# moberweger/deep-prior-pp

Measured on AMD Instinct MI355X. Metric: depth-crops/sec (NYU ResNet50 bs128) 1/2/4/8 GPU; mean 3D joint err (mm), higher is better.
Workload: dtype f32; 1 GPU; NYU posereg_embedding ResNet (type 0, 30-D PCA prior) train step: fused augment + fwd + bwd + ADAM, bs128/GPU fp32, 128x128x1 crops; global_batch=128, parallelism=dp1, augment=True, augment_pipelined=True, bn=local per-GPU batch statistics, launch_mode=native

## Files before the change

### deep-prior-pp_amd/csrc/bn.hip

```cpp
#include "dpp_common.h"

namespace {

constexpr int MAXQ = 256;

template <class TX>
__global__ __launch_bounds__(DPP_THREADS) void bn_stats_partial_kernel(const TX* __restrict__ X, int M, int C,
                                                                       int rpb, float* __restrict__ partial) {
    __shared__ float s_mean[DPP_THREADS * 4];
    __shared__ float s_m2[DPP_THREADS * 4];
    __shared__ float s_n[DPP_THREADS];
    const int Q = C >> 2;
    const int RP = DPP_THREADS / Q;
    const int tid = threadIdx.x;
    const int q = tid % Q, rr = tid / Q;
    const int r_begin = blockIdx.x * rpb;
    const int r_end = (r_begin + rpb < M) ? r_begin + rpb : M;
    float4 K = make_float4(0.f, 0.f, 0.f, 0.f), s1 = K, s2 = K;
    int n = 0;
    if (rr < RP) {
        for (int r = r_begin + rr; r < r_end; r += RP) {
            float4 v = dpp_ld4(X + (size_t)r * C + q * 4);
            if (n == 0) K = v;
            float dx = v.x - K.x, dy = v.y - K.y, dz = v.z - K.z, dw = v.w - K.w;
            s1.x += dx; s1.y += dy; s1.z += dz; s1.w += dw;
            s2.x += dx * dx; s2.y += dy * dy; s2.z += dz * dz; s2.w += dw * dw;
            ++n;
        }
    }
    float inv = n > 0 ? 1.0f / (float)n : 0.0f;
    s_n[tid] = (float)n;
    s_mean[tid * 4 + 0] = K.x + s1.x * inv; s_m2[tid * 4 + 0] = s2.x - s1.x * s1.x * inv;
    s_mean[tid * 4 + 1] = K.y + s1.y * inv; s_m2[tid * 4 + 1] = s2.y - s1.y * s1.y * inv;
    s_mean[tid * 4 + 2] = K.z + s1.z * inv; s_m2[tid * 4 + 2] = s2.z - s1.z * s1.z * inv;
    s_mean[tid * 4 + 3] = K.w + s1.w * inv; s_m2[tid * 4 + 3] = s2.w - s1.w * s1.w * inv;
    __syncthreads();
    for (int c = tid; c < C; c += DPP_THREADS) {
        int cq = c >> 2, ce = c & 3;
        double cn = 0.0, mean = 0.0, m2 = 0.0;
        for (int j = 0; j < RP; ++j) {
            int t = j * Q + cq;
            double nb = (double)s_n[t];
            if (nb == 0.0) continue;
            double mb = (double)s_mean[t * 4 + ce], m2b = (double)s_m2[t * 4 + ce];
            double delta = mb - mean, tot = cn + nb;
            mean += delta * nb / tot;
            m2 += m2b + delta * delta * cn * nb / tot;
            cn = tot;
        }
        partial[dpp_partial_index(0, c, blockIdx.x, C, gridDim.x)] = (float)mean;
        partial[dpp_partial_index(1, c, blockIdx.x, C, gridDim.x)] = (float)m2;
    }
}

__device__ __forceinline__ double wave_allsum(double v) {
    for (int o = 1; o < DPP_WAVE; o <<= 1) v += __shfl_xor(v, o);
    return v;
}

template <int WPC>
__device__ __forceinline__ double group_allsum(double v, double* slot) {
    v = wave_allsum(v);
    if (WPC == 1) return v;
    const int wave = threadIdx.x >> 6;
    if ((threadIdx.x & 63) == 0) slot[wave] = v;
    __syncthreads();
    return ((slot[0] + slot[1]) + slot[2]) + slot[3];
}

template <int U, int WPC>
__global__ __launch_bounds__(DPP_THREADS) void bn_finalize_kernel(const float* __restrict__ partial, int nbs, int nseg, int M, int rpb,
                                                                  int C, const float* __restrict__ gamma, float eps,
                                                                  float* __restrict__ mean_o, float* __restrict__ inv_std_o,
                                                                  float* __restrict__ scale_o, float* __restrict__ run_mean,
                                                                  float* __restrict__ run_inv_std, float alpha) {
    dpp_kernarg_warm<96>();
    __shared__ double slot_a[4], slot_b[4];
    constexpr int GT = DPP_WAVE * WPC;
    const int lane = threadIdx.x % GT;
    const int c = blockIdx.x * (DPP_THREADS / GT) + threadIdx.x / GT;
    const int cc = c < C ? c : C - 1;
    const bool upd = alpha > 0.0f && run_mean != nullptr;
    const float gam = gamma[cc];
    const float rm_old = (upd ? run_mean : gamma)[cc], ri_old = (upd ? run_inv_std : gamma)[cc];
    const int Mseg = M / nseg;
    auto rows_of = [&](int bi) { return (bi * rpb + rpb <= Mseg) ? rpb : (Mseg - bi * rpb); };
    const bool one_sweep = nseg == 1 && nbs <= GT * U;
    float pm0[U], pq0[U];
    if (one_sweep) {
        const float* pm_row = partial + dpp_partial_index(0, cc, 0, C, nbs);
        const float* pq_row = partial + dpp_partial_index(1, cc, 0, C, nbs);
        const float K = pm_row[0];
#pragma unroll
        for (int u = 0; u < U; ++u) {
            const int b = lane + u * GT;
            const int bb = b < nbs ? b : nbs - 1;
            pm0[u] = pm_row[bb];
            pq0[u] = pq_row[bb];
        }
        double s1 = 0.0, s2 = 0.0;
#pragma unroll
        for (int u = 0; u < U; ++u) {
            const int b = lane + u * GT;
            if (b < nbs) {
                const double d = (double)pm0[u] - (double)K, nb_ = (double)rows_of(b);
                s1 += nb_ * d;
                s2 += (double)pq0[u] + nb_ * d * d;
            }
        }
        s1 = group_allsum<WPC>(s1, slot_a);
        s2 = group_allsum<WPC>(s2, slot_b);
        if (lane != 0 || c >= C) return;
        const double mean1 = (double)K + s1 / (double)M;
        const double var1 = (s2 - s1 * s1 / (double)M) / (double)M;
        const float meanf = (float)mean1;
        const float inv_std = (float)(1.0 / sqrt((var1 > 0.0 ? var1 : 0.0) + (double)eps));
        mean_o[c] = meanf;
        inv_std_o[c] = inv_std;
        scale_o[c] = gam * inv_std;
        if (upd) {
            const float oma = 1.0f - alpha;
            run_mean[c] = oma * rm_old + alpha * meanf;
            run_inv_std[c] = oma * ri_old + alpha * inv_std;
        }
        return;
    }
    double snm = 0.0;
    for (int seg = 0; seg < nseg; ++seg) {
        const float* pm_row = partial + (size_t)seg * 2 * C * nbs + dpp_partial_index(0, cc, 0, C, nbs);
        const float* pq_row = partial + (size_t)seg * 2 * C * nbs + dpp_partial_index(1, cc, 0, C, nbs);
        for (int b0 = lane; b0 < nbs; b0 += GT * U) {
            float pm[U];
#pragma unroll
            for (int u = 0; u < U; ++u) {
                const int b = b0 + u * GT;
                const int bb = b < nbs ? b : nbs - 1;
                pm[u] = pm_row[bb];
            }
#pragma unroll
            for (int u = 0; u < U; ++u) {
                const int b = b0 + u * GT;
                if (b < nbs) snm += (double)rows_of(b) * (double)pm[u];
            }
        }
    }
    const double mean = group_allsum<WPC>(snm, slot_a) / (double)M;
    double q = 0.0;
    {
        for (int seg = 0; seg < nseg; ++seg) {
            const float* pm_row = partial + (size_t)seg * 2 * C * nbs + dpp_partial_index(0, cc, 0, C, nbs);
            const float* pq_row = partial + (size_t)seg * 2 * C * nbs + dpp_partial_index(1, cc, 0, C, nbs);
            for (int b0 = lane; b0 < nbs; b0 += GT * U) {
                float pm[U], pq[U];
#pragma unroll
                for (int u = 0; u < U; ++u) {
                    const int b = b0 + u * GT;
                    const int bb = b < nbs ? b : nbs - 1;
                    pm[u] = pm_row[bb];
                    pq[u] = pq_row[bb];
                }
#pragma unroll
                for (int u = 0; u < U; ++u) {
                    const int b = b0 + u * GT;
                    if (b < nbs) {
                        const double d = (double)pm[u] - mean;
                        q += (double)pq[u] + (double)rows_of(b) * d * d;
                    }
                }
            }
        }
    }
    const double m2 = group_allsum<WPC>(q, slot_b);
    if (lane != 0 || c >= C) return;
    double var = m2 / (double)M;
    float meanf = (float)mean;
    float inv_std = (float)(1.0 / sqrt(var + (double)eps));
    mean_o[c] = meanf;
    inv_std_o[c] = inv_std;
    scale_o[c] = gam * inv_std;
    if (upd) {
        float oma = 1.0f - alpha;
        run_mean[c] = oma * rm_old + alpha * meanf;
        run_inv_std[c] = oma * ri_old + alpha * inv_std;
    }
}

__global__ __launch_bounds__(DPP_THREADS) void bn_eval_coeffs_kernel(const float* __restrict__ gamma, const float* __restrict__ run_mean,
                                                                     const float* __restrict__ run_inv_std, int C,
                                                                     float* __restrict__ mean_o, float* __restrict__ inv_std_o,
                                                                     float* __restrict__ scale_o) {
    int c = blockIdx.x * DPP_THREADS + threadIdx.x;
    if (c >= C) return;
    mean_o[c] = run_mean[c];
    inv_std_o[c] = run_inv_std[c];
    scale_o[c] = gamma[c] * run_inv_std[c];
}

struct BnEvalJob { const float* gamma; const float* run_mean; const float* run_inv_std; float* mean; float* inv_std; float* scale; int C, block0; };
__global__ __launch_bounds__(DPP_THREADS) void bn_eval_coeffs_multi_kernel(const BnEvalJob* __restrict__ jobs, int njobs) {
    int lo = 0, hi = njobs - 1;
    while (lo < hi) {
        const int mid = (lo + hi + 1) >> 1;
        if ((int)blockIdx.x >= jobs[mid].block0) lo = mid; else hi = mid - 1;
    }
    const BnEvalJob jb = jobs[lo];
    const int c = ((int)blockIdx.x - jb.block0) * DPP_THREADS + threadIdx.x;
    if (c >= jb.C) return;
// ... 205 lines not shown
        if ((nb & 3) == 0) {
            for (int b = quarter * 4; b < nb; b += 16) {
                const float4 v = *reinterpret_cast<const float4*>(row + b);
                acc += ((double)v.x + (double)v.y) + ((double)v.z + (double)v.w);
            }
        } else {
            for (int b = quarter; b < nb; b += 4) acc += (double)row[b];
        }
        acc += __shfl_xor(acc, 1);
        acc += __shfl_xor(acc, 2);
        if (quarter == 0) s_sum[pair] = acc;
    }
    const float4 mu = *reinterpret_cast<const float4*>(mean + c0 + q * 4);
    const float4 is = *reinterpret_cast<const float4*>(inv_std + c0 + q * 4);
    const float4 sc = *reinterpret_cast<const float4*>(scale + c0 + q * 4);
    __syncthreads();
    if (blockIdx.x == 0 && tid < CS) {
        dbeta[c0 + tid] = (float)s_sum[tid];
        dgamma[c0 + tid] = (float)s_sum[CS + tid];
    }
    float4 a1, a2;
    a1.x = (float)(s_sum[q * 4 + 0] / (double)M); a1.y = (float)(s_sum[q * 4 + 1] / (double)M);
    a1.z = (float)(s_sum[q * 4 + 2] / (double)M); a1.w = (float)(s_sum[q * 4 + 3] / (double)M);
    a2.x = (float)(s_sum[CS + q * 4 + 0] / (double)M); a2.y = (float)(s_sum[CS + q * 4 + 1] / (double)M);
    a2.z = (float)(s_sum[CS + q * 4 + 2] / (double)M); a2.w = (float)(s_sum[CS + q * 4 + 3] / (double)M);
    float4 sa = zero4;
    for (; r < r_end; r += 4 * RP) {
#pragma unroll
        for (int u = 0; u < 4; ++u) {
            const int ru = r + u * RP;
            float4 v;
            v.x = sc.x * (g[u].x - a1.x - (x[u].x - mu.x) * is.x * a2.x);
            v.y = sc.y * (g[u].y - a1.y - (x[u].y - mu.y) * is.y * a2.y);
            v.z = sc.z * (g[u].z - a1.z - (x[u].z - mu.z) * is.z * a2.z);
            v.w = sc.w * (g[u].w - a1.w - (x[u].w - mu.w) * is.w * a2.w);
            if (add) { v.x += o[u].x; v.y += o[u].y; v.z += o[u].z; v.w += o[u].w; }
            if (ru < r_end) {
                dpp_st4(dX + (size_t)ru * C + c0 + q * 4, v);
                if (sizeof(TO) == 2) { v.x = dpp_bf16_round(v.x); v.y = dpp_bf16_round(v.y); v.z = dpp_bf16_round(v.z); v.w = dpp_bf16_round(v.w); }
                sa.x += v.x; sa.y += v.y; sa.z += v.z; sa.w += v.w;
            }
        }
        if (r + 4 * RP < r_end) fetch(r + 4 * RP);
    }
    if (colsum == nullptr) return;
    s_a[tid * 4 + 0] = sa.x; s_a[tid * 4 + 1] = sa.y; s_a[tid * 4 + 2] = sa.z; s_a[tid * 4 + 3] = sa.w;
    __syncthreads();
    if (tid < CS) {
        const int cq = tid >> 2, ce = tid & 3;
        double a = 0.0;
        for (int j = 0; j < RP; ++j) a += (double)s_a[(j * Q + cq) * 4 + ce];
        colsum[(size_t)blockIdx.x * C + c0 + tid] = (float)a;
    }
}

bool ok_c(int C) { return C >= 4 && (C & 3) == 0 && (C >> 2) <= MAXQ && (DPP_THREADS % (C >> 2) == 0 || (C >> 2) > DPP_THREADS); }

}

extern "C" int dpp_bn_stats_partial(const float* X, int M, int C, int rows_per_block, float* partial, int store, dpp_stream_t stream) {
    if (!X || !partial || M < 1 || rows_per_block < 1 || !ok_c(C) || (C >> 2) > DPP_THREADS || (store & ~DPP_ST_A)) return DPP_E_BADARG;
    int nb = dpp_cdiv(M, rows_per_block);
    if (store & DPP_ST_A)
        DPP_LAUNCH(bn_stats_partial_kernel<dpp_bf16>, dim3(nb), dim3(DPP_THREADS), 0, static_cast<hipStream_t>(stream),
                   reinterpret_cast<const dpp_bf16*>(X), M, C, rows_per_block, partial);
    else
        DPP_LAUNCH(bn_stats_partial_kernel<float>, dim3(nb), dim3(DPP_THREADS), 0, static_cast<hipStream_t>(stream), X, M, C, rows_per_block, partial);
    return dpp_launch_status();
}

extern "C" int dpp_bn_finalize(const float* partial, int nb, int nseg, int M, int rows_per_block, int C, const float* gamma, float eps,
                               float* mean, float* inv_std, float* scale, float* run_mean, float* run_inv_std, float alpha,
                               dpp_stream_t stream) {
    if (!partial || !gamma || !mean || !inv_std || !scale || nseg < 1 || M % nseg || nb != dpp_cdiv(M / nseg, rows_per_block))
        return DPP_E_BADARG;
    hipStream_t st = static_cast<hipStream_t>(stream);
#define DPP_BNF(U_, W_) DPP_LAUNCH((bn_finalize_kernel<U_, W_>), dim3(dpp_cdiv(C, 4 / W_)), dim3(DPP_THREADS), 0, st, partial, nb, nseg, \
                                           M, rows_per_block, C, gamma, eps, mean, inv_std, scale, run_mean, run_inv_std, alpha)
    if (nb <= 2 * DPP_WAVE) DPP_BNF(2, 1); else if (nb <= 8 * DPP_WAVE) DPP_BNF(8, 1); else if (nb <= 32 * DPP_WAVE) DPP_BNF(8, 4); else DPP_BNF(32, 4);
#undef DPP_BNF
    return dpp_launch_status();
}

extern "C" int dpp_bn_eval_coeffs(const float* gamma, const float* run_mean, const float* run_inv_std, int C, float* mean,
                                  float* inv_std, float* scale, dpp_stream_t stream) {
    if (!gamma || !run_mean || !run_inv_std || !mean || !inv_std || !scale || C < 1) return DPP_E_BADARG;
    DPP_LAUNCH(bn_eval_coeffs_kernel, dim3(dpp_cdiv(C, DPP_THREADS)), dim3(DPP_THREADS), 0, static_cast<hipStream_t>(stream),
                       gamma, run_mean, run_inv_std, C, mean, inv_std, scale);
    return dpp_launch_status();
}

extern "C" size_t dpp_bn_eval_job_bytes(void) { return sizeof(BnEvalJob); }

extern "C" int dpp_bn_eval_coeffs_multi(const void* jobs, int njobs, int total_blocks, dpp_stream_t stream) {
    if (!jobs || njobs < 1 || total_blocks < 1) return DPP_E_BADARG;
    DPP_LAUNCH(bn_eval_coeffs_multi_kernel, dim3(total_blocks), dim3(DPP_THREADS), 0, static_cast<hipStream_t>(stream),
               static_cast<const BnEvalJob*>(jobs), njobs);
    return dpp_launch_status();
}

extern "C" int dpp_bn_bwd_reduce(const float* dA, const float* X, int M, int C, const float* mean, const float* inv_std,
                                 const float* scale, const float* beta, int relu, float* G, int rows_per_block, float* partial,
                                 int store, dpp_stream_t stream) {
    if (!dA || !X || !G || !partial || M < 1 || rows_per_block < 1 || !ok_c(C) || (C >> 2) > DPP_THREADS || (store & ~(DPP_ST_BNX | DPP_ST_A | DPP_ST_C)))
        return DPP_E_BADARG;
    const bool x16 = (store & DPP_ST_BNX) != 0, g16 = (store & DPP_ST_A) != 0;
    if (g16 != ((store & DPP_ST_C) != 0)) return DPP_E_UNSUPPORTED;
    int nb = dpp_cdiv(M, rows_per_block);
    hipStream_t st = static_cast<hipStream_t>(stream);
#define DPP_BR(TX_, TG_) DPP_LAUNCH((bn_bwd_reduce_kernel<TX_, TG_>), dim3(nb), dim3(DPP_THREADS), 0, st, reinterpret_cast<const TG_*>(dA), \
                                    reinterpret_cast<const TX_*>(X), M, C, mean, inv_std, scale, beta, relu, reinterpret_cast<TG_*>(G), rows_per_block, partial)
    if (x16) { if (g16) DPP_BR(dpp_bf16, dpp_bf16); else DPP_BR(dpp_bf16, float); }
    else { if (g16) DPP_BR(float, dpp_bf16); else DPP_BR(float, float); }
#undef DPP_BR
    return dpp_launch_status();
}

extern "C" int dpp_bn_bwd_finalize(const float* partial, int nb, int nseg, int M, int C, float* dbeta, float* dgamma, float* c1,
                                   float* c2, const float* inv_std, const float* scale, float* q, float* p, dpp_stream_t stream) {
    if (!partial || !dbeta || !dgamma || !c1 || !c2 || nb < 1 || nseg < 1) return DPP_E_BADARG;
    if (q && !(p && inv_std && scale)) return DPP_E_BADARG;
    hipStream_t st = static_cast<hipStream_t>(stream);
#define DPP_BNBF(U_, W_) DPP_LAUNCH((bn_bwd_finalize_kernel<U_, W_>), dim3(dpp_cdiv(C, 4 / W_)), dim3(DPP_THREADS), 0, st, partial, nb, \
                                            nseg, M, C, dbeta, dgamma, c1, c2, inv_std, scale, q, p)
    if (nb <= 2 * DPP_WAVE) DPP_BNBF(2, 1); else if (nb <= 8 * DPP_WAVE) DPP_BNBF(8, 1); else if (nb <= 32 * DPP_WAVE) DPP_BNBF(8, 4); else DPP_BNBF(32, 4);
#undef DPP_BNBF
    return dpp_launch_status();
}

extern "C" int dpp_bn_bwd_apply(const float* G, const float* X, int M, int C, const float* mean, const float* inv_std,
                                const float* scale, const float* c1, const float* c2, const float* add, float* dX,
                                int rows_per_block, float* colsum_partial, int store, dpp_stream_t stream) {
    if (!G || !X || !dX || M < 1 || rows_per_block < 1 || !ok_c(C) || (C >> 2) > DPP_THREADS || (store & ~(DPP_ST_BNX | DPP_ST_A | DPP_ST_C)))
        return DPP_E_BADARG;
    const bool x16 = (store & DPP_ST_BNX) != 0, g16 = (store & DPP_ST_A) != 0, o16 = (store & DPP_ST_C) != 0;
    const dim3 grid(dpp_cdiv(M, rows_per_block));
    hipStream_t st = static_cast<hipStream_t>(stream);
#define DPP_BA(TX_, TG_, TO_) DPP_LAUNCH((bn_bwd_apply_kernel<TX_, TG_, TO_>), grid, dim3(DPP_THREADS), 0, st, reinterpret_cast<const TG_*>(G), \
                                         reinterpret_cast<const TX_*>(X), M, C, mean, inv_std, scale, c1, c2, reinterpret_cast<const TO_*>(add), \
                                         reinterpret_cast<TO_*>(dX), rows_per_block, colsum_partial)
#define DPP_BA_O(TX_, TG_) do { if (o16) DPP_BA(TX_, TG_, dpp_bf16); else DPP_BA(TX_, TG_, float); } while (0)
    if (x16) { if (g16) DPP_BA_O(dpp_bf16, dpp_bf16); else DPP_BA_O(dpp_bf16, float); }
    else { if (g16) DPP_BA_O(float, dpp_bf16); else DPP_BA_O(float, float); }
#undef DPP_BA_O
#undef DPP_BA
    return dpp_launch_status();
}

extern "C" int dpp_bn_bwd_finalize_apply_ok(int M, int C, int nb) { return M >= 1 && C >= 32 && (C & 31) == 0 && nb >= 1 && nb <= 256; }

extern "C" int dpp_bn_bwd_finalize_apply(const float* G, const float* X, int M, int C, const float* mean, const float* inv_std,
                                         const float* scale, const float* partial, int nb, const float* add, float* dX,
                                         int rows_per_block, float* colsum_partial, float* dbeta, float* dgamma, int store,
                                         dpp_stream_t stream) {
    if (!G || !X || !dX || !partial || !dbeta || !dgamma || rows_per_block < 1 || (store & ~(DPP_ST_BNX | DPP_ST_A | DPP_ST_C))) return DPP_E_BADARG;
    if (!dpp_bn_bwd_finalize_apply_ok(M, C, nb)) return DPP_E_UNSUPPORTED;
    const bool x16 = (store & DPP_ST_BNX) != 0, g16 = (store & DPP_ST_A) != 0, o16 = (store & DPP_ST_C) != 0;
    const dim3 grid(dpp_cdiv(M, rows_per_block), C / 32);
    hipStream_t st = static_cast<hipStream_t>(stream);
#define DPP_BFA(TX_, TG_, TO_) DPP_LAUNCH((bn_bwd_finalize_apply_kernel<TX_, TG_, TO_>), grid, dim3(DPP_THREADS), 0, st, reinterpret_cast<const TG_*>(G), \
                                          reinterpret_cast<const TX_*>(X), M, C, mean, inv_std, scale, partial, nb, reinterpret_cast<const TO_*>(add), \
                                          reinterpret_cast<TO_*>(dX), rows_per_block, colsum_partial, dbeta, dgamma)
#define DPP_BFA_O(TX_, TG_) do { if (o16) DPP_BFA(TX_, TG_, dpp_bf16); else DPP_BFA(TX_, TG_, float); } while (0)
    if (x16) { if (g16) DPP_BFA_O(dpp_bf16, dpp_bf16); else DPP_BFA_O(dpp_bf16, float); }
    else { if (g16) DPP_BFA_O(float, dpp_bf16); else DPP_BFA_O(float, float); }
#undef DPP_BFA_O
// ... 4 lines not shown
```

### deep-prior-pp_amd/csrc/conv3x3.hip

```cpp
#include <stdio.h>
#include <stdlib.h>
#include "dpp_common.h"
#include "conv3x3_wgrad_t.h"

namespace {

struct C3Stage {
    unsigned m_hw2, m_tw2;
    int lqp;
};

__host__ __device__ inline unsigned c3_magic(int d) { return (unsigned)(0x100000000ull / (unsigned)d) + 1u; }

struct Conv3Args {
    const float* X;
    int N, H, W, Ci, Co;
    dpp_act act;
    const float* Wk;
    int allw;
    int wide;
    const float* bias;
    const float* residual;
    float* Y;
    dpp_epilogue epi;
    int store;
    int lth, ltw;
    int img;
    int tiles_x, tiles_y;
    C3Stage sg;
    unsigned long long* prof;
    int ntiles, woff;
};

typedef __bf16 c3_bf16x8 __attribute__((ext_vector_type(8)));
typedef __bf16 c3_bf16x4 __attribute__((ext_vector_type(4)));

template <int PREC> struct C3Prec;
template <> struct C3Prec<0> { typedef float elem; static constexpr int PAD = 4; __device__ static int kp(int Ci) { return Ci; } };
template <> struct C3Prec<1> { typedef __bf16 elem; static constexpr int PAD = 8; __device__ static int kp(int Ci) { return Ci < 32 ? 32 : Ci; } };

__device__ __forceinline__ void c3_store4(float* dst, float4 v) { *reinterpret_cast<float4*>(dst) = v; }
__device__ __forceinline__ void c3_store4(__bf16* dst, float4 v) {
    c3_bf16x4 o;
    o[0] = (__bf16)v.x; o[1] = (__bf16)v.y; o[2] = (__bf16)v.z; o[3] = (__bf16)v.w;
    *reinterpret_cast<c3_bf16x4*>(dst) = o;
}

__device__ __forceinline__ void tile_origin(const Conv3Args& a, int bid, int& n0, int& y0, int& x0) {
    int bx = bid % a.tiles_x;
    int t = bid / a.tiles_x;
    int by = t % a.tiles_y;
    int bn = t / a.tiles_y;
    n0 = bn * a.img;
    y0 = by << a.lth;
    x0 = bx << a.ltw;
}

template <int UB, class E, class TX>
__device__ __forceinline__ void stage_halo(const TX* __restrict__ X, int N, int H, int W, int Ci, const dpp_act& act, int n0,
                                           int y0, int x0, int TH, int TW, int IMG, E* Ah, int LDA, int KP, const C3Stage& sg) {
    if (KP < Ci) KP = Ci;
    const int HW2 = (TH + 2) * (TW + 2), TW2 = TW + 2;
    const int HP = IMG * HW2;
    const int c0 = ((int)threadIdx.x & ((1 << sg.lqp) - 1)) * 4;
    const int hstep = DPP_THREADS >> sg.lqp;
    if (c0 >= KP) return;
    const bool cld = c0 < Ci;
    float4 mu = make_float4(0.f, 0.f, 0.f, 0.f), sc = mu, be = mu;
    if (cld && (act.mode & 2)) {
        mu = *reinterpret_cast<const float4*>(act.mean + c0);
        sc = *reinterpret_cast<const float4*>(act.scale + c0);
        be = *reinterpret_cast<const float4*>(act.beta + c0);
    }
    for (int hb = (int)threadIdx.x >> sg.lqp; hb < HP; hb += UB * hstep) {
        float4 v[UB];
        bool in[UB];
#pragma unroll
        for (int u = 0; u < UB; ++u) {
            const int hp = hb + u * hstep;
            const int im = (int)__umulhi((unsigned)hp, sg.m_hw2), rem = hp - im * HW2;
            const int hy = (int)__umulhi((unsigned)rem, sg.m_tw2), hx = rem - hy * TW2;
            const int n = n0 + im, y = y0 + hy - 1, x = x0 + hx - 1;
            in[u] = hp < HP && cld && n < N && y >= 0 && y < H && x >= 0 && x < W;
            v[u] = make_float4(0.f, 0.f, 0.f, 0.f);
            if (in[u]) v[u] = dpp_ld4(X + (((size_t)n * H + y) * W + x) * Ci + c0);
        }
#pragma unroll
        for (int u = 0; u < UB; ++u) {
            const int hp = hb + u * hstep;
            if (hp < HP) {
                float4 t = v[u];
                if (in[u]) {
                    if (act.mode & 2) {
                        t.x = dpp_fma(t.x - mu.x, sc.x, be.x); t.y = dpp_fma(t.y - mu.y, sc.y, be.y);
                        t.z = dpp_fma(t.z - mu.z, sc.z, be.z); t.w = dpp_fma(t.w - mu.w, sc.w, be.w);
                    }
                    if (act.mode & 1) { t.x = fmaxf(t.x, 0.0f); t.y = fmaxf(t.y, 0.0f); t.z = fmaxf(t.z, 0.0f); t.w = fmaxf(t.w, 0.0f); }
                }
                c3_store4(&Ah[hp * LDA + c0], t);
            }
        }
    }
}

template <int BM, int BN, int PREC = 0, class TX = float, bool EST = false>
__global__ __launch_bounds__(DPP_THREADS) void conv3x3_kernel(Conv3Args a) {
    dpp_kernarg_warm<sizeof(Conv3Args)>();
    HIP_DYNAMIC_SHARED(float4, smem4)
    float* smem = reinterpret_cast<float*>(smem4);
    typedef typename C3Prec<PREC>::elem elem;
    constexpr int RM = BM / 64;
    constexpr int CN = BN / 16;
    constexpr int KSTEP = PREC ? 32 : 16;
    const int TH = 1 << a.lth, TW = 1 << a.ltw;
    const int Ci = a.Ci, KP = C3Prec<PREC>::kp(Ci), LDA = KP + C3Prec<PREC>::PAD;
    const int HP = a.img * (TH + 2) * (TW + 2);
    elem* Ah = reinterpret_cast<elem*>(smem);
    elem* Bs = Ah + HP * LDA;
    const int tid = threadIdx.x, wave = tid >> 6, lane = tid & 63, l15 = lane & 15, kq = lane >> 4;
    int n0, y0, x0;
    tile_origin(a, blockIdx.x, n0, y0, x0);
    const int col0 = blockIdx.y * BN;

    dpp_stamp(a.prof, 0);
    dpp_wide_coef wco;
    if (a.wide) wco.load<BN>(col0, a.Co, a.bias, a.epi, a.Y);
    if (((HP + (DPP_THREADS >> a.sg.lqp) - 1) >> (8 - a.sg.lqp)) <= 4)
        stage_halo<4>(reinterpret_cast<const TX*>(a.X), a.N, a.H, a.W, Ci, a.act, n0, y0, x0, TH, TW, a.img, Ah, LDA, KP, a.sg);
    else
        stage_halo<8>(reinterpret_cast<const TX*>(a.X), a.N, a.H, a.W, Ci, a.act, n0, y0, x0, TH, TW, a.img, Ah, LDA, KP, a.sg);
    dpp_stamp(a.prof, 1);

    int hbase[RM];
#pragma unroll
    for (int rt = 0; rt < RM; ++rt) {
        int row = wave * (BM / 4) + rt * 16 + l15;
        int im = row >> (a.lth + a.ltw);
        int ty = (row >> a.ltw) & (TH - 1);
        int tx = row & (TW - 1);
        hbase[rt] = (im * (TH + 2) + ty + 1) * (TW + 2) + tx + 1;
    }

    f32x4 acc[RM][CN];
#pragma unroll
    for (int i = 0; i < RM; ++i)
#pragma unroll
        for (int j = 0; j < CN; ++j) acc[i][j] = (f32x4){0.f, 0.f, 0.f, 0.f};

    constexpr int WSLOTS = (BN * 16 + DPP_THREADS - 1) / DPP_THREADS;
    float4 wreg[WSLOTS];
    const float* wp[WSLOTS];
    int wo[WSLOTS];
#pragma unroll
    for (int s = 0; s < WSLOTS; ++s) {
        const int slot = tid + s * DPP_THREADS;
        const int j = slot >> a.sg.lqp, c0 = (slot & ((1 << a.sg.lqp) - 1)) * 4;
        wo[s] = (j < BN && c0 < KP) ? j * LDA + c0 : -1;
        wp[s] = (j < BN && c0 < Ci && col0 + j < a.Co) ? a.Wk + (size_t)(col0 + j) * 9 * Ci + c0 : nullptr;
    }
    auto wfetch = [&](int tap) {
#pragma unroll
        for (int s = 0; s < WSLOTS; ++s) {
            wreg[s] = make_float4(0.f, 0.f, 0.f, 0.f);
            if (wp[s] != nullptr) wreg[s] = *reinterpret_cast<const float4*>(wp[s] + tap * Ci);
        }
    };
    auto wcommit = [&](elem* dst) {
#pragma unroll
        for (int s = 0; s < WSLOTS; ++s)
            if (wo[s] >= 0) c3_store4(&dst[wo[s]], wreg[s]);
    };
    const bool allw = a.allw != 0;
    if (allw) {
#pragma unroll
        for (int t3 = 0; t3 < 9; t3 += 3) {
            float4 w3[3][WSLOTS];
#pragma unroll
            for (int u = 0; u < 3; ++u)
#pragma unroll
                for (int s = 0; s < WSLOTS; ++s) {
                    w3[u][s] = make_float4(0.f, 0.f, 0.f, 0.f);
                    if (wp[s] != nullptr) w3[u][s] = *reinterpret_cast<const float4*>(wp[s] + (t3 + u) * Ci);
                }
#pragma unroll
            for (int u = 0; u < 3; ++u)
#pragma unroll
                for (int s = 0; s < WSLOTS; ++s)
                    if (wo[s] >= 0) c3_store4(&Bs[(t3 + u) * BN * LDA + wo[s]], w3[u][s]);
        }
    } else {
        wfetch(0);
        wcommit(Bs);
    }
    __syncthreads();
    dpp_stamp(a.prof, 2);
    for (int tap = 0; tap < 9; ++tap) {
        const elem* Bcur = allw ? Bs + tap * BN * LDA : Bs + (tap & 1) * BN * LDA;
        if (!allw && tap + 1 < 9) wfetch(tap + 1);
        const int toff = (tap / 3 - 1) * (TW + 2) + (tap % 3 - 1);
        for (int kc = 0; kc < KP; kc += KSTEP) {
            if constexpr (PREC == 0) {
                float4 av[RM], bv[CN];
#pragma unroll
                for (int rt = 0; rt < RM; ++rt)
                    av[rt] = *reinterpret_cast<const float4*>(&Ah[(hbase[rt] + toff) * LDA + kc + kq * 4]);
#pragma unroll
                for (int ct = 0; ct < CN; ++ct)
                    bv[ct] = *reinterpret_cast<const float4*>(&Bcur[(ct * 16 + l15) * LDA + kc + kq * 4]);
#pragma unroll
// ... 425 lines not shown
                        v = dpp_ld4(reinterpret_cast<const TY*>(a.dY) + (((size_t)n * a.H + y) * a.W + x) * Co + c0);
                    *reinterpret_cast<float4*>(&Ys[row * LDY + c0]) = v;
                }
            }
        }
        __syncthreads();

#pragma unroll 1
        for (int rc = 0; rc < BM; rc += 16) {
            int hb[4];
#pragma unroll
            for (int t = 0; t < 4; ++t) {
                int row = rc + kq * 4 + t;
                int im = row >> (a.lth + a.ltw);
                int ty = (row >> a.ltw) & (TH - 1);
                int tx = row & (TW - 1);
                hb[t] = ((im * (TH + 2) + ty + 1) * (TW + 2) + tx + 1) * LDA;
            }
            const float* yrow = Ys + (rc + kq * 4) * LDY;
#pragma unroll
            for (int i = 0; i < MAXACC; ++i) {
                if (yoff[i] >= 0) {
#pragma unroll
                    for (int t = 0; t < 4; ++t) {
                        float av = yrow[t * LDY + yoff[i]];
                        float bv = Ah[hb[t] + xoff[i]];
                        acc[i] = __builtin_amdgcn_mfma_f32_16x16x4f32(av, bv, acc[i], 0, 0, 0);
                    }
                }
            }
        }
    }

    float* out = a.partial + (size_t)blockIdx.x * Co * 9 * Ci;
#pragma unroll
    for (int i = 0; i < MAXACC; ++i) {
        int p = wave + 4 * i;
        if (p < pairs) {
            int tap = tap0 + p / NT, tile = p % NT;
            int to = tile / ntc, tc = tile - to * ntc;
#pragma unroll
            for (int r = 0; r < 4; ++r) {
                int o = to * 16 + kq * 4 + r, c = tc * 16 + l15;
                out[((size_t)o * 9 + tap) * Ci + c] = acc[i][r];
            }
        }
    }
}

constexpr int WGRAD_MAX_BLOCKS = 256;

int ilog2(int v) { int l = 0; while ((1 << l) < v) ++l; return l; }

void pick_tile(int N, int H, int W, int bm, int& lth, int& ltw, int& img) {
    int tw = 1; while (tw * 2 <= W && tw < 16) tw *= 2;
    int th = 1; while (th * 2 <= H && th < 8 && th * tw * 2 <= bm) th *= 2;
    while (th * tw > bm) tw /= 2;
    img = bm / (th * tw);
    lth = ilog2(th); ltw = ilog2(tw);
}

}

extern "C" int dpp_conv3x3_tiling(int N, int H, int W, int bm, int* th, int* tw, int* img) {
    int lth, ltw, im;
    if (bm != 64 && bm != 128) return -1;
    pick_tile(N, H, W, bm, lth, ltw, im);
    if (th) *th = 1 << lth;
    if (tw) *tw = 1 << ltw;
    if (img) *img = im;
    return dpp_cdiv(W, 1 << ltw) * dpp_cdiv(H, 1 << lth) * dpp_cdiv(N, im);
}

static int conv3x3_launch(const float* X, int N, int H, int W, int Ci, const dpp_act* act, const float* Wk, int Co,
                          const float* bias, const float* residual, float* Y, int bm, const dpp_epilogue* epi, int precision, int store,
                          dpp_stream_t stream) {
    if (!X || !Wk || !Y || N < 1 || H < 1 || W < 1 || Ci < 16 || (Ci & 15) || Co < 16 || (Co & 15)) return DPP_E_BADARG;
    if (store & ~(DPP_ST_A | DPP_ST_C | DPP_ST_BNX)) return DPP_E_BADARG;
    Conv3Args a;
    a.store = store;
    a.X = X; a.N = N; a.H = H; a.W = W; a.Ci = Ci; a.Co = Co;
    a.prof = dpp_prof_buffer;
    if (act && (act->mode & 4)) return DPP_E_UNSUPPORTED;
    if (act) a.act = *act; else { a.act.mode = 0; a.act.cmod = 1; a.act.mean = a.act.scale = a.act.beta = nullptr; }
    a.Wk = Wk; a.bias = bias; a.residual = residual; a.Y = Y;
    if (epi) a.epi = *epi; else a.epi = dpp_epilogue{};
    if (a.epi.bn_x && !(a.epi.bn_mean && a.epi.bn_inv_std && a.epi.bn_scale && a.epi.bn_beta && a.epi.bn_partial)) return DPP_E_BADARG;
    long pixels = (long)N * H * W;
    if (bm == 0) bm = (pixels / 128) * dpp_cdiv(Co, 64) >= 512 ? 128 : 64;
    pick_tile(N, H, W, bm, a.lth, a.ltw, a.img);
    int TH = 1 << a.lth, TW = 1 << a.ltw;
    a.tiles_x = dpp_cdiv(W, TW); a.tiles_y = dpp_cdiv(H, TH);
    int nblk = a.tiles_x * a.tiles_y * dpp_cdiv(N, a.img);
    if (Ci > 64) return DPP_E_UNSUPPORTED;
    a.sg.m_hw2 = c3_magic((TH + 2) * (TW + 2));
    a.sg.m_tw2 = c3_magic(TW + 2);
    a.sg.lqp = ilog2(((precision && Ci < 32) ? 32 : Ci) / 4);
    int bn = Co >= 64 ? 64 : (Co >= 32 ? 32 : 16);
    static const long min_wgs = []() { const char* e = getenv("DPP_C3_MIN_WGS"); return (e && atol(e) > 0) ? atol(e) : 512L; }();
    while (bn > 16 && (long)nblk * dpp_cdiv(Co, bn) < min_wgs) bn >>= 1;
    size_t halo = (size_t)a.img * (TH + 2) * (TW + 2);
    const size_t rowb = precision ? (size_t)((Ci < 32 ? 32 : Ci) + 8) * 2 : (size_t)(Ci + 4) * sizeof(float);
    a.allw = (halo + 9 * bn) * rowb <= 48 * 1024;
    size_t lds = (halo + (a.allw ? 9 : 2) * bn) * rowb;
    static const bool wide_ok = []() { const char* e = getenv("DPP_GEMM_WIDE_EPILOGUE"); return !(e && e[0] == '0'); }();
    auto al16 = [](const void* p) { return (reinterpret_cast<uintptr_t>(p) & 15) == 0; };
    a.wide = wide_ok && al16(Y) && al16(residual) && al16(a.epi.bn_x) && al16(bias) && al16(a.epi.bn_mean) && al16(a.epi.bn_scale) &&
             al16(a.epi.bn_beta) && al16(a.epi.bn_inv_std);
    if ((store & (DPP_ST_C | DPP_ST_BNX)) && !a.wide) return DPP_E_UNSUPPORTED;
    size_t need = a.wide ? ((size_t)bm * (bn + 4) + 16 * bn) * sizeof(float) : (size_t)4 * bn * sizeof(float);
    if (lds < need) lds = need;
    if (lds > 160 * 1024) return DPP_E_UNSUPPORTED;
    dim3 grid(nblk, dpp_cdiv(Co, bn));
    hipStream_t st = static_cast<hipStream_t>(stream);
    const char* pe = getenv("DPP_C3_PERSIST");
    const int persist = pe ? atoi(pe) : 1024;
    static const int p_min = []() { const char* e = getenv("DPP_C3_P_MIN_TILES"); return e ? atoi(e) : 0; }();
    const bool p_always = nblk > p_min;
    auto pow2 = [](int v) { return v > 0 && (v & (v - 1)) == 0; };
    const char* g0e = getenv("DPP_C3_P_64W");
    const int bn64 = g0e ? atoi(g0e) : 32;
    const bool geom0 = (Ci == 16 || Ci == 32 || (Ci == 64 && precision && (bn64 == 64 || bn64 == 32))) && a.img == 1 && TH == 8 && TW == 16 && H % TH == 0 && W % TW == 0 &&
                       pow2(a.tiles_x) && pow2(a.tiles_y);
    const char* g1e = getenv("DPP_C3_P_64");
    const int geom1_on = g1e ? atoi(g1e) : 1;
    const bool geom1 = (geom1_on >= 2 || (geom1_on == 1 && precision)) && Ci == 64 && H == 8 && W == 8 && a.img == 2 && TH == 8 && TW == 8;
    if (persist > 0 && a.wide && Ci == Co && bm == 128 && p_always && (geom0 || geom1) && (long)N * H * W * Ci < (1L << 31)) {
        const int pbn = geom1 ? 16 : (Ci == 64 ? bn64 : Co);
        const size_t pneed = ((size_t)bm * (pbn + 4) + 16 * pbn) * sizeof(float);
        const size_t region0 = (halo * rowb > pneed ? halo * rowb : pneed);
        const size_t ldsp = ((region0 + 15) & ~(size_t)15) + 9 * pbn * rowb + 8 * 64 * sizeof(float);
        const long pwgs = (long)(persist < nblk ? persist : nblk) * (Co / pbn);
        if (ldsp <= 64 * 1024 || (ldsp <= 80 * 1024 && pwgs <= 512) || (ldsp <= 160 * 1024 && pwgs <= 256)) {
            a.woff = (int)((region0 + 15) & ~(size_t)15);
            a.ntiles = nblk;
            if (geom0) { a.ltw = ilog2(a.tiles_x); a.lth = ilog2(a.tiles_y); }
            const dim3 gp(persist < nblk ? persist : nblk, Co / pbn);
            if (getenv("DPP_C3_PERSIST_VERBOSE")) fprintf(stderr, "conv3x3_p_kernel: %d tiles on %d x %d workgroups, C %d, prec %d, store %d, %zu bytes of LDS\n", nblk, (int)gp.x, (int)gp.y, Ci, precision, store, ldsp);
#define DPP_C3P(CI_, BN_, P_, T_, E_, G_) do { \
            if (ldsp > 64 * 1024) (void)hipFuncSetAttribute(reinterpret_cast<const void*>(&conv3x3_p_kernel<CI_, BN_, P_, T_, E_, G_>), hipFuncAttributeMaxDynamicSharedMemorySize, (int)ldsp); \
            DPP_LAUNCH((conv3x3_p_kernel<CI_, BN_, P_, T_, E_, G_>), gp, dim3(DPP_THREADS), ldsp, st, a); return dpp_launch_status(); } while (0)
#define DPP_C3PE(CI_, BN_, P_, T_, G_) do { if (store & (DPP_ST_C | DPP_ST_BNX)) DPP_C3P(CI_, BN_, P_, T_, true, G_); else DPP_C3P(CI_, BN_, P_, T_, false, G_); } while (0)
#define DPP_C3PX(CI_, BN_, G_) if (Ci == CI_) { \
            if (precision) { if (store & DPP_ST_A) DPP_C3PE(CI_, BN_, 1, dpp_bf16, G_); else DPP_C3PE(CI_, BN_, 1, float, G_); } \
            if (store & DPP_ST_A) DPP_C3PE(CI_, BN_, 0, dpp_bf16, G_); else DPP_C3PE(CI_, BN_, 0, float, G_); }
            DPP_C3PX(16, 16, 0) DPP_C3PX(32, 32, 0)
            if (geom1) { DPP_C3PX(64, 16, 1) }
            if (Ci == 64 && precision && pbn == 64) { if (store & DPP_ST_A) DPP_C3PE(64, 64, 1, dpp_bf16, 0); else DPP_C3PE(64, 64, 1, float, 0); }
            if (Ci == 64 && precision && pbn == 32) { if (store & DPP_ST_A) DPP_C3PE(64, 32, 1, dpp_bf16, 0); else DPP_C3PE(64, 32, 1, float, 0); }
#undef DPP_C3PX
#undef DPP_C3PE
#undef DPP_C3P
        }
    }
#define DPP_C3K(BM_, BN_, P_, T_, E_) do { \
        if (lds > 64 * 1024) (void)hipFuncSetAttribute(reinterpret_cast<const void*>(&conv3x3_kernel<BM_, BN_, P_, T_, E_>), hipFuncAttributeMaxDynamicSharedMemorySize, (int)lds); \
        DPP_LAUNCH((conv3x3_kernel<BM_, BN_, P_, T_, E_>), grid, dim3(DPP_THREADS), lds, st, a); return dpp_launch_status(); } while (0)
#define DPP_C3E(BM_, BN_, P_, T_) do { if (store & (DPP_ST_C | DPP_ST_BNX)) DPP_C3K(BM_, BN_, P_, T_, true); else DPP_C3K(BM_, BN_, P_, T_, false); } while (0)
#define DPP_C3(BM_, BN_) if (bm == BM_ && bn == BN_) { \
        if (precision) { if (store & DPP_ST_A) DPP_C3E(BM_, BN_, 1, dpp_bf16); else DPP_C3E(BM_, BN_, 1, float); } \
        if (store & DPP_ST_A) DPP_C3E(BM_, BN_, 0, dpp_bf16); else DPP_C3E(BM_, BN_, 0, float); }
    DPP_C3(128, 64) DPP_C3(128, 32) DPP_C3(128, 16) DPP_C3(64, 64) DPP_C3(64, 32) DPP_C3(64, 16)
#undef DPP_C3
#undef DPP_C3E
#undef DPP_C3K
    return DPP_E_UNSUPPORTED;
}

extern "C" int dpp_conv3x3(const float* X, int N, int H, int W, int Ci, const dpp_act* act, const float* Wk, int Co,
                           const float* bias, const float* residual, float* Y, int bm, const dpp_epilogue* epi, int store, dpp_stream_t stream) {
    return conv3x3_launch(X, N, H, W, Ci, act, Wk, Co, bias, residual, Y, bm, epi, 0, store, stream);
}

extern "C" int dpp_conv3x3_bf16(const float* X, int N, int H, int W, int Ci, const dpp_act* act, const float* Wk, int Co,
                                const float* bias, const float* residual, float* Y, int bm, const dpp_epilogue* epi, int store, dpp_stream_t stream) {
    return conv3x3_launch(X, N, H, W, Ci, act, Wk, Co, bias, residual, Y, bm, epi, 1, store, stream);
}

extern "C" int dpp_conv3x3_wtrans(const float* Wk, int Co, int Ci, float* Wd, dpp_stream_t stream) {
    if (!Wk || !Wd || Co < 1 || Ci < 1) return DPP_E_BADARG;
    int n = Co * 9 * Ci;
    DPP_LAUNCH(conv3x3_wtrans_kernel, dim3(dpp_cdiv(n, DPP_THREADS)), dim3(DPP_THREADS), 0, static_cast<hipStream_t>(stream), Wk, Co, Ci, Wd);
    return dpp_launch_status();
}

extern "C" size_t dpp_wtrans_job_bytes(void) { return sizeof(WtransJob); }

extern "C" int dpp_conv3x3_wtrans_multi(const void* jobs_dev, int njobs, int total_blocks, dpp_stream_t stream) {
    if (!jobs_dev || njobs < 1 || total_blocks < 1) return DPP_E_BADARG;
    DPP_LAUNCH(conv3x3_wtrans_multi_kernel, dim3(total_blocks), dim3(DPP_THREADS), 0, static_cast<hipStream_t>(stream),
               static_cast<const WtransJob*>(jobs_dev), njobs);
    return dpp_launch_status();
}

static void wgrad_geometry(int N, int H, int W, int Ci, int Co, int bm, int& nblk, int& taps_pb) {
    int lth, ltw, img;
    pick_tile(N, H, W, bm, lth, ltw, img);
    const int ntiles = dpp_cdiv(W, 1 << ltw) * dpp_cdiv(H, 1 << lth) * dpp_cdiv(N, img);
    const int NT = (Co >> 4) * (Ci >> 4);
    taps_pb = NT <= 4 ? 9 : (NT <= 16 ? 3 : 1);
    int cap = WGRAD_MAX_BLOCKS;
    while (cap > 32 && (long)cap * Co * 9 * Ci * 4 > 6L * 1024 * 1024) cap >>= 1;
    if (Ci == 64 && Co == 64 && dpp_conv3x3_wgrad_t_ok(N, H, W, Ci, Co, nullptr) && cap < 64) cap = 64;
    if (Ci == 32 && Co == 32 && ntiles >= 1024 && dpp_conv3x3_wgrad_t_ok(N, H, W, Ci, Co, nullptr) && cap < 256) cap = 256;
    nblk = ntiles < cap ? ntiles : cap;
    while (taps_pb > 1 && nblk * (9 / taps_pb) < 256) taps_pb = taps_pb == 9 ? 3 : 1;
}

extern "C" int dpp_conv3x3_wgrad_blocks(int N, int H, int W, int Ci, int Co, int bm) {
    if ((bm != 64 && bm != 128) || Ci < 16 || Co < 16) return -1;
    int nblk, taps_pb;
    wgrad_geometry(N, H, W, Ci, Co, bm, nblk, taps_pb);
    return nblk;
}

static int conv3x3_wgrad_launch(const float* X, int N, int H, int W, int Ci, const dpp_act* act, const float* dY, int Co,
                                float* partial, int bm, int store, int precision, dpp_stream_t stream);

extern "C" int dpp_conv3x3_wgrad(const float* X, int N, int H, int W, int Ci, const dpp_act* act, const float* dY, int Co,
                                 float* partial, int bm, int store, dpp_stream_t stream) {
    return conv3x3_wgrad_launch(X, N, H, W, Ci, act, dY, Co, partial, bm, store, 0, stream);
}

extern "C" int dpp_conv3x3_wgrad_bf16_ok(int N, int H, int W, int Ci, int Co) { return dpp_conv3x3_wgrad_t_ok(N, H, W, Ci, Co, nullptr) ? 1 : 0; }

extern "C" int dpp_conv3x3_wgrad_bf16(const float* X, int N, int H, int W, int Ci, const dpp_act* act, const float* dY, int Co,
                                      float* partial, int bm, int store, dpp_stream_t stream) {
    return conv3x3_wgrad_launch(X, N, H, W, Ci, act, dY, Co, partial, bm, store, 1, stream);
}

static int conv3x3_wgrad_launch(const float* X, int N, int H, int W, int Ci, const dpp_act* act, const float* dY, int Co,
                                float* partial, int bm, int store, int precision, dpp_stream_t stream) {
    if (!X || !dY || !partial || N < 1 || Ci < 16 || (Ci & 15) || Co < 16 || (Co & 15) || (bm != 64 && bm != 128) || (store & ~(DPP_ST_A | DPP_ST_B))) return DPP_E_BADARG;
    const int y16 = (store & DPP_ST_B) ? 1 : 0;
    Wgrad3Args a;
    a.X = X; a.N = N; a.H = H; a.W = W; a.Ci = Ci; a.Co = Co; a.dY = dY; a.partial = partial;
    if (act && (act->mode & 4)) return DPP_E_UNSUPPORTED;
    if (act) a.act = *act; else { a.act.mode = 0; a.act.cmod = 1; a.act.mean = a.act.scale = a.act.beta = nullptr; }
    pick_tile(N, H, W, bm, a.lth, a.ltw, a.img);
    int TH = 1 << a.lth, TW = 1 << a.ltw;
    a.tiles_x = dpp_cdiv(W, TW); a.tiles_y = dpp_cdiv(H, TH);
    a.ntiles = a.tiles_x * a.tiles_y * dpp_cdiv(N, a.img);
    int nblk, taps_pb;
    wgrad_geometry(N, H, W, Ci, Co, bm, nblk, taps_pb);
    if (dpp_conv3x3_wgrad_t_ok(N, H, W, Ci, Co, act))
        return dpp_conv3x3_wgrad_t_launch(X, N, H, W, Ci, act, dY, partial, nblk, taps_pb, store, precision, static_cast<hipStream_t>(stream));
    if (precision) return DPP_E_UNSUPPORTED;
    int NT = (Co >> 4) * (Ci >> 4);
    int pairs = taps_pb * NT;
    int maxacc = dpp_cdiv(pairs, 4);
    a.taps_pb = taps_pb;
    a.sg.m_hw2 = c3_magic((TH + 2) * (TW + 2));
    a.sg.m_tw2 = c3_magic(TW + 2);
    a.sg.lqp = ilog2(Ci / 4);
    a.lqy = ilog2(Co / 4);
    size_t lds = ((size_t)a.img * (TH + 2) * (TW + 2) * (Ci + 4) + (size_t)bm * (Co + 4)) * sizeof(float);
    if (lds > 160 * 1024) return DPP_E_UNSUPPORTED;
    dim3 grid(nblk, 9 / taps_pb);
    hipStream_t st = static_cast<hipStream_t>(stream);
#define DPP_W3K(BM_, MA_, T_, Y_) do { \
        if (lds > 64 * 1024) (void)hipFuncSetAttribute(reinterpret_cast<const void*>(&conv3x3_wgrad_kernel<BM_, MA_, T_, Y_>), hipFuncAttributeMaxDynamicSharedMemorySize, (int)lds); \
        DPP_LAUNCH((conv3x3_wgrad_kernel<BM_, MA_, T_, Y_>), grid, dim3(DPP_THREADS), lds, st, a); return dpp_launch_status(); } while (0)
#define DPP_W3(BM_, MA_) if (bm == BM_ && maxacc <= MA_) { \
        if (store & DPP_ST_A) { if (y16) DPP_W3K(BM_, MA_, dpp_bf16, dpp_bf16); else DPP_W3K(BM_, MA_, dpp_bf16, float); } \
        else { if (y16) DPP_W3K(BM_, MA_, float, dpp_bf16); else DPP_W3K(BM_, MA_, float, float); } }
    DPP_W3(128, 3) DPP_W3(128, 4) DPP_W3(128, 9) DPP_W3(128, 12) DPP_W3(128, 16)
    DPP_W3(64, 3) DPP_W3(64, 4) DPP_W3(64, 9) DPP_W3(64, 12) DPP_W3(64, 16)
#undef DPP_W3
    return DPP_E_UNSUPPORTED;
}
```

### deep-prior-pp_amd/csrc/conv3x3_wgrad_t.hip

```cpp
#include <stdlib.h>
#include "dpp_common.h"
#include "conv3x3_wgrad_t.h"

namespace {

template <class T> struct W3Raw;
template <> struct W3Raw<float> {
    typedef float4 type;
    __device__ static __forceinline__ type ld(const float* p) { return *reinterpret_cast<const float4*>(p); }
    __device__ static __forceinline__ float4 widen(const type& r) { return r; }
};
template <> struct W3Raw<dpp_bf16> {
    typedef uint2 type;
    __device__ static __forceinline__ type ld(const dpp_bf16* p) { return *reinterpret_cast<const uint2*>(p); }
    __device__ static __forceinline__ float4 widen(const type& r) {
        return make_float4(__uint_as_float(r.x << 16), __uint_as_float(r.x & 0xffff0000u), __uint_as_float(r.y << 16),
                           __uint_as_float(r.y & 0xffff0000u));
    }
};

struct Wgrad3TArgs {
    const void* X;
    const void* dY;
    float* partial;
// ... 222 lines not shown
                            const w3_u32x4 bv = w3_shift8(b0, lo, hi, dxi);
                            acc[dyi * 3 + dxi][n] = __builtin_amdgcn_mfma_f32_16x16x32_bf16(__builtin_bit_cast(dpp_bf16x8, av), __builtin_bit_cast(dpp_bf16x8, bv),
                                                                                            acc[dyi * 3 + dxi][n], 0, 0, 0);
                        }
                    }
                }
                }
            }
        }
    }

    if (C == 16) {
        f32x4* const red = reinterpret_cast<f32x4*>(smem);
        __syncthreads();
        if (wave >= 2) {
#pragma unroll
            for (int t = 0; t < TPB; ++t) red[((wave - 2) * TPB + t) * 64 + lane] = acc[t][0];
        }
        __syncthreads();
        if (wave < 2) {
#pragma unroll
            for (int t = 0; t < TPB; ++t) acc[t][0] += red[(wave * TPB + t) * 64 + lane];
        }
        __syncthreads();
        if (wave == 1) {
#pragma unroll
            for (int t = 0; t < TPB; ++t) red[t * 64 + lane] = acc[t][0];
        }
        __syncthreads();
        if (wave == 0) {
#pragma unroll
            for (int t = 0; t < TPB; ++t) acc[t][0] += red[t * 64 + lane];
        }
    }
    if (C != 16 || wave == 0) {
        float* out = a.partial + (size_t)blockIdx.x * C * 9 * C;
#pragma unroll
        for (int t = 0; t < TPB; ++t) {
            const int tap = tap0 + t;
#pragma unroll
            for (int n = 0; n < NTC; ++n)
#pragma unroll
                for (int r = 0; r < 4; ++r) {
                    const int o = (OS ? (int)blockIdx.y : to) * 16 + kq * 4 + r, c = (tc0 + n) * 16 + l15;
                    out[((size_t)o * 9 + tap) * C + c] = acc[t][n][r];
                }
        }
    }
}

template <int C, int TPB, bool PB>
int w3t_launch_typed(const Wgrad3TArgs& a, dim3 grid, size_t lds, bool x16, bool y16, hipStream_t st) {
#define DPP_W3T(TX_, TY_) do { DPP_LAUNCH((conv3x3_wgrad_t_kernel<C, TPB, TX_, TY_, PB>), grid, dim3(DPP_THREADS), lds, st, a); return dpp_launch_status(); } while (0)
    if (x16) { if (y16) DPP_W3T(dpp_bf16, dpp_bf16); else DPP_W3T(dpp_bf16, float); }
    if (y16) DPP_W3T(float, dpp_bf16);
    DPP_W3T(float, float);
#undef DPP_W3T
}

template <int C, bool PB>
int w3t_launch_taps(const Wgrad3TArgs& a, int taps_pb, dim3 grid, size_t lds, bool x16, bool y16, hipStream_t st) {
    if (taps_pb == 9) return w3t_launch_typed<C, 9, PB>(a, grid, lds, x16, y16, st);
    if (taps_pb == 3) return w3t_launch_typed<C, 3, PB>(a, grid, lds, x16, y16, st);
    return w3t_launch_typed<C, 1, PB>(a, grid, lds, x16, y16, st);
}

template <bool PB>
int w3t_launch_c64(const Wgrad3TArgs& a, dim3 grid, size_t lds, bool x16, bool y16, hipStream_t st) {
#define DPP_W3T64(TX_, TY_) do { \
        if (lds > 64 * 1024) (void)hipFuncSetAttribute(reinterpret_cast<const void*>(&conv3x3_wgrad_t_kernel<64, 9, TX_, TY_, PB, true>), hipFuncAttributeMaxDynamicSharedMemorySize, (int)lds); \
        DPP_LAUNCH((conv3x3_wgrad_t_kernel<64, 9, TX_, TY_, PB, true>), grid, dim3(DPP_THREADS), lds, st, a); return dpp_launch_status(); } while (0)
    if (x16) { if (y16) DPP_W3T64(dpp_bf16, dpp_bf16); else DPP_W3T64(dpp_bf16, float); }
    if (y16) DPP_W3T64(float, dpp_bf16);
    DPP_W3T64(float, float);
#undef DPP_W3T64
}

}

bool dpp_conv3x3_wgrad_t_ok(int N, int H, int W, int Ci, int Co, const dpp_act* act) {
    static const bool on = []() { const char* e = getenv("DPP_WGRAD3_T"); return !(e && e[0] == '0'); }();
    if (!on || Ci != Co || (Ci != 16 && Ci != 32 && Ci != 64) || W < 12 || H < 4) return false;
    if ((long)N * H * W * Ci >= (1L << 31)) return false;
    if (act && ((act->mode & 4) || (act->mode && (act->cmod & 3)))) return false;
    return true;
}

int dpp_conv3x3_wgrad_t_launch(const float* X, int N, int H, int W, int C, const dpp_act* act, const float* dY, float* partial, int nblk,
                               int taps_pb, int store, int precision, hipStream_t st) {
    Wgrad3TArgs a;
    a.X = X; a.dY = dY; a.partial = partial; a.N = N; a.H = H; a.W = W;
    if (act) a.act = *act; else { a.act = dpp_act{}; a.act.mode = 0; a.act.cmod = 4; }
    a.tiles_x = dpp_cdiv(W, W3_TW); a.tiles_y = dpp_cdiv(H, W3_TH);
    a.ntiles = a.tiles_x * a.tiles_y * N;
    const bool x16 = (store & DPP_ST_A) != 0, y16 = (store & DPP_ST_B) != 0;
    const dim3 grid(nblk, 9 / taps_pb);
    size_t lds = precision ? (size_t)C * (W3_CPXB + W3_CPYB) * 2 : (size_t)C * (W3_CPX + W3_CPY) * sizeof(float);
    const size_t red = C == 16 ? (size_t)2 * taps_pb * 64 * 16 : 0;
    if (lds < red) lds = red;
    if (C == 64) {
        const dim3 g64(nblk, 4);
        const size_t l64 = precision ? (size_t)(64 * W3_CPXB + 16 * W3_CPYB) * 2 : (size_t)(64 * W3_CPX + 16 * W3_CPY) * sizeof(float);
        return precision ? w3t_launch_c64<true>(a, g64, l64, x16, y16, st) : w3t_launch_c64<false>(a, g64, l64, x16, y16, st);
    }
    if (precision) return C == 16 ? w3t_launch_taps<16, true>(a, taps_pb, grid, lds, x16, y16, st) : w3t_launch_taps<32, true>(a, taps_pb, grid, lds, x16, y16, st);
    return C == 16 ? w3t_launch_taps<16, false>(a, taps_pb, grid, lds, x16, y16, st) : w3t_launch_taps<32, false>(a, taps_pb, grid, lds, x16, y16, st);
}
```

### deep-prior-pp_amd/csrc/convpool.hip

```cpp
#include "dpp_common.h"

namespace {

constexpr int TP = 8;
constexpr int WG_WAVES = DPP_THREADS / DPP_WAVE;

struct cp_geom {
    int N, H, W, Ci, kh, kw, pad, Co, pool, Hp, Wp, tiles_x, tiles_y, sy, sx;
};

__host__ inline bool cp_make_geom(cp_geom& g, int N, int H, int W, int Ci, int kh, int kw, int pad, int Co, int pool) {
    if (N < 1 || H < 1 || W < 1 || Ci < 1 || Ci > 32 || Co < 1 || Co > 32 || kh < 1 || kw < 1 || kh > 7 || kw > 7 || pad < 0 ||
        pad > 3 || pool < 1 || pool > 4)
        return false;
    g.N = N; g.H = H; g.W = W; g.Ci = Ci; g.kh = kh; g.kw = kw; g.pad = pad; g.Co = Co; g.pool = pool;
    int Hc = H + 2 * pad - kh + 1, Wc = W + 2 * pad - kw + 1;
    if (Hc < pool || Wc < pool) return false;
    g.Hp = Hc / pool; g.Wp = Wc / pool;
    g.tiles_y = dpp_cdiv(g.Hp, TP); g.tiles_x = dpp_cdiv(g.Wp, TP);
    g.sy = TP * pool + kh - 1; g.sx = TP * pool + kw - 1;
    return true;
}

__device__ __forceinline__ void cp_stage(float* xs, const float* __restrict__ X, const dpp_act& act, const cp_geom& g, int n, int ty,
// ... 371 lines not shown
    for (int s0 = threadIdx.x; s0 < S * S * g.Co; s0 += DPP_THREADS * SU) {
        float d[SU];
        int m[SU];
#pragma unroll
        for (int u = 0; u < SU; ++u) {
            const int s = s0 + u * DPP_THREADS;
            const int co = s % g.Co, rc = s / g.Co;
            const int c = rc % S, r = rc / S;
            const int cy = cy0 + r, cx = cx0 + c;
            const bool ok = (s < S * S * g.Co) & (cy >= 0) & (cx >= 0) & (cy < Hc) & (cx < Wc);
            const int py = ok ? cy / P : 0, px = ok ? cx / P : 0;
            const int j = ok ? (cy - py * P) * P + (cx - px * P) : 0;
            const size_t o = (((size_t)n * g.Hp + py) * g.Wp + px) * g.Co + (ok ? co : 0);
            d[u] = dY[o];
            m[u] = ok ? ((ties ? (int)ties[o] : 1) >> j) & 1 : 0;
        }
#pragma unroll
        for (int u = 0; u < SU; ++u) {
            const int s = s0 + u * DPP_THREADS;
            const int co = s % g.Co, rc = s / g.Co;
            if (s < S * S * g.Co) gcs[(co * S + rc / S) * S + rc % S] = m[u] ? d[u] : 0.0f;
        }
    }
    for (int s = threadIdx.x; s < g.Co * taps * 8; s += DPP_THREADS) {
        const int ci = s & 7, ct = s >> 3;
        ws[s] = (c0 + ci < g.Ci) ? Wk[(size_t)ct * g.Ci + c0 + ci] : 0.0f;
    }
    __syncthreads();
    const int ly0 = (threadIdx.x >> 4) * PX, lx0 = (threadIdx.x & 15) * PX;
    float acc[PX * PX][8];
#pragma unroll
    for (int q = 0; q < PX * PX; ++q)
#pragma unroll
        for (int c = 0; c < 8; ++c) acc[q][c] = 0.0f;
    for (int co = 0; co < g.Co; ++co) {
        float patch[R][R];
        const float* gp = gcs + (co * S + ly0) * S + lx0;
#pragma unroll
        for (int r = 0; r < R; ++r)
#pragma unroll
            for (int c = 0; c < R; ++c) patch[r][c] = gp[r * S + c];
#pragma unroll
        for (int dy = 0; dy < K; ++dy)
#pragma unroll
            for (int dx = 0; dx < K; ++dx) {
                const float4* wp = reinterpret_cast<const float4*>(ws + (co * taps + dy * K + dx) * 8);
                const float4 w0 = wp[0], w1 = wp[1];
                const float w[8] = {w0.x, w0.y, w0.z, w0.w, w1.x, w1.y, w1.z, w1.w};
#pragma unroll
                for (int qy = 0; qy < PX; ++qy)
#pragma unroll
                    for (int qx = 0; qx < PX; ++qx) {
                        const float gv = patch[qy + K - 1 - dy][qx + K - 1 - dx];
#pragma unroll
                        for (int c = 0; c < 8; ++c) acc[qy * PX + qx][c] = fmaf(gv, w[c], acc[qy * PX + qx][c]);
                    }
            }
    }
#pragma unroll
    for (int qy = 0; qy < PX; ++qy)
#pragma unroll
        for (int qx = 0; qx < PX; ++qx) {
            const int iy = iy0 + ly0 + qy, ix = ix0 + lx0 + qx;
            if (iy < g.H && ix < g.W) {
                float* o = dX + (((size_t)n * g.H + iy) * g.W + ix) * g.Ci + c0;
#pragma unroll
                for (int c = 0; c < 8; ++c)
                    if (c0 + c < g.Ci) o[c] = acc[qy * PX + qx][c];
            }
        }
}

inline dpp_act cp_act(const dpp_act* a) {
    dpp_act r = {nullptr, nullptr, nullptr, 0, 1};
    return a ? *a : r;
}

constexpr int CP_WGRAD_MAX_BLOCKS = 512;

}

extern "C" int dpp_convpool_fwd(const float* X, int N, int H, int W, int Ci, const dpp_act* act, const float* Wk, int kh, int kw, int pad,
                                int Co, int pool, const float* bias, float* Y, uint16_t* ties, dpp_stream_t stream) {
    if (act && (act->mode & 4)) return DPP_E_UNSUPPORTED;
    cp_geom g;
    if (!X || !Wk || !bias || !Y || !cp_make_geom(g, N, H, W, Ci, kh, kw, pad, Co, pool)) return DPP_E_BADARG;
    size_t lds = (size_t)g.sy * g.sx * Ci * sizeof(float);
    if (lds > 64 * 1024) return DPP_E_UNSUPPORTED;
    dim3 grid(N * g.tiles_x * g.tiles_y), block(DPP_THREADS);
    hipStream_t st = static_cast<hipStream_t>(stream);
    int cpt = dpp_cdiv(Co, WG_WAVES);
    const size_t lds_fast = lds + (size_t)Co * kh * kw * Ci * sizeof(float);
    if (kh == kw && cpt <= 2 && lds_fast <= 64 * 1024) {
#define DPP_CPF(K_, P_) if (kh == K_ && pool == P_) { \
            DPP_LAUNCH((convpool_fwd_fast_kernel<K_, P_, 2>), grid, block, lds_fast, st, X, cp_act(act), Wk, bias, Y, ties, g); \
            return dpp_launch_status(); }
        DPP_CPF(5, 4) DPP_CPF(5, 2) DPP_CPF(5, 1) DPP_CPF(3, 1) DPP_CPF(3, 2)
#undef DPP_CPF
    }
    if (cpt <= 2)
        DPP_LAUNCH((convpool_fwd_kernel<2>), grid, block, lds, st, X, cp_act(act), Wk, bias, Y, ties, g);
    else if (cpt <= 4)
        DPP_LAUNCH((convpool_fwd_kernel<4>), grid, block, lds, st, X, cp_act(act), Wk, bias, Y, ties, g);
    else
        DPP_LAUNCH((convpool_fwd_kernel<8>), grid, block, lds, st, X, cp_act(act), Wk, bias, Y, ties, g);
    return dpp_launch_status();
}

extern "C" int dpp_convpool_wgrad_blocks(int N, int Hp, int Wp) {
    if (N < 1 || Hp < 1 || Wp < 1) return 0;
    long total = (long)N * dpp_cdiv(Hp, TP) * dpp_cdiv(Wp, TP);
    return (int)(total < CP_WGRAD_MAX_BLOCKS ? total : CP_WGRAD_MAX_BLOCKS);
}

extern "C" int dpp_convpool_wgrad(const float* X, int N, int H, int W, int Ci, const dpp_act* act, const float* dY, const uint16_t* ties,
                                  int kh, int kw, int pad, int Co, int pool, float* partial, dpp_stream_t stream) {
    if (act && (act->mode & 4)) return DPP_E_UNSUPPORTED;
    cp_geom g;
    if (!X || !dY || !partial || !cp_make_geom(g, N, H, W, Ci, kh, kw, pad, Co, pool) || (pool > 1 && !ties)) return DPP_E_BADARG;
    size_t lds = ((size_t)g.sy * g.sx * Ci + 2 * 64 * Co) * sizeof(float);
    if (lds > 64 * 1024) return DPP_E_UNSUPPORTED;
    int total = N * g.tiles_x * g.tiles_y;
    int blocks = dpp_convpool_wgrad_blocks(N, g.Hp, g.Wp);
    if (kh * kw * Ci <= DPP_THREADS && pool <= 2) {
        const int T = (Ci <= 2) ? 32 : 16;
        const size_t need = ((size_t)Ci * (T + kh - 1) * (T + kw - 1) + (size_t)T * T * 8) * sizeof(float);
        if (need <= 64 * 1024 && (size_t)DPP_THREADS * 8 <= (size_t)T * T * 8) {
            const int tiles_x = dpp_cdiv(g.Wp * pool, T), tiles_y = dpp_cdiv(g.Hp * pool, T);
            DPP_LAUNCH(convpool_wgrad_dense_kernel, dim3(blocks, dpp_cdiv(Co, 8)), dim3(DPP_THREADS), need, static_cast<hipStream_t>(stream), X,
                       cp_act(act), dY, ties, partial, g, T, tiles_x, tiles_y, N * tiles_x * tiles_y);
            return dpp_launch_status();
        }
    }
    DPP_LAUNCH(convpool_wgrad_kernel, dim3(blocks), dim3(DPP_THREADS), lds, static_cast<hipStream_t>(stream), X, cp_act(act), dY,
                       ties, partial, g, total);
    return dpp_launch_status();
}

extern "C" int dpp_convpool_dgrad(const float* dY, const uint16_t* ties, int N, int H, int W, int Ci, const float* Wk, int kh, int kw,
                                  int pad, int Co, int pool, float* dX, dpp_stream_t stream) {
    cp_geom g;
    if (!dY || !Wk || !dX || !cp_make_geom(g, N, H, W, Ci, kh, kw, pad, Co, pool) || (pool > 1 && !ties)) return DPP_E_BADARG;
    if (kh == kw) {
        const int px = ((long)N * dpp_cdiv(H, 32) * dpp_cdiv(W, 32) >= 1024 && (H > 16 || W > 16)) ? 2 : 1, T = 16 * px, S = T + kh - 1;
        const size_t lds = ((size_t)Co * S * S + (size_t)Co * kh * kw * 8) * sizeof(float);
        const int tiles_x = dpp_cdiv(W, T), tiles_y = dpp_cdiv(H, T);
        const dim3 fgrid(N * tiles_x * tiles_y, dpp_cdiv(Ci, 8));
        if (lds <= 64 * 1024) {
#define DPP_CPD(K_, P_, PX_) if (kh == K_ && pool == P_ && px == PX_) { \
                DPP_LAUNCH((convpool_dgrad_fast_kernel<K_, P_, PX_>), fgrid, dim3(DPP_THREADS), lds, static_cast<hipStream_t>(stream), dY, ties, \
                           Wk, dX, g, tiles_x, tiles_y); \
                return dpp_launch_status(); }
            DPP_CPD(5, 2, 2) DPP_CPD(5, 2, 1) DPP_CPD(5, 1, 2) DPP_CPD(5, 1, 1) DPP_CPD(3, 1, 2) DPP_CPD(3, 1, 1) DPP_CPD(3, 2, 2) DPP_CPD(3, 2, 1)
            DPP_CPD(5, 4, 2) DPP_CPD(5, 4, 1)
#undef DPP_CPD
        }
    }
    size_t npix = (size_t)N * H * W;
    dim3 grid((unsigned)((npix + DPP_THREADS - 1) / DPP_THREADS), dpp_cdiv(Ci, 8));
    DPP_LAUNCH(convpool_dgrad_kernel, grid, dim3(DPP_THREADS), 0, static_cast<hipStream_t>(stream), dY, ties, Wk, dX, g);
    return dpp_launch_status();
}
```

### deep-prior-pp_amd/csrc/dpp_common.h

```cpp
#pragma once
#include <hip/hip_runtime.h>
#include <stdint.h>
#include "../../include/dpp_hip.h"

typedef float f32x4 __attribute__((ext_vector_type(4)));

typedef __bf16 dpp_bf16;
typedef __bf16 dpp_bf16x4 __attribute__((ext_vector_type(4)));
typedef __bf16 dpp_bf16x8 __attribute__((ext_vector_type(8)));

template <class T> __device__ __forceinline__ float4 dpp_ld4(const T* p);
template <> __device__ __forceinline__ float4 dpp_ld4<float>(const float* p) { return *reinterpret_cast<const float4*>(p); }
template <> __device__ __forceinline__ float4 dpp_ld4<dpp_bf16>(const dpp_bf16* p) {
    const dpp_bf16x4 v = *reinterpret_cast<const dpp_bf16x4*>(p);
    return make_float4((float)v[0], (float)v[1], (float)v[2], (float)v[3]);
}
template <class T> __device__ __forceinline__ float dpp_ld1(const T* p) { return (float)p[0]; }
template <class T> __device__ __forceinline__ void dpp_st4(T* p, float4 v);
template <> __device__ __forceinline__ void dpp_st4<float>(float* p, float4 v) { *reinterpret_cast<float4*>(p) = v; }
template <> __device__ __forceinline__ void dpp_st4<dpp_bf16>(dpp_bf16* p, float4 v) {
    dpp_bf16x4 o;
    o[0] = (dpp_bf16)v.x; o[1] = (dpp_bf16)v.y; o[2] = (dpp_bf16)v.z; o[3] = (dpp_bf16)v.w;
    *reinterpret_cast<dpp_bf16x4*>(p) = o;
}
// ... 89 lines not shown
extern unsigned long long* dpp_prof_buffer;

#ifdef DPP_HIP_EMU
#define DPP_WAVES_PER_EU(lo, hi)
#else
#define DPP_WAVES_PER_EU(lo, hi) __attribute__((amdgpu_waves_per_eu(lo, hi)))
#endif

#ifdef DPP_HIP_EMU
#define DPP_SCHED_FENCE()
#else
#define DPP_SCHED_FENCE() __builtin_amdgcn_sched_barrier(0)
#endif

#ifdef DPP_HIP_EMU
#define DPP_SETPRIO(p)
#else
#define DPP_SETPRIO(p) __builtin_amdgcn_s_setprio(p)
#endif

#ifdef DPP_HIP_EMU
#define DPP_WAVE_SYNC() ((void)__shfl_xor(0, 1))
#else
#define DPP_WAVE_SYNC() __builtin_amdgcn_wave_barrier()
#endif

template <int NBYTES>
__device__ __forceinline__ void dpp_kernarg_warm() {
#ifndef DPP_HIP_EMU
    typedef __attribute__((address_space(4))) const int kint;
    kint* ka = (kint*)__builtin_amdgcn_kernarg_segment_ptr();
    constexpr int L = (NBYTES + 63) / 64;
    int t[L];
#pragma unroll
    for (int i = 0; i < L; ++i) t[i] = ka[i * 16];
#pragma unroll
    for (int i = 0; i < L; ++i) asm volatile("" ::"s"(t[i]));
#endif
}

__device__ __forceinline__ int dpp_map_row(const dpp_rowmap& m, int r) {
    if (m.s == 1) return r;
    int n = r / m.HoWo;
    int q = r - n * m.HoWo;
    int y = q / m.Wo;
    int x = q - y * m.Wo;
    return n * m.HiWi + (y * m.s) * m.Wi + x * m.s;
}

__device__ __forceinline__ float dpp_fma(float a, float b, float c) { return __builtin_fmaf(a, b, c); }

__device__ __forceinline__ float dpp_act1(float x, const dpp_act& a, int c) {
    float v = x;
    if (a.mode & 2) v = dpp_fma(x - a.mean[c], a.scale[c], a.beta[c]);
    if (a.mode & 1) v = fmaxf(v, 0.0f);
    return v;
}

__device__ __forceinline__ float4 dpp_act4(float4 x, const dpp_act& a, int c) {
    float4 v = x;
    if (a.mode & 2) {
        const float4 mu = *reinterpret_cast<const float4*>(a.mean + c);
        const float4 sc = *reinterpret_cast<const float4*>(a.scale + c);
        const float4 be = *reinterpret_cast<const float4*>(a.beta + c);
        v.x = dpp_fma(x.x - mu.x, sc.x, be.x);
        v.y = dpp_fma(x.y - mu.y, sc.y, be.y);
        v.z = dpp_fma(x.z - mu.z, sc.z, be.z);
        v.w = dpp_fma(x.w - mu.w, sc.w, be.w);
    }
    if (a.mode & 1) {
        v.x = fmaxf(v.x, 0.0f);
        v.y = fmaxf(v.y, 0.0f);
        v.z = fmaxf(v.z, 0.0f);
        v.w = fmaxf(v.w, 0.0f);
    }
    return v;
}

__device__ __forceinline__ float dpp_f4_get(const float4& v, int i) {
    return i == 0 ? v.x : (i == 1 ? v.y : (i == 2 ? v.z : v.w));
}

__device__ __forceinline__ size_t dpp_partial_index(int s, int c, int b, int C, int NB) { return ((size_t)s * C + c) * NB + b; }


template <int CN, int WM, int WN, int BN>
__device__ __forceinline__ void dpp_tile_colsum(float (&s)[CN], float* red, int wm, int wn, int l15, int kq) {
#pragma unroll
    for (int ct = 0; ct < CN; ++ct) {
        s[ct] += __shfl_xor(s[ct], 16);
        s[ct] += __shfl_xor(s[ct], 32);
    }
    if (WM > 1) {
        __syncthreads();
        if (kq == 0) {
#pragma unroll
            for (int ct = 0; ct < CN; ++ct) red[wm * BN + wn * (BN / WN) + ct * 16 + l15] = s[ct];
        }
        __syncthreads();
#pragma unroll
        for (int ct = 0; ct < CN; ++ct) {
            float t = 0.0f;
#pragma unroll
            for (int w = 0; w < WM; ++w) t += red[w * BN + wn * (BN / WN) + ct * 16 + l15];
            s[ct] = t;
        }
    }
}

struct dpp_wide_coef {
    float cbias[4], cmean[4], cscale[4], cbeta[4], cistd[4];
    float4 raw[5];
    bool on_bias, on_bn;
    template <int BN>
    __device__ __forceinline__ void load(int col0, int N, const float* bias, const dpp_epilogue& ep, const float* safe) {
        const int col = col0 + ((int)threadIdx.x % (BN / 4)) * 4;
        const bool cin = col < N;
        on_bias = cin && bias != nullptr;
        on_bn = cin && ep.bn_x != nullptr;
        raw[0] = *reinterpret_cast<const float4*>(on_bias ? bias + col : safe);
        raw[1] = *reinterpret_cast<const float4*>(on_bn ? ep.bn_mean + col : safe);
        raw[2] = *reinterpret_cast<const float4*>(on_bn ? ep.bn_scale + col : safe);
        raw[3] = *reinterpret_cast<const float4*>(on_bn ? ep.bn_beta + col : safe);
        raw[4] = *reinterpret_cast<const float4*>(on_bn ? ep.bn_inv_std + col : safe);
    }
    __device__ __forceinline__ void finish() {
        auto quad = [](const float4& v, bool on, float (&dst)[4]) {
            dst[0] = on ? v.x : 0.0f; dst[1] = on ? v.y : 0.0f; dst[2] = on ? v.z : 0.0f; dst[3] = on ? v.w : 0.0f;
        };
        quad(raw[0], on_bias, cbias);
        quad(raw[1], on_bn, cmean);
        quad(raw[2], on_bn, cscale);
        quad(raw[3], on_bn, cbeta);
        quad(raw[4], on_bn, cistd);
    }
};

template <int RM, int CN, int WM, int WN, int BM, int BN, int NIMG = 1, bool ST = false, class RowOff>
__device__ __forceinline__ void dpp_epilogue_wide(f32x4 (&acc)[RM][CN], float* smem, int col0, int N, dpp_wide_coef& co,
                                                  const float* residual, float* C, const dpp_epilogue& ep, int nvalid, int wm,
                                                  int wn, int l15, int kq, RowOff rowoff, int img = 0, int store = 0, int blk = -1, int nblk = 0) {
    const int pblk = blk >= 0 ? blk : (int)blockIdx.x, pnblk = blk >= 0 ? nblk : (int)gridDim.x;
    const bool c16 = ST && (store & DPP_ST_C) != 0, x16 = ST && (store & DPP_ST_BNX) != 0;
    co.finish();
    constexpr int LDT = BN + 4;
    constexpr int Q = BN / 4;
    constexpr int RSTEP = DPP_THREADS / Q;
    constexpr int ITERS = (BM + RSTEP - 1) / RSTEP;
    float* Ts = smem;
    float* red = smem + NIMG * BM * LDT;
    const int tid = threadIdx.x, lane = tid & 63, wave = tid >> 6;
    const int cq = tid % Q, rb = tid / Q;
    const int col = col0 + cq * 4;
    const bool cin = col < N;
    const bool bn = ep.bn_x != nullptr;
    long rofs[ITERS];
    float4 res32[ITERS], bnx32[ITERS];
    uint2 res16[ITERS], bnx16[ITERS];
    auto request = [&](int it) {
        const int rl = rb + it * RSTEP;
        rofs[it] = (rl < BM && cin) ? rowoff(rl) : -1L;
        const size_t o = rofs[it] >= 0 ? (size_t)rofs[it] + col : (size_t)0;
        if (residual) {
            if (c16) res16[it] = *reinterpret_cast<const uint2*>(reinterpret_cast<const dpp_bf16*>(residual) + o);
            else res32[it] = *reinterpret_cast<const float4*>(residual + o);
        }
// ... 135 lines not shown
```

### deep-prior-pp_amd/csrc/gemm.hip

```cpp
#include "gemm_kernels.h"

namespace {

__global__ __launch_bounds__(DPP_THREADS) void reduce_partials_kernel(const float* __restrict__ partial, int nz, int n,
                                                                      const float* __restrict__ bias, int nbias,
                                                                      float* __restrict__ out, int ZL) {
    __shared__ float red[DPP_THREADS];
    const int CB = DPP_THREADS / ZL;
    const int col = threadIdx.x % CB, zl = threadIdx.x / CB;
    for (int i0 = blockIdx.x * CB; i0 < n; i0 += gridDim.x * CB) {
        int i = i0 + col;
        float s = 0.0f;
        if (i < n)
            for (int z = zl; z < nz; z += ZL) s += partial[(size_t)z * n + i];
        if (ZL > 1) {
            red[threadIdx.x] = s;
            __syncthreads();
            if (zl == 0) {
                for (int j = 1; j < ZL; ++j) s += red[j * CB + col];
            }
        }
        if (zl == 0 && i < n) {
            if (bias) s += bias[i % nbias];
            out[i] = s;
// ... 9 lines not shown
};

constexpr int RM_COLS = 64;

__global__ __launch_bounds__(DPP_THREADS) void reduce_multi_kernel(const ReduceJob* __restrict__ jobs, int njobs) {
    __shared__ __attribute__((aligned(16))) float red[DPP_THREADS * 4];
    __shared__ int s_job;
    if (threadIdx.x == 0) {
        int lo = 0, hi = njobs - 1;
        while (lo < hi) {
            int mid = (lo + hi + 1) >> 1;
            if (jobs[mid].block0 <= (int)blockIdx.x) lo = mid; else hi = mid - 1;
        }
        s_job = lo;
    }
    __syncthreads();
    const ReduceJob jb = jobs[s_job];
    constexpr int ZL = 16, CQ = DPP_THREADS / ZL;
    const int cq = threadIdx.x % CQ, zl = threadIdx.x / CQ;
    const int i = ((int)blockIdx.x - jb.block0) * RM_COLS + cq * 4;
    const int n = jb.n, nz = jb.nz;
    const bool vec = (n & 3) == 0 && (reinterpret_cast<uintptr_t>(jb.partial) & 15) == 0;
    float s[4][4];
#pragma unroll
    for (int u = 0; u < 4; ++u)
#pragma unroll
        for (int j = 0; j < 4; ++j) s[u][j] = 0.0f;
    if (i < n) {
        if (vec) {
            const float* p = jb.partial + i;
            int z = zl;
            for (; z + 3 * ZL < nz; z += 4 * ZL) {
                float4 v[4];
#pragma unroll
                for (int u = 0; u < 4; ++u) v[u] = *reinterpret_cast<const float4*>(p + (size_t)(z + u * ZL) * n);
#pragma unroll
                for (int u = 0; u < 4; ++u) { s[u][0] += v[u].x; s[u][1] += v[u].y; s[u][2] += v[u].z; s[u][3] += v[u].w; }
            }
            for (; z < nz; z += ZL) {
                const float4 v = *reinterpret_cast<const float4*>(p + (size_t)z * n);
                s[0][0] += v.x; s[0][1] += v.y; s[0][2] += v.z; s[0][3] += v.w;
            }
        } else {
            for (int z = zl; z < nz; z += ZL)
#pragma unroll
                for (int j = 0; j < 4; ++j)
                    if (i + j < n) s[0][j] += jb.partial[(size_t)z * n + i + j];
        }
    }
    float4 t;
    t.x = (s[0][0] + s[1][0]) + (s[2][0] + s[3][0]);
    t.y = (s[0][1] + s[1][1]) + (s[2][1] + s[3][1]);
    t.z = (s[0][2] + s[1][2]) + (s[2][2] + s[3][2]);
    t.w = (s[0][3] + s[1][3]) + (s[2][3] + s[3][3]);
    *reinterpret_cast<float4*>(&red[threadIdx.x * 4]) = t;
    __syncthreads();
    if (zl == 0 && i < n) {
        for (int j = 1; j < ZL; ++j) {
            const float4 o = *reinterpret_cast<const float4*>(&red[(j * CQ + cq) * 4]);
            t.x += o.x; t.y += o.y; t.z += o.z; t.w += o.w;
        }
        if (vec && (reinterpret_cast<uintptr_t>(jb.out) & 15) == 0) *reinterpret_cast<float4*>(jb.out + i) = t;
        else {
            const float tv[4] = {t.x, t.y, t.z, t.w};
#pragma unroll
            for (int j = 0; j < 4; ++j)
                if (i + j < n) jb.out[i + j] = tv[j];
        }
    }
}

bool aligned16(const void* p) { return (reinterpret_cast<uintptr_t>(p) & 15) == 0; }

static int gemm_prepare(const dpp_gemm_desc* dp, GemmArgs& ga) {
    if (!dp || !dp->A || !dp->B || dp->M <= 0 || dp->N <= 0 || dp->K <= 0) return DPP_E_BADARG;
    ga.d = *dp;
    ga.prof = dpp_prof_buffer;
    dpp_gemm_desc& d = ga.d;
    if (d.splitk < 1) d.splitk = 1;
    if (d.splitk > 1 && !d.partial) return DPP_E_BADARG;
    if (d.splitk > 1 && (d.epi.stats || d.epi.bn_x)) return DPP_E_BADARG;
    if (d.epi.bn_x && !(d.epi.bn_mean && d.epi.bn_inv_std && d.epi.bn_scale && d.epi.bn_beta && d.epi.bn_partial)) return DPP_E_BADARG;
    if (d.splitk == 1 && !d.C) return DPP_E_BADARG;
    if (d.actA.mode && d.actA.cmod <= 0) return DPP_E_BADARG;
    if (d.actB.mode && d.actB.cmod <= 0) return DPP_E_BADARG;
    ga.vecA = aligned16(d.A) && (d.lda % 4 == 0);
    if (d.actB.mode & 4) return DPP_E_UNSUPPORTED;
    if (d.actA.mode & 4) {
        if (d.actA.mode != 4 || d.variant == 1 || !d.actA.x2 || !d.actA.aux || !d.actA.mean || !d.actA.scale || !d.actA.beta) return DPP_E_BADARG;
        ga.vecA = ga.vecA && aligned16(d.actA.x2) && aligned16(d.actA.out);
        if (d.actA.out && (!d.a_kc || d.splitk != 1 || d.mapA.s != 1)) return DPP_E_UNSUPPORTED;
        if (!(aligned16(d.actA.mean) && aligned16(d.actA.scale) && aligned16(d.actA.beta) && aligned16(d.actA.aux))) return DPP_E_BADARG;
    }
    ga.vecB = aligned16(d.B) && (d.ldb % 4 == 0);
    if (d.store & ~(DPP_ST_A | DPP_ST_B | DPP_ST_C | DPP_ST_BNX)) return DPP_E_BADARG;
    if (d.precision != 0 && d.precision != 1) return DPP_E_BADARG;
    if (d.precision == 1 && (d.variant == 1 || (d.actA.mode & 4))) return DPP_E_UNSUPPORTED;
    if ((d.store & DPP_ST_A) && (!ga.vecA || (d.actA.mode & 4))) return DPP_E_UNSUPPORTED;
    if ((d.store & DPP_ST_B) && !ga.vecB) return DPP_E_UNSUPPORTED;
    if ((d.store & (DPP_ST_C | DPP_ST_BNX)) && d.splitk != 1) return DPP_E_UNSUPPORTED;
    ga.shA = (d.store & DPP_ST_A) ? 1 : 0;
    ga.shB = (d.store & DPP_ST_B) ? 1 : 0;
    static const bool wide_ok = []() { const char* e = getenv("DPP_GEMM_WIDE_EPILOGUE"); return !(e && e[0] == '0'); }();
    ga.wide = wide_ok && d.splitk == 1 && d.N % 4 == 0 && d.ldc % 4 == 0 && aligned16(d.C) && aligned16(d.residual) &&
              aligned16(d.epi.bn_x) && aligned16(d.bias) && aligned16(d.epi.bn_mean) && aligned16(d.epi.bn_scale) &&
              aligned16(d.epi.bn_beta) && aligned16(d.epi.bn_inv_std);
    if ((d.actA.mode & 2) && !(aligned16(d.actA.mean) && aligned16(d.actA.scale) && aligned16(d.actA.beta))) return DPP_E_BADARG;
    if ((d.actB.mode & 2) && !(aligned16(d.actB.mean) && aligned16(d.actB.scale) && aligned16(d.actB.beta))) return DPP_E_BADARG;
    if ((d.store & (DPP_ST_C | DPP_ST_BNX)) && !ga.wide) return DPP_E_UNSUPPORTED;
    return DPP_OK;
}

}

extern "C" int dpp_abi_version(void) { return DPP_ABI_VERSION; }

extern "C" int dpp_gemm_variant_rows(const dpp_gemm_desc* dp) {
    GemmArgs ga;
    if (gemm_prepare(dp, ga) != DPP_OK) return 0;
    if (ga.d.variant == 2) return ksplit_bn(ga.d, ga) ? 32 : 0;
    if (ga.d.variant == 3) return stream16_rows(ga.d, ga);
    if (ga.d.variant == 4) return dpp_gemm_expand_rows(ga.d, ga);
    return 0;
}

extern "C" int dpp_gemm(const dpp_gemm_desc* dp, dpp_stream_t stream) {
    GemmArgs ga;
    const int prep = gemm_prepare(dp, ga);
    if (prep != DPP_OK) return prep;
    dpp_gemm_desc& d = ga.d;
    const bool red_layout = !d.a_kc && !d.b_kc;
    static const int bk64_min_k = []() { const char* e = getenv("DPP_GEMM_BK64_MINK"); return e ? atoi(e) : 128; }();
    ga.bk = (d.K > 16) ? 32 : 16;
    if (d.a_kc && d.K / d.splitk >= bk64_min_k) ga.bk = 64;
    const int chunk = red_layout ? 64 : ga.bk;
    int kper = dpp_cdiv(d.K, d.splitk);
    ga.Kper = dpp_cdiv(kper, chunk) * chunk;
    int bm = d.bm, bn = d.bn, wm = d.wm;
    if (bm == 0) {
        if (d.M <= 16) { bm = 16; bn = 64; wm = 1; }
        else if (d.M <= 32) { bm = 32; bn = 64; wm = 1; }
        else {
            wm = 4;
            bn = d.N > 32 ? 64 : (d.N > 16 ? 32 : 16);
            long blocks128 = (long)dpp_cdiv(d.M, 128) * dpp_cdiv(d.N, bn) * d.splitk;
            bm = blocks128 >= 512 ? 128 : 64;
        }
    }
    hipStream_t st = static_cast<hipStream_t>(stream);
    if (d.variant == 4) {
        const int rpw = dpp_gemm_expand_rows(d, ga);
        if (!rpw) return DPP_E_UNSUPPORTED;
        return dpp_gemm_expand_launch(ga, rpw, st);
    }
    if (d.precision == 1) {
        if (d.variant == 0 && !red_layout && ga.bk < 32) return DPP_E_UNSUPPORTED;
        return dpp_gemm_dispatch_pb(ga, bm, bn, wm, st);
    }
    return d.store ? dpp_gemm_dispatch_st(ga, bm, bn, wm, st) : gemm_dispatch<false>(ga, bm, bn, wm, st);
}

extern "C" size_t dpp_reduce_job_bytes(void) { return sizeof(ReduceJob); }

extern "C" int dpp_reduce_multi_block_cols(void) { return RM_COLS; }

extern "C" int dpp_reduce_multi(const void* jobs_dev, int njobs, int total_blocks, dpp_stream_t stream) {
    if (!jobs_dev || njobs < 1 || total_blocks < 1) return DPP_E_BADARG;
    DPP_LAUNCH(reduce_multi_kernel, dim3(total_blocks), dim3(DPP_THREADS), 0, static_cast<hipStream_t>(stream),
                       static_cast<const ReduceJob*>(jobs_dev), njobs);
    return dpp_launch_status();
// ... 14 lines not shown
```

### deep-prior-pp_amd/csrc/gemm_expand.hip

```cpp
#include "gemm_args.h"

namespace {

template <int KT, bool BKC, bool IT2, bool ACT, bool RES, bool BNB, bool LZ = false, bool PB = false, bool ST = false>
__global__ __launch_bounds__(DPP_THREADS) DPP_WAVES_PER_EU(1, 2) void gemm_expand_kernel(GemmArgs ga, int rpw) {
    static_assert(!PB || ((KT % 32 == 0 || KT == 16) && !LZ), "bf16 MFMA operands: whole 32-deep steps, or K = 16 with a zero upper half");
    dpp_kernarg_warm<sizeof(GemmArgs)>();
    const dpp_gemm_desc& d = ga.d;
    constexpr int KL = KT / 4, KV = KL / 4;
    constexpr int RT = 2, RI = 16 * RT;
    const int lane = threadIdx.x & 63, l15 = lane & 15, kq = lane >> 4;
    const int NG = d.N >> 6, nblk = d.M / rpw;
    const int gw = blockIdx.x * 4 + (threadIdx.x >> 6);
    if (gw >= NG * nblk) return;
    const int cg = gw % NG, rblk = gw / NG;
    const int n0 = cg * 64 + 4 * l15;
    const int wrow0 = rblk * rpw, iters = rpw / RI;
    const dpp_epilogue& ep = d.epi;
    const int modeA = ACT ? d.actA.mode : 0;
    const bool relu_mask = BNB && ep.bn_relu != 0;
    const bool a16 = ST && !LZ && ga.shA != 0, c16 = ST && (d.store & DPP_ST_C) != 0, x16 = ST && (d.store & DPP_ST_BNX) != 0;
    dpp_stamp(ga.prof, 0);

    float bw[4][KL];
    if (BKC) {
#pragma unroll
        for (int ct = 0; ct < 4; ++ct)
#pragma unroll
            for (int j = 0; j < KV; ++j) {
                const float4 t = *reinterpret_cast<const float4*>(d.B + (size_t)(n0 + ct) * d.ldb + kq * KL + 4 * j);
                bw[ct][4 * j] = t.x; bw[ct][4 * j + 1] = t.y; bw[ct][4 * j + 2] = t.z; bw[ct][4 * j + 3] = t.w;
            }
    } else {
#pragma unroll
        for (int e = 0; e < KL; ++e) {
            const float4 t = *reinterpret_cast<const float4*>(d.B + (size_t)(kq * KL + e) * d.ldb + n0);
            bw[0][e] = t.x; bw[1][e] = t.y; bw[2][e] = t.z; bw[3][e] = t.w;
        }
    }
    constexpr int KS = PB ? (KL + 7) / 8 : 1;
    dpp_bf16x8 bwp[4][KS];
    if (PB) {
#pragma unroll
        for (int ct = 0; ct < 4; ++ct)
#pragma unroll
            for (int ss = 0; ss < KS; ++ss)
#pragma unroll
                for (int q = 0; q < 8; ++q) bwp[ct][ss][q] = (dpp_bf16)(ss * 8 + q < KL ? bw[ct][ss * 8 + q < KL ? ss * 8 + q : 0] : 0.0f);
    }
    struct Regs { float4 a[RT][KV]; float4 a2[RT][LZ ? KV : 1]; float4 res[RT][4]; float4 bx[RT][4]; };
    auto fetch = [&](Regs& g, int it) {
        const int r0 = wrow0 + it * RI;
#pragma unroll
        for (int rt = 0; rt < RT; ++rt) {
            const size_t oa = (size_t)(r0 + rt * 16 + l15) * d.lda + kq * KL;
            if (a16) {
#pragma unroll
                for (int j = 0; j < KV; ++j) g.a[rt][j] = dpp_raw8(d.A + ((oa + 4 * j) >> 1));
            } else {
#pragma unroll
                for (int j = 0; j < KV; ++j) {
                    g.a[rt][j] = *reinterpret_cast<const float4*>(d.A + oa + 4 * j);
                    if (LZ) g.a2[rt][j] = *reinterpret_cast<const float4*>(d.actA.x2 + oa + 4 * j);
                }
            }
        }
#pragma unroll
        for (int rt = 0; rt < RT; ++rt)
#pragma unroll
            for (int r = 0; r < 4; ++r) {
                const size_t o = (size_t)(r0 + rt * 16 + kq * 4 + r) * d.ldc + n0;
                if (RES) g.res[rt][r] = c16 ? dpp_raw8(d.residual + (o >> 1)) : *reinterpret_cast<const float4*>(d.residual + o);
                if (BNB) g.bx[rt][r] = x16 ? dpp_raw8(ep.bn_x + (o >> 1)) : *reinterpret_cast<const float4*>(ep.bn_x + o);
            }
    };
    Regs g0, g1;
    fetch(g0, 0);
    float4 mu[KV], sc[KV], be[KV], ax[LZ ? KV : 1];
#pragma unroll
    for (int j = 0; j < KV; ++j) {
        mu[j] = sc[j] = be[j] = make_float4(0.f, 0.f, 0.f, 0.f);
        if (LZ || (modeA & 2)) {
            mu[j] = *reinterpret_cast<const float4*>(d.actA.mean + kq * KL + 4 * j);
            sc[j] = *reinterpret_cast<const float4*>(d.actA.scale + kq * KL + 4 * j);
            be[j] = *reinterpret_cast<const float4*>(d.actA.beta + kq * KL + 4 * j);
        }
        if (LZ) ax[j] = *reinterpret_cast<const float4*>(d.actA.aux + kq * KL + 4 * j);
    }
    const bool lz_store = LZ && d.actA.out != nullptr && cg == 0;
    float4 cbias = make_float4(0.f, 0.f, 0.f, 0.f), cmean = cbias, cscale = cbias, cbeta = cbias, cistd = cbias;
    if (d.bias) cbias = *reinterpret_cast<const float4*>(d.bias + n0);
    if (BNB) {
        cmean = *reinterpret_cast<const float4*>(ep.bn_mean + n0); cscale = *reinterpret_cast<const float4*>(ep.bn_scale + n0);
        cbeta = *reinterpret_cast<const float4*>(ep.bn_beta + n0); cistd = *reinterpret_cast<const float4*>(ep.bn_inv_std + n0);
    }
    dpp_stamp(ga.prof, 1);

    float sx[4] = {0.f, 0.f, 0.f, 0.f}, sy[4] = {0.f, 0.f, 0.f, 0.f};
    float rmean[4] = {0.f, 0.f, 0.f, 0.f}, rm2[4] = {0.f, 0.f, 0.f, 0.f};
    const bool want_stats = ep.stats != nullptr;
    auto colsum = [&](float (&s)[4]) {
#pragma unroll
        for (int j = 0; j < 4; ++j) { s[j] += __shfl_xor(s[j], 16); s[j] += __shfl_xor(s[j], 32); }
    };

    auto step = [&](Regs& g, int it) {
        const int r0 = wrow0 + it * RI;
        f32x4 acc[RT][4];
#pragma unroll
        for (int rt = 0; rt < RT; ++rt)
#pragma unroll
            for (int ct = 0; ct < 4; ++ct) acc[rt][ct] = (f32x4){0.f, 0.f, 0.f, 0.f};
        dpp_bf16x8 ap[RT][KS];
        if (PB && KL < 8) {
#pragma unroll
            for (int rt = 0; rt < RT; ++rt)
#pragma unroll
                for (int q = 0; q < 8; ++q) ap[rt][0][q] = (dpp_bf16)0.0f;
        }
#pragma unroll
        for (int j = 0; j < KV; ++j) {
            float av[RT][4];
#pragma unroll
            for (int rt = 0; rt < RT; ++rt) {
                float4 v = a16 ? dpp_widen4(g.a[rt][j]) : g.a[rt][j];
                if (LZ) {
                    const float4 x = g.a2[rt][j];
                    v = make_float4(sc[j].x * v.x - ax[j].x * (x.x - mu[j].x) - be[j].x, sc[j].y * v.y - ax[j].y * (x.y - mu[j].y) - be[j].y,
                                    sc[j].z * v.z - ax[j].z * (x.z - mu[j].z) - be[j].z, sc[j].w * v.w - ax[j].w * (x.w - mu[j].w) - be[j].w);
                    if (lz_store) *reinterpret_cast<float4*>(d.actA.out + (size_t)(r0 + rt * 16 + l15) * d.lda + kq * KL + 4 * j) = v;
                }
                if (modeA & 2) {
                    v.x = dpp_fma(v.x - mu[j].x, sc[j].x, be[j].x); v.y = dpp_fma(v.y - mu[j].y, sc[j].y, be[j].y);
                    v.z = dpp_fma(v.z - mu[j].z, sc[j].z, be[j].z); v.w = dpp_fma(v.w - mu[j].w, sc[j].w, be[j].w);
                }
                if (modeA & 1) { v.x = fmaxf(v.x, 0.f); v.y = fmaxf(v.y, 0.f); v.z = fmaxf(v.z, 0.f); v.w = fmaxf(v.w, 0.f); }
                av[rt][0] = v.x; av[rt][1] = v.y; av[rt][2] = v.z; av[rt][3] = v.w;
                if (PB) {
#pragma unroll
                    for (int t = 0; t < 4; ++t) ap[rt][j / 2][(j & 1) * 4 + t] = (dpp_bf16)av[rt][t];
                }
            }
            if (PB) {
                if ((j & 1) || KL < 8) {
#pragma unroll
                    for (int rt = 0; rt < RT; ++rt)
#pragma unroll
                        for (int ct = 0; ct < 4; ++ct)
                            acc[rt][ct] = __builtin_amdgcn_mfma_f32_16x16x32_bf16(ap[rt][j / 2], bwp[ct][j / 2], acc[rt][ct], 0, 0, 0);
                }
            } else {
#pragma unroll
                for (int t = 0; t < 4; ++t)
#pragma unroll
                    for (int rt = 0; rt < RT; ++rt)
#pragma unroll
                        for (int ct = 0; ct < 4; ++ct)
                            acc[rt][ct] = __builtin_amdgcn_mfma_f32_16x16x4f32(av[rt][t], bw[ct][4 * j + t], acc[rt][ct], 0, 0, 0);
            }
        }
        float vals[RT][4][4];
#pragma unroll
        for (int rt = 0; rt < RT; ++rt)
#pragma unroll
            for (int r = 0; r < 4; ++r) {
                float v[4] = {acc[rt][0][r] + cbias.x, acc[rt][1][r] + cbias.y, acc[rt][2][r] + cbias.z, acc[rt][3][r] + cbias.w};
                if (RES) {
                    const float4 rr = c16 ? dpp_widen4(g.res[rt][r]) : g.res[rt][r];
                    v[0] += rr.x; v[1] += rr.y; v[2] += rr.z; v[3] += rr.w;
                }
// ... 19 lines not shown
#pragma unroll
                for (int j = 0; j < 4; ++j) vals[rt][r][j] = v[j];
            }
        if (want_stats) {
            float sm[4] = {0.f, 0.f, 0.f, 0.f}, m2[4] = {0.f, 0.f, 0.f, 0.f};
#pragma unroll
            for (int rt = 0; rt < RT; ++rt)
#pragma unroll
                for (int r = 0; r < 4; ++r)
#pragma unroll
                    for (int j = 0; j < 4; ++j) sm[j] += vals[rt][r][j];
            colsum(sm);
#pragma unroll
            for (int j = 0; j < 4; ++j) sm[j] *= 1.0f / (float)RI;
#pragma unroll
            for (int rt = 0; rt < RT; ++rt)
#pragma unroll
                for (int r = 0; r < 4; ++r)
#pragma unroll
                    for (int j = 0; j < 4; ++j) { const float dv = vals[rt][r][j] - sm[j]; m2[j] += dv * dv; }
            colsum(m2);
            if (it == 0) {
#pragma unroll
                for (int j = 0; j < 4; ++j) { rmean[j] = sm[j]; rm2[j] = m2[j]; }
            } else {
                const float na = (float)(it * RI), nb = (float)RI, nn = na + nb;
#pragma unroll
                for (int j = 0; j < 4; ++j) {
                    const float dl = sm[j] - rmean[j];
                    rmean[j] += dl * (nb / nn);
                    rm2[j] += m2[j] + dl * dl * (na * nb / nn);
                }
            }
        }
    };

    if (IT2) {
        for (int it = 0; it < iters; it += 2) {
            if (it + 1 < iters) fetch(g1, it + 1);
            DPP_SCHED_FENCE();
            step(g0, it);
            if (it + 1 < iters) {
                if (it + 2 < iters) fetch(g0, it + 2);
                DPP_SCHED_FENCE();
                step(g1, it + 1);
            }
        }
    } else {
        DPP_SCHED_FENCE();
        step(g0, 0);
    }
    dpp_stamp(ga.prof, 3);
    if (BNB && ep.bn_partial != nullptr) {
        float tx[4] = {sx[0], sx[1], sx[2], sx[3]}, ty[4] = {sy[0], sy[1], sy[2], sy[3]};
        colsum(tx);
        colsum(ty);
        if (kq == 0) {
#pragma unroll
            for (int j = 0; j < 4; ++j) {
                ep.bn_partial[dpp_partial_index(0, n0 + j, rblk, d.N, nblk)] = tx[j];
                ep.bn_partial[dpp_partial_index(1, n0 + j, rblk, d.N, nblk)] = ty[j];
            }
        }
    }
    if (want_stats && kq == 0) {
#pragma unroll
        for (int j = 0; j < 4; ++j) {
            ep.stats[dpp_partial_index(0, n0 + j, rblk, d.N, nblk)] = rmean[j];
            ep.stats[dpp_partial_index(1, n0 + j, rblk, d.N, nblk)] = rm2[j];
        }
    }
    dpp_stamp(ga.prof, 4);
}

}

int dpp_gemm_expand_rows(const dpp_gemm_desc& d, const GemmArgs& ga) {
    if ((d.store & DPP_ST_B) || (d.store && (d.actA.mode & 4))) return 0;
    if (!d.a_kc || d.splitk != 1 || !d.C || !ga.vecA || !ga.vecB || !ga.wide) return 0;
    if (d.K != 16 && d.K != 32 && d.K != 64) return 0;
    if (d.N % 64 || d.M % 32) return 0;
    if (d.mapA.s != 1 || d.mapB.s != 1 || d.mapC.s != 1 || d.actB.mode != 0) return 0;
    if (d.actA.mode != 0 && d.actA.cmod < d.K) return 0;
    if (d.epi.stats && d.epi.bn_x) return 0;
    if (d.b_kc ? (d.epi.bn_x != nullptr || (d.actA.mode & 4)) : (d.actA.mode != 0 && d.actA.mode != 4)) return 0;
    if (d.actA.mode == 4 && d.actA.out && d.lda != d.K) return 0;
    if (d.precision != 0 && (d.precision != 1 || (d.actA.mode & 4))) return 0;
    int rpw = d.bm;
    if (rpw <= 0) rpw = d.M >= 65536 ? 128 : (d.M >= 16384 ? 64 : 32);
    if (rpw % 32 || d.M % rpw) return 0;
    return rpw;
}

namespace {

template <int KT>
int launch_expand(const GemmArgs& ga, int rpw, hipStream_t st) {
    const dpp_gemm_desc& d = ga.d;
    const int waves = (d.M / rpw) * (d.N / 64);
    const dim3 grid(dpp_cdiv(waves, 4));
    const bool it2 = rpw > 32, act = d.actA.mode != 0, res = d.residual != nullptr, bnb = d.epi.bn_x != nullptr, lz = d.actA.mode == 4;
    const bool pb = d.precision == 1;
    const bool stg = d.store != 0;
#define DPP_EXS(K_, I_, A_, R_, B_, L_, P_, S_) DPP_LAUNCH((gemm_expand_kernel<KT, K_, I_, A_, R_, B_, L_, P_, S_>), grid, dim3(DPP_THREADS), 0, st, ga, rpw)
#define DPP_EX(K_, I_, A_, R_, B_, L_, P_) do { if (!(L_) && stg) DPP_EXS(K_, I_, A_, R_, B_, L_, P_, !(L_)); else DPP_EXS(K_, I_, A_, R_, B_, L_, P_, false); } while (0)
#define DPP_EX_P(K_, I_, A_, R_, B_) do { if (pb) { DPP_EX(K_, I_, A_, R_, B_, false, true); break; } \
                                          DPP_EX(K_, I_, A_, R_, B_, false, false); } while (0)
#define DPP_EX_I(K_, A_, R_, B_, L_) do { if (L_) { if (it2) DPP_EX(K_, true, A_, R_, B_, true, false); else DPP_EX(K_, false, A_, R_, B_, true, false); } \
                                          else if (it2) DPP_EX_P(K_, true, A_, R_, B_); else DPP_EX_P(K_, false, A_, R_, B_); } while (0)
#define DPP_EX_R(K_, A_, B_, L_) do { if (res) DPP_EX_I(K_, A_, true, B_, L_); else DPP_EX_I(K_, A_, false, B_, L_); } while (0)
    if (d.b_kc) {
        if (act) DPP_EX_R(true, true, false, false); else DPP_EX_R(true, false, false, false);
    } else if (lz) {
        if (bnb) DPP_EX_R(false, false, true, true); else DPP_EX_R(false, false, false, true);
    } else {
        if (bnb) DPP_EX_R(false, false, true, false); else DPP_EX_R(false, false, false, false);
    }
#undef DPP_EX_P
#undef DPP_EXS
#undef DPP_EX_R
#undef DPP_EX_I
#undef DPP_EX
    return dpp_launch_status();
}

}

int dpp_gemm_expand_launch(const GemmArgs& ga, int rpw, hipStream_t st) {
    const dpp_gemm_desc& d = ga.d;
    return d.K == 64 ? launch_expand<64>(ga, rpw, st) : (d.K == 32 ? launch_expand<32>(ga, rpw, st) : launch_expand<16>(ga, rpw, st));
}
```

### deep-prior-pp_amd/hipdp/engine.py

```python
import os
from ctypes import c_int as C_int

import numpy as np

from . import evalfuse, layout, ops
from . import heuristics as hz
from .lib import Act, RowMap
from .ops import Plan
from .runtime import default_runtime
from .backward import BackwardMixin
from .store import BNState, ParamStore, TensorV, View, _collect, _dedupe_specs, _layer_kind, _pad4, _param_specs, bf16_bits_to_f32, get_store


class CompiledNet(BackwardMixin):
    def __init__(self, net, train=False, runtime=None, loss=None, weight_decay=0.0, dp=None, fuse_bn=True, bf16=None, optimizer=None,
                 fuse_blocks=None):
        self.rt = rt = runtime or default_runtime()
        self.optimizer = dict(optimizer) if optimizer else dict(name='ADAM')
        self.prec = int(bool(hz.BF16_DEFAULT if bf16 is None else bf16))
        self.store16 = self.grad16 = False
        self.dp = dp
        self.fuse_bn = bool(fuse_bn) and not (dp is not None and dp.sync_bn)
        self.net, self.train = net, train
        self.N = net.cfgParams.batch_size
# ... 228 lines not shown
        return v

    def _emit_concat(self, var):
        parts = [self._emit(p) for p in var.inputs]
        if any(p.base.is16 for p in parts):
            raise NotImplementedError("concatenation of bf16-stored maps")
        N = parts[0].shape[0]
        widths = [int(p.shape[1]) for p in parts]
        total = sum(widths)
        cat = self._new_tensor((N, total), 'concat')
        cat.concat_parts = []
        off = 0
        for p, w in zip(parts, widths):
            if p.bn is not None or len(p.shape) != 2 or int(np.prod(p.base.shape[1:])) != w:
                raise NotImplementedError("concatenation of anything but flattened (ReLU) maps")
            self.fwd.add(ops.copy2d(self.rt, p.base.buf, w, cat.buf.view(off, (N * total - off,)), total, N, w, relu=p.relu,
                                    name='concat_pack'))
            cat.concat_parts.append((p, off, w))
            off += w
        return View(cat)

    def _split_concat_grad(self, cat):
        N, total = cat.shape
        for p, off, w in cat.concat_parts:
            if p.base in self.x_ins:
                continue
            tgt, dst = self._view_grad(p)
            if tgt.grad_written:
                raise NotImplementedError("concatenated value with another consumer")
            self.bwd.add(ops.copy2d(self.rt, cat.grad.view(off, (N * total - off,)), total, dst, w, N, w, name='concat_split'))
            tgt.grad_written = True

    def _emit_add(self, var):
        a, b = var.inputs
        if self.fuse_blocks:
            fused = evalfuse.emit_block(self, var)
            if fused is not None:
                return fused

        def fusable(x):
            return x.kind == 'layer' and _layer_kind(x.layer) in ('ConvLayer',) and self._single_consumer(x) \
                and x.layer.cfgParams.activation is None

        cand = [x for x in (a, b) if fusable(x)]
        if not cand:
            raise NotImplementedError("residual add whose operands are not conv outputs")
        q = max(cand, key=lambda x: (self._depth(x) if hz.SIDE_SHORTCUT else 0, x.layer.layerNum))
        p = b if q is a else a
        beside = hz.SIDE_SHORTCUT and self.train and p in cand and id(p) not in self._memo
        if beside:
            self._emit(p.inputs[0])
            n0 = len(self.fwd.ops)
        pv = self._emit(p)
        if not pv.plain:
            raise NotImplementedError("residual add on a non-materialised operand")
        if beside:
            moved = list(self.fwd.ops[n0:])
            if all(isinstance(op, ops.Launch) for op, _ in moved):
                fork = ops.Fork()
                self.fwd.ops[n0:] = [(fork, False)] + [(op, True) for op, _ in moved]
                self.fwd.uses_side = True
                self._emit(q.inputs[0])
                self.fwd.join()
                self._beside.append(([id(fork), id(self.fwd.ops[-1][0])], [id(op) for op, _ in moved]))
        if p.kind == 'layer' and p.layer.layerNum > q.layer.layerNum:
            self._bwd_after[id(p.layer)] = q.layer
        out = self._emit(q, residual=pv.base, out_var=var)
        self._memo[id(q)] = out
        return out

    def _depth(self, var):
        memo = self.__dict__.setdefault('_depth_memo', {})
        if id(var) not in memo:
            d = max([self._depth(i) for i in getattr(var, 'inputs', None) or []] or [0])
            memo[id(var)] = d + (1 if var.kind == 'layer' else 0)
        return memo[id(var)]

    def _feeds_batchnorm(self, var):
        for c in self.consumers.get(id(var), []):
            if c.kind == 'layer' and _layer_kind(c.layer) == 'BatchNormLayer':
                return True
        return False

    def _emit_layer(self, var, residual, out_var=None):
        layer = var.layer
        kind = _layer_kind(layer)
        rt, st = self.rt, self.store
        src = self._emit(var.inputs[0])
        if kind == 'BatchNormLayer':
            if not src.plain:
                raise NotImplementedError("BatchNorm on a non-materialised input")
            C = src.base.C
            M = src.base.rows
            sync = self.train and self.dp is not None and self.dp.sync_bn
            b = BNState(layer, C, M, self.dp.world if sync else 1)
            b.mean, b.inv_std, b.scale = (rt.alloc(_pad4(C)) for _ in range(3))
            b.beta_buf, b.gamma_buf = st.view(layer.beta), st.view(layer.gamma)
            b.run_mean, b.run_inv_std = st.view(layer.mean), st.view(layer.inv_std)
            self.bn_states[id(layer)] = b
            fused = getattr(src.base, 'stats', None) if self.train else None
            if fused is not None:
                part, nblk, rows = fused
                self.fwd.add(ops.bn_finalize(rt, part, nblk, M, rows, C, b.gamma_buf, layer.cfgParams.epsilon, b.mean, b.inv_std,
                                             b.scale, b.run_mean, b.run_inv_std, layer.cfgParams.alpha))
            elif self.train:
                W = b.world
                part = self.scratch(b.nb * 2 * C * (W + 1)).view(0, (b.nb * 2 * C,))
                self.fwd.add(ops.bn_stats_partial(rt, src.base.buf, M, C, b.rpb, part))
                if W > 1:
                    allp = self.scratch(b.nb * 2 * C * (W + 1)).view(b.nb * 2 * C, (W * b.nb * 2 * C,))
                    self.fwd.add(self.dp.all_gather_op(part, allp, 'bn_stats_allgather'))
                    part = allp
                self.fwd.add(ops.bn_finalize(rt, part, b.nb, M * W, b.rpb, C, b.gamma_buf, layer.cfgParams.epsilon, b.mean, b.inv_std,
                                             b.scale, b.run_mean, b.run_inv_std, layer.cfgParams.alpha, nseg=W))
            elif hz.EVAL_FUSE:
                self._bn_eval_jobs.append((b.gamma_buf, b.run_mean, b.run_inv_std, C, b.mean, b.inv_std, b.scale))
            else:
                self.fwd.add(ops.bn_eval_coeffs(rt, b.gamma_buf, b.run_mean, b.run_inv_std, C, b.mean, b.inv_std, b.scale))
            v = View(src.base, b, False, shape=src.shape, chan=src.chan)
            v.var = var
            return v
        if kind == 'NonlinearityLayer':
            if layer.cfgParams.activation is None:
                return src
            if layer.cfgParams.activation_str != 'ReLU':
                raise NotImplementedError("only ReLU is on the hot path")
            v = View(src.base, src.bn, True, shape=src.shape, chan=src.chan)
            v.var = var
            return v
        if kind == 'ConvPoolLayer':
            return self._emit_stem(layer, src, out_var if out_var is not None else var)
        if kind == 'ConvLayer':
            return self._emit_conv(layer, src, residual, out_var if out_var is not None else var)
        if kind == 'HiddenLayer':
            return self._emit_fc(layer, src)
        if kind == 'DropoutLayer':
            return self._emit_dropout(layer, src)
        raise NotImplementedError(kind)

    def _emit_stem(self, layer, src, out_var=None):
        c = layer.cfgParams
        N, H, W, Ci = src.base.shape
        ok = (src.base is self.x_in and Ci == 1 and tuple(c.filterDim) == (5, 5) and c.border_mode == 'half' and
              tuple(c.poolsize) == (2, 2) and tuple(c.stride) == (1, 1) and c.activation is None and c.nFilters <= 32)
        if not ok:
            return self._emit_convpool(layer, src)
        Co = c.nFilters
        out = self._new_tensor((N, H // 2, W // 2, Co), 'stem', act=True)
        arg = self.rt.alloc((N, H // 2, W // 2, Co), np.uint8, zero=False) if self.train else None
        stats = None
        if self.train and self.fuse_bn and H % 16 == 0 and W % 16 == 0 and out_var is not None and self._feeds_batchnorm(out_var):
            nblk = N * (H // 16) * (W // 16)
            out.stats = (self.rt.alloc((nblk, 2, Co), zero=False), nblk, 64)
            stats = out.stats[0]
        self.fwd.add(ops.stem_fwd(self.rt, src.base.buf.reshape(N, H, W), N, H, W, self.store.view(layer.W), self.store.view(layer.b), Co,
                                  out.buf, arg, stats))
        self.layer_io[id(layer)] = dict(in_view=src, out=out, argmax=arg, stem=True)
        return View(out)

    def _emit_convpool(self, layer, src):
        c = layer.cfgParams
        N, H, W, Ci = src.base.shape
        kh, kw = c.filterDim[0], c.filterDim[1]
        if len(src.shape) != 4:
            raise NotImplementedError("ConvPoolLayer on a flattened input")
        if self.store16:
            raise NotImplementedError("bf16 storage is built for the ResNet path (stem + ConvLayer); the generic ConvPoolLayer kernels are f32")
        if c.border_mode not in ('valid', 'half') or tuple(c.stride) != (1, 1) or c.poolsize[0] != c.poolsize[1]:
            raise NotImplementedError("ConvPoolLayer border %s stride %s pool %s" % (c.border_mode, c.stride, c.poolsize))
        if c.border_mode == 'half' and (kh % 2 == 0 or kw % 2 == 0):
            raise NotImplementedError("'half' padding with an even filter size")
        pad = kh // 2 if c.border_mode == 'half' else 0
        if c.border_mode == 'half' and kh != kw:
            raise NotImplementedError("'half' padding with a non-square filter")
        pool, Co = int(c.poolsize[0]), c.nFilters
        _, Co_, Hp, Wp = c.outputDim
        assert Co_ == Co
        out = self._new_tensor((N, Hp, Wp, Co), 'convpool%d' % layer.layerNum)
        ties = self.rt.alloc((N, Hp, Wp, Co), np.uint16, zero=False) if (self.train and pool > 1) else None
        geom = dict(N=N, H=H, W=W, Ci=Ci, kh=kh, kw=kw, pad=pad, Co=Co, pool=pool, Hp=Hp, Wp=Wp)
        self.fwd.add(ops.convpool_fwd(self.rt, src.base.buf, N, H, W, Ci, self.store.view(layer.W), kh, kw, pad, Co, pool,
                                      self.store.view(layer.b), out.buf, ties, actX=self._act(src), name='convpool_%d' % layer.layerNum))
        self.layer_io[id(layer)] = dict(in_view=src, out=out, ties=ties, geom=geom, stem=False)
        return View(out)

    def _emit_conv(self, layer, src, residual, out_var=None):
        c = layer.cfgParams
        N, Hi, Wi, Ci = src.base.shape
        _, Co, Ho, Wo = c.outputDim
        k, s = tuple(c.filterDim), tuple(c.stride)
        if c.border_mode != 'half' or k not in ((1, 1), (3, 3)) or s[0] != s[1] or (k == (3, 3) and s != (1, 1)):
            raise NotImplementedError("ConvLayer %s stride %s border %s" % (k, s, c.border_mode))
        out = self._new_tensor((N, Ho, Wo, Co), 'conv%d' % layer.layerNum, act=True)
        act = self._act(src)
        rt, st = self.rt, self.store
        res = residual.buf if residual is not None else None
        want_stats = self.train and self.fuse_bn and out_var is not None and self._feeds_batchnorm(out_var)
        M = N * Ho * Wo
        epi = None
        if k == (1, 1):
            tile, _ = hz.gemm_plan(M, Co, Ci, allow_split=False)
            rs = hz.rowstream_plan(M, Co, Ci, True)
            if rs is not None:
                tile = rs
            ks = hz.ksplit_plan(M, Co, Ci) if (s[0] == 1 and rs is None) else None
            if ks is not None:
                tile = ks
            ex = hz.expand_plan(M, Co, Ci, True) if (s[0] == 1 and rs is None and ks is None) else None
            s16 = hz.stream16_plan(M, Co, Ci, True) if (s[0] == 1 and rs is None and ks is None and ex is None) else None
            if s16 is not None:
                tile = s16
            if ex is not None:
                tile = ex
            mp = RowMap.strided(s[0], Ho, Wo, Hi, Wi) if s[0] != 1 else None
            variant = 1 if rs is not None else (2 if ks is not None else (4 if ex is not None else (3 if s16 is not None else 0)))

            def build(tile, variant, epi):
                return ops.gemm(rt, src.base.buf, st.view(layer.W), out.buf, M, Co, Ci, 1, 1, Ci, Ci, Co, mapA=mp, actA=act,
                                bias=st.view(layer.b), residual=res, tile=tile, epi=epi, variant=variant,
                                name='conv1x1_%d' % layer.layerNum, precision=self._gemm_prec(variant, Ci))
            if variant in (2, 3, 4) and ops.gemm_variant_rows(rt, build(tile, variant, None)) != tile[0]:
                variant, (tile, _) = 0, hz.gemm_plan(M, Co, Ci, allow_split=False)
            if want_stats:
                nblk = -(-M // tile[0])
                out.stats = (rt.alloc((nblk, 2, Co), zero=False), nblk, tile[0])
                epi = ops.epilogue(stats=out.stats[0])
            self.fwd.add(build(tile, variant, epi))
        elif self._conv3_stream(N, Hi, Wi, Ci, Co, src.base.buf, out.buf) and residual is None:
            rows = rt.lib.dpp_conv3x3_stream_rows(N, Hi, Wi, Ci)
            if want_stats:
                out.stats = (rt.alloc((M // rows, 2, Co), zero=False), M // rows, rows)
                epi = ops.epilogue(stats=out.stats[0])
            self.fwd.add(ops.conv3x3_stream(rt, src.base.buf, N, Hi, Wi, Ci, st.view(layer.W), out.buf, actX=act, bias=st.view(layer.b), epi=epi,
                                            name='conv3x3_%d' % layer.layerNum))
        else:
            bm = hz.conv3x3_bm(M, Co, hw=(Hi, Wi), prec=self.prec)
            if want_stats:
                th, tw, img = (C_int() for _ in range(3))
                nblk = rt.lib.dpp_conv3x3_tiling(N, Hi, Wi, bm, th, tw, img)
                if Hi % th.value == 0 and Wi % tw.value == 0 and (N % img.value == 0 or nblk == 1):
                    out.stats = (rt.alloc((nblk, 2, Co), zero=False), nblk, bm)
                    epi = ops.epilogue(stats=out.stats[0])
            self.fwd.add(ops.conv3x3(rt, src.base.buf, N, Hi, Wi, Ci, st.view(layer.W), Co, out.buf, actX=act, bias=st.view(layer.b),
                                     residual=res, bm=bm, epi=epi, name='conv3x3_%d' % layer.layerNum, precision=self.prec))
        self.layer_io[id(layer)] = dict(in_view=src, out=out, residual=residual)
        return View(out)

    def _conv3_stream(self, N, H, W, Ci, Co, *bufs):
        if Ci != Co or Ci not in hz.CONV3_STREAM_C or self.prec:
            return False
        if any(b is not None and b.dtype == ops.BF16 for b in bufs):
            return False
        return self.rt.lib.dpp_conv3x3_stream_rows(N, H, W, Ci) > 0

    def _emit_fc(self, layer, src):
        c = layer.cfgParams
        if len(src.shape) != 2:
            raise NotImplementedError("HiddenLayer on a non-flattened input")
        Nb, K = src.shape
        Nout = c.outputDim[1]
        assert K == c.inputDim[1], (K, c.inputDim)
        out = self._new_tensor((Nb, Nout), 'fc%d' % layer.layerNum)
        rt, st = self.rt, self.store
        act = self._act(src)
        if self._fc1_stream(Nb, K, Nout):
            splitk = max(1, min(hz.FC1_SLICES, K // 512))
            part = self.scratch(splitk * Nb * Nout)
            self.fwd.add(ops.fc_gemm(rt, src.base.buf, st.view(layer.W), None, Nb, Nout, K, 1, 0, K, Nout, Nout, actA=act, splitk=splitk,
                                     partial=part, precision=self.prec, kchunk=hz.FC1_KCHUNK, name='fc_%d' % layer.layerNum))
            self.fwd.add(ops.reduce_partials(rt, part, splitk, Nb * Nout, out.buf, bias=st.view(layer.b), nbias=Nout))
            self.layer_io[id(layer)] = dict(in_view=src, out=out)
            return View(out)
        tile, splitk = hz.gemm_plan(Nb, Nout, K)
        if K >= 4096 and Nb <= 128 and Nout >= 64:
            tile, splitk = ((128, 64, 4) if Nb > 64 and hz.knob('DPP_FC1_TILE128', '1') != '0' else (64, 64, 4)), max(1, K // 512)
        act = self._act(src)
        if splitk > 1:
            part = self.scratch(splitk * Nb * Nout)
            self.fwd.add(ops.gemm(rt, src.base.buf, st.view(layer.W), None, Nb, Nout, K, 1, 0, K, Nout, Nout, actA=act, splitk=splitk,
                                  partial=part, tile=tile, name='fc_%d' % layer.layerNum))
            red = self.fwd.add(ops.reduce_partials(rt, part, splitk, Nb * Nout, out.buf, bias=st.view(layer.b), nbias=Nout))
            self._loss_fusable = (red, dict(partial=part, nz=splitk, bias=st.view(layer.b), out=out.buf))
        else:
            self.fwd.add(ops.gemm(rt, src.base.buf, st.view(layer.W), out.buf, Nb, Nout, K, 1, 0, K, Nout, Nout, actA=act,
                                  bias=st.view(layer.b), tile=tile, name='fc_%d' % layer.layerNum))
        self.layer_io[id(layer)] = dict(in_view=src, out=out)
        return View(out)

    def _emit_dropout(self, layer, src):
        if src.bn is not None or len(src.shape) != 2:
            raise NotImplementedError("DropoutLayer after BatchNorm / on a 4-D map")
        n = int(np.prod(src.shape))
        out = self._new_tensor(src.shape, 'drop%d' % layer.layerNum)
        keep = np.float32(1.0 - layer.cfgParams.p)
        mask = None
        if self.train:
            mask = self.rt.alloc(src.shape)
            self.dropout_masks[id(layer)] = (mask, float(keep), layer.mask_seed)
            rank = self.dp.rank if self.dp is not None else 0
            self.fwd.add(ops.bernoulli_mask(self.rt, mask, n, float(keep), layer.mask_seed, (layer.layerNum << 40) + (rank << 32), self.step_ctr))
        self.fwd.add(ops.scale(self.rt, src.base.buf, out.buf, n, a=keep, relu=src.relu, mask=mask))
        self.layer_io[id(layer)] = dict(in_view=src, out=out, mask=mask)
        return View(out)

    def set_input(self, x):
        xs = x if isinstance(x, (list, tuple)) else [x]
        if len(xs) != len(self.x_ins):
            raise ValueError("the net takes %d inputs, got %d" % (len(self.x_ins), len(xs)))
        for t, a in zip(self.x_ins, xs):
            a = np.asarray(a, np.float32)
            want = (t.shape[0], t.shape[3], t.shape[1], t.shape[2])
            if tuple(a.shape) != want:
                raise ValueError("input shape %s, expected %s" % (a.shape, want))
            t.buf.set(a if a.shape[1] == 1 else layout.nchw_to_nhwc(a))

    def forward(self, x=None):
        self.store.check_live()
        if x is not None:
            self.set_input(x)
# ... 143 lines not shown
```

### deep-prior-pp_amd/hipdp/heuristics.py

```python
import os

def knob(name, default):
    if os.environ.get('DPP_EXPERIMENT', '0') != '1':
        return default
    return os.environ.get(name, default)


BN_RPB_TARGET_BLOCKS = int(knob('DPP_BN_BLOCKS', '1024'))
BN_BWD_FUSE_MAX_BLOCKS = int(knob('DPP_BN_BWD_FUSE_NB', '0'))
BN_BWD_FUSE_TARGET_WGS = int(knob('DPP_BN_BWD_FUSE_WGS', '512'))



GEMM_TARGET_BLOCKS = int(knob('DPP_GEMM_TARGET_BLOCKS', '1024'))


def gemm_plan(M, N, K, allow_split=True):
    if M <= 16:
        bm, bn, wm = 16, 64, 1
    elif M <= 32:
        bm, bn, wm = 32, 64, 1
    else:
        wm = 4
        cands = [(128, 64), (64, 64), (128, 32), (64, 32), (128, 16), (64, 16)]
        if knob('DPP_NO_128x64', '1') != '0':
            cands = cands[1:]
        cands = [(a, b) for (a, b) in cands if b <= max(16, 16 * (-(-N // 16))) or b == 16]
        bm, bn = cands[-1]
        for (a, b) in cands:
            if (-(-M // a)) * (-(-N // b)) >= GEMM_TARGET_BLOCKS:
                bm, bn = a, b
                break
    tiles = (-(-M // bm)) * (-(-N // bn))
    splitk = 1
    if allow_split and tiles < 512 and K >= 256:
        splitk = int(min(max(1, 2048 // tiles), max(1, K // 128), 256))
    return (bm, bn, wm), splitk


EVAL_FUSE = knob('DPP_EVAL_FUSE', '1') != '0'
FUSE_LOSS = knob('DPP_FUSE_LOSS', '1') != '0'
ADAM_TICKED = knob('DPP_ADAM_TICKED', '1') != '0'
EVAL_FUSE_BF16 = knob('DPP_EVAL_FUSE_BF16', '1') != '0'
OVERLAP_ALLREDUCE = knob('DPP_OVERLAP_ALLREDUCE', '1') != '0'
EARLY_BUCKET_MIN = int(knob('DPP_EARLY_BUCKET_MIN', str(1 << 22)))
LAZY_BN_BWD = int(knob('DPP_LAZY_BN_BWD', '0'))
BF16_DEFAULT = os.environ.get('DPP_BF16', '0') == '1'
BF16_STORE = knob('DPP_BF16_STORE', '1') != '0'
BF16_GRADS = knob('DPP_BF16_GRADS', '1') != '0'
BF16_GEMM = knob('DPP_BF16_GEMM', '1') != '0'
BF16_GEMM_ALL = knob('DPP_BF16_GEMM_ALL', '1') != '0'
BF16_GEMM_ROLES = tuple(knob('DPP_BF16_GEMM_ROLES', 'fwd,dgrad,wgrad').split(','))
BF16_GEMM_VARIANTS = tuple(knob('DPP_BF16_GEMM_VARIANTS', '0,2,3').split(','))
BF16_WGRAD3 = knob('DPP_BF16_WGRAD3', '1') != '0'
EARLY_ADAM = knob('DPP_EARLY_ADAM', '0') != '0'
EARLY_REDUCE_BYTES = int(knob('DPP_EARLY_REDUCE_MB', '0')) << 20
TAIL_REDUCE = knob('DPP_TAIL_REDUCE', '0') != '0'
FC1_STREAM = knob('DPP_FC1_STREAM', 'auto')
FC1_WGRAD_STREAM = knob('DPP_FC1_WGRAD_STREAM', '1') != '0'
FC1_WGRAD_DEFER = int(knob('DPP_FC1_WGRAD_DEFER', '0'))
FC1_KCHUNK = int(knob('DPP_FC1_KCHUNK', '0'))
FC1_SLICES = int(knob('DPP_FC1_SLICES', '32'))
FC1_MIN_K = int(knob('DPP_FC1_MIN_K', '4096'))


def is_fc1_shape(Nb, K, Nout):
    return K >= FC1_MIN_K and Nout >= 64 and Nout % 4 == 0 and K % 4 == 0
ROWSTREAM = knob('DPP_ROWSTREAM', '0') != '0'

def rowstream_plan(M, N, K, b_kc):
    if not ROWSTREAM or M < 2048:
        return None
    K16 = (K + 15) // 16 * 16
    for bn in (64, 32, 16):
        if bn > 16 and bn >= 2 * N:
            continue
        lds = (bn * (K16 + 4) if b_kc else K16 * (bn + 4)) * 4
        if lds > 48 * 1024:
            continue
        bm = 128 if (M // 128) * (-(-N // bn)) >= 1024 else 64
        return (bm, bn, 4)
    return None


KSPLIT = int(knob('DPP_KSPLIT', '2'))
KSPLIT_MAX_M = int(knob('DPP_KSPLIT_MAX_M', '65536'))


def ksplit_plan(M, N, K):
    if KSPLIT <= 0 or M % 32 or M > KSPLIT_MAX_M * (2 if K == 128 else 1):
        return None
    if K == 256 and N % 64 == 0:
        return (32, 64, 4)
# ... 97 lines not shown
```

### deep-prior-pp_amd/hipdp/lib.py

```python
import ctypes as C
import os

_HERE = os.path.dirname(os.path.abspath(__file__))
DEFAULT_LIB = os.path.join(os.path.dirname(_HERE), 'lib', 'libdpp_hip.so')

ABI_VERSION = 13
ST_A, ST_B, ST_C, ST_BNX = 1, 2, 4, 8
c_float_p = C.c_void_p
stream_t = C.c_void_p


class RowMap(C.Structure):
    _fields_ = [('s', C.c_int), ('Wo', C.c_int), ('HoWo', C.c_int), ('Wi', C.c_int), ('HiWi', C.c_int)]

    @staticmethod
    def identity():
        return RowMap(1, 0, 0, 0, 0)

    @staticmethod
    def strided(s, Ho, Wo, Hi, Wi):
        return RowMap(s, Wo, Ho * Wo, Wi, Hi * Wi)


class Act(C.Structure):
    _fields_ = [('mean', C.c_void_p), ('scale', C.c_void_p), ('beta', C.c_void_p), ('mode', C.c_int), ('cmod', C.c_int),
                ('x2', C.c_void_p), ('aux', C.c_void_p), ('out', C.c_void_p)]

    NONE, RELU, BN, BN_RELU, BN_BWD = 0, 1, 2, 3, 4

    @staticmethod
    def none():
        return Act(None, None, None, 0, 1, None, None, None)


class Epilogue(C.Structure):
    _fields_ = [('stats', C.c_void_p), ('bn_x', C.c_void_p), ('bn_mean', C.c_void_p), ('bn_inv_std', C.c_void_p),
                ('bn_scale', C.c_void_p), ('bn_beta', C.c_void_p), ('bn_relu', C.c_int), ('pad_', C.c_int),
                ('bn_partial', C.c_void_p)]


class GemmDesc(C.Structure):
    _fields_ = [('A', C.c_void_p), ('lda', C.c_int), ('a_kc', C.c_int), ('mapA', RowMap), ('actA', Act),
                ('B', C.c_void_p), ('ldb', C.c_int), ('b_kc', C.c_int), ('mapB', RowMap), ('actB', Act),
                ('C', C.c_void_p), ('ldc', C.c_int), ('mapC', RowMap),
                ('bias', C.c_void_p), ('residual', C.c_void_p),
                ('M', C.c_int), ('N', C.c_int), ('K', C.c_int),
                ('splitk', C.c_int), ('partial', C.c_void_p),
                ('bm', C.c_int), ('bn', C.c_int), ('wm', C.c_int), ('variant', C.c_int), ('epi', Epilogue), ('store', C.c_int), ('precision', C.c_int)]


class BnEval(C.Structure):
    _fields_ = [('mean', C.c_void_p), ('inv_std', C.c_void_p), ('gamma', C.c_void_p), ('beta', C.c_void_p)]


class ResblockDesc(C.Structure):
    _fields_ = [('X', C.c_void_p), ('N', C.c_int), ('H', C.c_int), ('W', C.c_int), ('Cin', C.c_int),
                ('stride', C.c_int), ('Ho', C.c_int), ('Wo', C.c_int), ('Cout', C.c_int), ('Nb', C.c_int),
                ('bn0', BnEval), ('bn1', BnEval), ('bn2', BnEval),
                ('W1', C.c_void_p), ('b1', C.c_void_p), ('W2', C.c_void_p), ('b2', C.c_void_p), ('W3', C.c_void_p), ('b3', C.c_void_p),
                ('Wsc', C.c_void_p), ('bsc', C.c_void_p), ('Y', C.c_void_p), ('store', C.c_int)]


SIGNATURES = {
    'dpp_abi_version': (C.c_int, []),
    'dpp_gemm': (C.c_int, [C.POINTER(GemmDesc), stream_t]),
    'dpp_gemm_variant_rows': (C.c_int, [C.POINTER(GemmDesc)]),
    'dpp_fc_gemm': (C.c_int, [C.POINTER(GemmDesc), C.c_int, C.c_int, stream_t]),
    'dpp_reduce_partials': (C.c_int, [C.c_void_p, C.c_int, C.c_int, C.c_void_p, C.c_int, C.c_void_p, stream_t]),
    'dpp_conv3x3': (C.c_int, [C.c_void_p, C.c_int, C.c_int, C.c_int, C.c_int, C.POINTER(Act), C.c_void_p, C.c_int,
                              C.c_void_p, C.c_void_p, C.c_void_p, C.c_int, C.POINTER(Epilogue), C.c_int, stream_t]),
    'dpp_conv3x3_bf16': (C.c_int, [C.c_void_p, C.c_int, C.c_int, C.c_int, C.c_int, C.POINTER(Act), C.c_void_p, C.c_int,
                                   C.c_void_p, C.c_void_p, C.c_void_p, C.c_int, C.POINTER(Epilogue), C.c_int, stream_t]),
    'dpp_conv3x3_tiling': (C.c_int, [C.c_int, C.c_int, C.c_int, C.c_int, C.POINTER(C.c_int), C.POINTER(C.c_int), C.POINTER(C.c_int)]),
    'dpp_conv3x3_stream_rows': (C.c_int, [C.c_int, C.c_int, C.c_int, C.c_int]),
    'dpp_conv3x3_stream': (C.c_int, [C.c_void_p, C.c_int, C.c_int, C.c_int, C.c_int, C.POINTER(Act), C.c_void_p, C.c_void_p, C.c_void_p,
                                     C.POINTER(Epilogue), stream_t]),
    'dpp_conv3x3_wtrans': (C.c_int, [C.c_void_p, C.c_int, C.c_int, C.c_void_p, stream_t]),
    'dpp_conv3x3_wgrad_blocks': (C.c_int, [C.c_int, C.c_int, C.c_int, C.c_int, C.c_int, C.c_int]),
    'dpp_conv3x3_wgrad': (C.c_int, [C.c_void_p, C.c_int, C.c_int, C.c_int, C.c_int, C.POINTER(Act), C.c_void_p, C.c_int,
                                    C.c_void_p, C.c_int, C.c_int, stream_t]),
    'dpp_conv3x3_wgrad_bf16': (C.c_int, [C.c_void_p, C.c_int, C.c_int, C.c_int, C.c_int, C.POINTER(Act), C.c_void_p, C.c_int,
                                    C.c_void_p, C.c_int, C.c_int, stream_t]),
    'dpp_conv3x3_wgrad_bf16_ok': (C.c_int, [C.c_int, C.c_int, C.c_int, C.c_int, C.c_int]),
    'dpp_stem_fwd': (C.c_int, [C.c_void_p, C.c_int, C.c_int, C.c_int, C.c_void_p, C.c_void_p, C.c_int, C.c_void_p,
                               C.c_void_p, C.c_void_p, C.c_int, stream_t]),
    'dpp_stem_wgrad_blocks': (C.c_int, [C.c_int, C.c_int, C.c_int, C.c_int]),
    'dpp_stem_wgrad': (C.c_int, [C.c_void_p, C.c_int, C.c_int, C.c_int, C.c_void_p, C.c_void_p, C.c_int, C.c_void_p,
                                 C.c_int, stream_t]),
    'dpp_convpool_fwd': (C.c_int, [C.c_void_p, C.c_int, C.c_int, C.c_int, C.c_int, C.c_void_p, C.c_void_p, C.c_int, C.c_int,
                                   C.c_int, C.c_int, C.c_int, C.c_void_p, C.c_void_p, C.c_void_p, stream_t]),
    'dpp_convpool_wgrad_blocks': (C.c_int, [C.c_int, C.c_int, C.c_int]),
    'dpp_convpool_wgrad': (C.c_int, [C.c_void_p, C.c_int, C.c_int, C.c_int, C.c_int, C.c_void_p, C.c_void_p, C.c_void_p, C.c_int,
                                     C.c_int, C.c_int, C.c_int, C.c_int, C.c_void_p, stream_t]),
    'dpp_convpool_dgrad': (C.c_int, [C.c_void_p, C.c_void_p, C.c_int, C.c_int, C.c_int, C.c_int, C.c_void_p, C.c_int, C.c_int,
                                     C.c_int, C.c_int, C.c_int, C.c_void_p, stream_t]),
    'dpp_bn_stats_partial': (C.c_int, [C.c_void_p, C.c_int, C.c_int, C.c_int, C.c_void_p, C.c_int, stream_t]),
    'dpp_bn_finalize': (C.c_int, [C.c_void_p, C.c_int, C.c_int, C.c_int, C.c_int, C.c_int, C.c_void_p, C.c_float, C.c_void_p,
                                  C.c_void_p, C.c_void_p, C.c_void_p, C.c_void_p, C.c_float, stream_t]),
    'dpp_bn_eval_coeffs': (C.c_int, [C.c_void_p, C.c_void_p, C.c_void_p, C.c_int, C.c_void_p, C.c_void_p, C.c_void_p,
                                     stream_t]),
    'dpp_bn_eval_job_bytes': (C.c_size_t, []),
    'dpp_bn_eval_coeffs_multi': (C.c_int, [C.c_void_p, C.c_int, C.c_int, stream_t]),
    'dpp_resblock_eval_ok': (C.c_int, [C.c_int] * 5),
    'dpp_resblock_eval': (C.c_int, [C.POINTER(ResblockDesc), stream_t]),
    'dpp_resblock_eval_check': (C.c_int, [C.POINTER(ResblockDesc)]),
    'dpp_bn_bwd_reduce': (C.c_int, [C.c_void_p, C.c_void_p, C.c_int, C.c_int, C.c_void_p, C.c_void_p, C.c_void_p,
                                    C.c_void_p, C.c_int, C.c_void_p, C.c_int, C.c_void_p, C.c_int, stream_t]),
    'dpp_bn_bwd_finalize': (C.c_int, [C.c_void_p, C.c_int, C.c_int, C.c_int, C.c_int, C.c_void_p, C.c_void_p, C.c_void_p,
                                      C.c_void_p, C.c_void_p, C.c_void_p, C.c_void_p, C.c_void_p, stream_t]),
    'dpp_bn_bwd_finalize_apply_ok': (C.c_int, [C.c_int, C.c_int, C.c_int]),
    'dpp_bn_bwd_finalize_apply': (C.c_int, [C.c_void_p, C.c_void_p, C.c_int, C.c_int, C.c_void_p, C.c_void_p, C.c_void_p, C.c_void_p, C.c_int,
                                            C.c_void_p, C.c_void_p, C.c_int, C.c_void_p, C.c_void_p, C.c_void_p, C.c_int, stream_t]),
    'dpp_bn_bwd_apply': (C.c_int, [C.c_void_p, C.c_void_p, C.c_int, C.c_int, C.c_void_p, C.c_void_p, C.c_void_p,
                                   C.c_void_p, C.c_void_p, C.c_void_p, C.c_void_p, C.c_int, C.c_void_p, C.c_int, stream_t]),
    'dpp_reduce_job_bytes': (C.c_size_t, []),
    'dpp_reduce_multi_block_cols': (C.c_int, []),
    'dpp_reduce_multi': (C.c_int, [C.c_void_p, C.c_int, C.c_int, stream_t]),
    'dpp_colsum_partial': (C.c_int, [C.c_void_p, C.c_int, C.c_int, C.c_int, C.c_void_p, stream_t]),
    'dpp_wgrad_stream_slices': (C.c_int, [C.c_int, C.c_int, C.c_int, C.c_int]),
    'dpp_wgrad_stream': (C.c_int, [C.c_void_p, C.c_int, C.c_void_p, C.c_int, C.c_void_p, C.c_void_p, C.c_int, C.c_int, C.c_void_p, C.c_int, stream_t]),
    'dpp_fc_wgrad_stream_ok': (C.c_int, [C.c_int, C.c_int, C.c_int]),
    'dpp_fc_wgrad_stream': (C.c_int, [C.c_void_p, C.c_void_p, C.c_void_p, C.c_int, C.c_int, C.c_int, C.c_void_p, C.c_int, stream_t]),
    'dpp_wgrad_stream_bf16': (C.c_int, [C.c_void_p, C.c_int, C.c_void_p, C.c_int, C.c_void_p, C.c_void_p, C.c_int, C.c_int, C.c_void_p, C.c_int, stream_t]),
    'dpp_wgrad_stream_bf16_ok': (C.c_int, [C.c_int, C.c_int]),
    'dpp_wgrad3_stream_slices': (C.c_int, [C.c_int] * 6),
    'dpp_wgrad3_stream': (C.c_int, [C.c_void_p, C.c_int, C.c_void_p, C.c_int, C.c_int, C.c_int, C.c_int, C.c_void_p, C.c_int, C.c_void_p, C.c_int, stream_t]),
    'dpp_wtrans_job_bytes': (C.c_size_t, []),
    'dpp_conv3x3_wtrans_multi': (C.c_int, [C.c_void_p, C.c_int, C.c_int, stream_t]),
    'dpp_loss_sse': (C.c_int, [C.c_void_p, C.c_void_p, C.c_int, C.c_int, C.c_int, C.c_void_p, C.c_void_p, stream_t]),
    'dpp_reduce_partials_loss': (C.c_int, [C.c_void_p, C.c_int, C.c_int, C.c_int, C.c_void_p, C.c_void_p, C.c_void_p, C.c_int, C.c_void_p, C.c_void_p, stream_t]),
    'dpp_loss_sse_bcast': (C.c_int, [C.c_void_p, C.c_void_p, C.c_int, C.c_void_p, C.c_void_p, C.c_void_p, stream_t]),
    'dpp_error_l2': (C.c_int, [C.c_void_p, C.c_void_p, C.c_int, C.c_int, C.c_void_p, stream_t]),
    'dpp_adam': (C.c_int, [C.c_void_p, C.c_void_p, C.c_void_p, C.c_void_p, C.c_size_t, C.c_void_p, stream_t]),
    'dpp_adam_ticked': (C.c_int, [C.c_void_p, C.c_void_p, C.c_void_p, C.c_void_p, C.c_size_t, C.c_void_p, stream_t]),
    'dpp_adam_tick': (C.c_int, [C.c_void_p, stream_t]),
    'dpp_counter_add': (C.c_int, [C.c_void_p, C.c_ulonglong, stream_t]),
    'dpp_axpy': (C.c_int, [C.c_void_p, C.c_void_p, C.c_float, C.c_size_t, stream_t]),
    'dpp_sumsq': (C.c_int, [C.c_void_p, C.c_size_t, C.c_float, C.c_void_p, C.c_int, stream_t]),
    'dpp_sumsq_multi_workspace_bytes': (C.c_size_t, []),
    'dpp_sumsq_multi': (C.c_int, [C.c_void_p, C.c_void_p, C.c_int, C.c_float, C.c_void_p, C.c_void_p, C.c_int, stream_t]),
    'dpp_axpy_multi': (C.c_int, [C.c_void_p, C.c_void_p, C.c_void_p, C.c_int, C.c_float, stream_t]),
    'dpp_scale': (C.c_int, [C.c_void_p, C.c_void_p, C.c_float, C.c_int, C.c_void_p, C.c_size_t, stream_t]),
    'dpp_relu_bwd': (C.c_int, [C.c_void_p, C.c_void_p, C.c_void_p, C.c_float, C.c_void_p, C.c_size_t, stream_t]),
    'dpp_fill_zero': (C.c_int, [C.c_void_p, C.c_size_t, stream_t]),
    'dpp_copy2d': (C.c_int, [C.c_void_p, C.c_int, C.c_void_p, C.c_int, C.c_int, C.c_int, C.c_int, stream_t]),
    'dpp_rowscale': (C.c_int, [C.c_void_p, C.c_void_p, C.c_int, C.c_int, C.c_float, C.c_void_p, C.c_int, C.c_int, stream_t]),
    'dpp_crop_center': (C.c_int, [C.c_void_p, C.c_int, C.c_int, C.c_int, C.c_void_p, C.c_int, C.c_int, stream_t]),
    'dpp_bernoulli_mask': (C.c_int, [C.c_void_p, C.c_size_t, C.c_float, C.c_ulonglong, C.c_ulonglong, C.c_void_p, stream_t]),
    'dpp_augment_record_bytes': (C.c_size_t, []),
    'dpp_augment_prepare': (C.c_int, [C.c_void_p] * 5 + [C.c_int] * 3 + [C.c_void_p] * 5 + [C.c_int, C.c_ulonglong,
                                      C.c_ulonglong, C.c_double, C.c_double, C.c_double, C.c_double, C.c_double,
                                      C.c_double, C.c_double, C.c_int, C.c_int, C.c_void_p, C.c_void_p, C.c_int, C.c_void_p,
                                      C.c_void_p, C.c_void_p, C.c_void_p, stream_t]),
    'dpp_augment_warp': (C.c_int, [C.c_void_p, C.c_void_p, C.c_int, C.c_int, C.c_void_p, stream_t]),
    'dpp_augment': (C.c_int, [C.c_void_p] * 5 + [C.c_int] * 3 + [C.c_void_p] * 5 + [C.c_int, C.c_ulonglong,
                              C.c_ulonglong, C.c_double, C.c_double, C.c_double, C.c_double, C.c_double,
                              C.c_double, C.c_double, C.c_int, C.c_int, C.c_void_p, C.c_void_p, C.c_int, C.c_void_p,
                              C.c_void_p, C.c_void_p, C.c_void_p, C.c_void_p, C.c_void_p, C.c_ulonglong, C.c_ulonglong, C.c_int,
                              stream_t]),
    'dpp_crop_record_bytes': (C.c_size_t, []),
    'dpp_crop_prepare': (C.c_int, [C.c_void_p, C.c_int, C.c_int, C.c_int, C.c_void_p, C.c_void_p, C.c_double, C.c_double, C.c_int, C.c_int,
                                   C.c_void_p, C.c_void_p, stream_t]),
    'dpp_crop_com_workspace_bytes': (C.c_size_t, [C.c_int]),
    'dpp_crop_com': (C.c_int, [C.c_void_p, C.c_void_p, C.c_int, C.c_int, C.c_int, C.c_void_p, C.c_void_p, stream_t]),
    'dpp_crop_warp': (C.c_int, [C.c_void_p, C.c_void_p, C.c_int, C.c_int, C.c_int, C.c_int, C.c_int, C.c_float, C.c_void_p, stream_t]),
    'dpp_crop_warp_ex': (C.c_int, [C.c_void_p, C.c_void_p, C.c_int, C.c_int, C.c_int, C.c_int, C.c_int, C.c_float, C.c_float, C.c_float,
                                   C.c_void_p, stream_t]),
    'dpp_resize_crops': (C.c_int, [C.c_void_p, C.c_int, C.c_int, C.c_int, C.c_int, C.c_int, C.c_int, C.c_float, C.c_void_p, stream_t]),
    'dpp_recrop': (C.c_int, [C.c_void_p, C.c_int, C.c_int, C.c_int, C.c_void_p, C.c_void_p, C.c_int, C.c_int, C.c_float, C.c_double, C.c_int,
                             C.c_void_p, C.c_void_p, stream_t]),
    'dpp_inverse_crop': (C.c_int, [C.c_void_p, C.c_int, C.c_int, C.c_int, C.c_void_p, C.c_void_p, C.c_int, C.c_int, C.c_int, C.c_float, C.c_float,
                                   C.c_int, C.c_void_p, stream_t]),
    'dpp_crop_refine': (C.c_int, [C.c_void_p, C.c_void_p, C.c_int, C.c_int, C.c_int, C.c_void_p, C.c_void_p, C.c_void_p, C.c_double, C.c_double,
                                  C.c_double, C.c_double, C.c_int, C.c_void_p, C.c_int, C.c_void_p, C.c_void_p, C.c_int, C.c_void_p, C.c_void_p,
                                  C.c_void_p, C.c_void_p, stream_t]),
    'dpp_frame_range_bytes': (C.c_size_t, [C.c_int]),
    'dpp_frame_range': (C.c_int, [C.c_void_p, C.c_int, C.c_int, C.c_int, C.c_void_p, stream_t]),
    'dpp_crop_prepare_ranged': (C.c_int, [C.c_void_p, C.c_int, C.c_void_p, C.c_void_p, C.c_double, C.c_double, C.c_int, C.c_int, C.c_void_p,
                                          C.c_void_p, stream_t]),
    'dpp_track_refine': (C.c_int, [C.c_void_p, C.c_void_p, C.c_int, C.c_int, C.c_int, C.c_void_p, C.c_void_p, C.c_void_p] + [C.c_double] * 4 +
                         [C.c_int, C.c_double, C.c_double, C.c_int] + [C.c_void_p] * 5 + [stream_t]),
# ... 58 lines not shown
```

### deep-prior-pp_amd/hipdp/ops.py

```python
import ctypes as C
import os

import numpy as np

from .lib import ST_A, ST_B, ST_BNX, ST_C, Act, BnEval, DppError, Epilogue, GemmDesc, ResblockDesc, RowMap, check


class Launch(object):
    __slots__ = ('fn', 'args', 'keep', 'name', 'meta', 'kernels')

    def __init__(self, fn, args, keep, name, meta=None, kernels=1):
        self.fn, self.args, self.keep, self.name, self.meta = fn, args, keep, name, meta
        self.kernels = kernels

    def __call__(self, stream):
        st = self.fn(*self.args, stream)
        if st != 0:
            check(st, self.name)


class Fork(object):
    name = 'fork'
    meta = None

# ... 119 lines not shown
        return [o for (o, _) in self.ops if not isinstance(o, (Fork, Join))]

    def _compile(self, rt):
        key = (id(rt), LAUNCH_MODE, id(self._ops), self._ops.version)
        if self._compiled is not None and self._compiled[0] == key:
            return self._compiled[1]
        segs, cur = [], []
        for op, side in self.ops:
            if isinstance(op, (Launch, Fork, Join)):
                cur.append((op, side))
            else:
                if cur:
                    segs.append(NativePlan(rt, cur, LAUNCH_MODE))
                    cur = []
                segs.append(op)
        if cur:
            segs.append(NativePlan(rt, cur, LAUNCH_MODE))
        self._compiled = (key, segs)
        return segs

    def segment_counts(self):
        native, host, open_ = 0, 0, False
        for op, _ in self.ops:
            if isinstance(op, (Launch, Fork, Join)):
                if not open_:
                    native, open_ = native + 1, True
            else:
                host, open_ = host + 1, False
        return native, host

    def run(self, rt_or_stream):
        rt = rt_or_stream if hasattr(rt_or_stream, 'stream') else None
        if rt is not None and LAUNCH_MODE != 'python':
            for seg in self._compile(rt):
                if isinstance(seg, NativePlan):
                    seg.run(rt)
                else:
                    seg(rt.stream)
            return
        if rt is None or not self.uses_side or not getattr(rt, 'has_side_stream', False):
            st = rt.stream if rt is not None else rt_or_stream
            for op, _ in self.ops:
                if not isinstance(op, (Fork, Join)):
                    op(st)
            return
        main, side = rt.stream, rt.side_stream
        for op, on_side in self.ops:
            if isinstance(op, Fork):
                rt.side_wait_main()
            elif isinstance(op, Join):
                rt.main_wait_side()
            else:
                op(side if on_side else main)

    def __len__(self):
        return len(self.launches())


def _p(buf):
    return None if buf is None else buf.ptr


BF16 = np.dtype(np.uint16)


def _is16(buf):
    return buf is not None and getattr(buf, 'dtype', None) == BF16


def _store(a=None, b=None, c=None, bnx=None):
    return (ST_A if _is16(a) else 0) | (ST_B if _is16(b) else 0) | (ST_C if _is16(c) else 0) | (ST_BNX if _is16(bnx) else 0)


def _esz(buf):
    return 2.0 if _is16(buf) else 4.0


def act(mode=0, mean=None, scale=None, beta=None, cmod=1, x2=None, aux=None, out=None):
    a = Act(_p(mean), _p(scale), _p(beta), int(mode), int(cmod), _p(x2), _p(aux), _p(out))
    a._keep = (mean, scale, beta, x2, aux, out)
    return a


def act_bn_bwd(bn, q, p, x, C, out=None):
    return act(Act.BN_BWD, mean=bn.mean, scale=bn.scale, beta=q, cmod=C, x2=x, aux=p, out=out)


def epilogue(stats=None, bn=None, bn_x=None, bn_relu=True, bn_partial=None):
    e = Epilogue()
    e.stats = _p(stats)
    if bn is not None:
        e.bn_x, e.bn_mean, e.bn_inv_std, e.bn_scale, e.bn_beta = bn_x.ptr, bn.mean.ptr, bn.inv_std.ptr, bn.scale.ptr, bn.beta_buf.ptr
        e.bn_relu, e.bn_partial = int(bn_relu), bn_partial.ptr
    e._bn_x = bn_x
    e._keep = (stats, bn, bn_x, bn_partial)
    return e


def gemm(rt, A, B, Cbuf, M, N, K, a_kc, b_kc, lda, ldb, ldc=0, mapA=None, mapB=None, mapC=None, actA=None, actB=None,
         bias=None, residual=None, splitk=1, partial=None, tile=(0, 0, 0), epi=None, variant=0, name='gemm', precision=0):
    d = GemmDesc()
    d.A, d.lda, d.a_kc = A.ptr, lda, int(a_kc)
    d.mapA = mapA or RowMap.identity()
    d.actA = actA or Act.none()
    d.B, d.ldb, d.b_kc = B.ptr, ldb, int(b_kc)
    d.mapB = mapB or RowMap.identity()
    d.actB = actB or Act.none()
    d.C, d.ldc = _p(Cbuf), ldc
    d.mapC = mapC or RowMap.identity()
    d.bias, d.residual = _p(bias), _p(residual)
    d.M, d.N, d.K = int(M), int(N), int(K)
    d.splitk, d.partial = int(splitk), _p(partial)
    d.bm, d.bn, d.wm = tile
    d.variant = int(variant)
    if epi is not None:
        d.epi = epi
    if _is16(residual) != _is16(Cbuf) and residual is not None and Cbuf is not None:
        raise ValueError("dpp_gemm: C and residual must be stored alike")
    d.store = _store(A, B, Cbuf, getattr(epi, '_bn_x', None) if epi is not None else None)
    d.precision = int(precision)
    meta = dict(kernel='gemm_mfma_bf16' if precision else 'gemm_mfma_f32', flops=2.0 * M * N * K,
                bytes=_esz(A) * M * K + _esz(B) * K * N + (4.0 * M * N * max(1, splitk) if splitk > 1 else _esz(Cbuf) * M * N) +
                (_esz(residual) * M * N if residual is not None else 0))
    return Launch(rt.lib.dpp_gemm, (C.byref(d),), (d, A, B, Cbuf, bias, residual, partial, actA, actB, epi), name, meta)


def gemm_variant_rows(rt, launch):
    return int(rt.lib.dpp_gemm_variant_rows(C.byref(launch.keep[0])))


def wgrad_stream(rt, dY, Co, X, Ci, M, rows_per_wave, partial, mapX=None, actX=None, name='wgrad_stream', precision=0):
    nsl = rt.lib.dpp_wgrad_stream_slices(Co, Ci, M, rows_per_wave)
    meta = dict(kernel='gemm_mfma_bf16' if precision else 'gemm_mfma_f32', flops=2.0 * M * Co * Ci,
                bytes=_esz(dY) * M * Co + 4.0 * nsl * Co * Ci + _esz(X) * M * Ci)
    return Launch(rt.lib.dpp_wgrad_stream_bf16 if precision else rt.lib.dpp_wgrad_stream, (dY.ptr, int(Co), X.ptr, int(Ci), C.byref(mapX) if mapX is not None else None, _actp(actX), int(M),
                                            int(rows_per_wave), partial.ptr, _store(a=dY, b=X)), (dY, X, partial, mapX, actX), name, meta)


def wgrad3_stream(rt, dY, Co, X, Ci, N, H, W, rows_per_wave, partial, actX=None, name='conv3x3_wgrad_stream'):
    nsl = rt.lib.dpp_wgrad3_stream_slices(Co, Ci, N, H, W, rows_per_wave)
    px = float(N) * H * W
    meta = dict(kernel='conv3x3_wgrad_mfma_f32', flops=2.0 * px * 9 * Ci * Co, bytes=4.0 * (px * Co + nsl * 9.0 * Ci * Co) + _esz(X) * px * Ci)
    return Launch(rt.lib.dpp_wgrad3_stream, (dY.ptr, int(Co), X.ptr, int(Ci), int(N), int(H), int(W), _actp(actX), int(rows_per_wave),
                                             partial.ptr, _store(a=dY, b=X)), (dY, X, partial, actX), name, meta)


def fc_gemm(rt, A, B, Cbuf, M, N, K, a_kc, b_kc, lda, ldb, ldc=0, actA=None, actB=None, bias=None, residual=None, splitk=1, partial=None,
            precision=0, kchunk=0, name='fc_gemm'):
    d = GemmDesc()
    d.A, d.lda, d.a_kc = A.ptr, lda, int(a_kc)
    d.mapA, d.mapB, d.mapC = RowMap.identity(), RowMap.identity(), RowMap.identity()
    d.actA = actA or Act.none()
    d.B, d.ldb, d.b_kc = B.ptr, ldb, int(b_kc)
    d.actB = actB or Act.none()
    d.C, d.ldc = _p(Cbuf), ldc
    d.bias, d.residual = _p(bias), _p(residual)
    d.M, d.N, d.K = int(M), int(N), int(K)
    d.splitk, d.partial = int(splitk), _p(partial)
    d.store = _store(A, B, Cbuf)
    if _is16(residual) != _is16(Cbuf) and residual is not None and Cbuf is not None:
        raise ValueError("dpp_fc_gemm: C and residual must be stored alike")
    meta = dict(kernel='fc_gemm_mfma_bf16' if precision else 'gemm_mfma_f32', flops=2.0 * M * N * K,
                bytes=4.0 * (M * K + K * N + M * N * (max(1, splitk) if splitk > 1 else 1) + (M * N if residual is not None else 0)))
    return Launch(rt.lib.dpp_fc_gemm, (C.byref(d), int(precision), int(kchunk)), (d, A, B, Cbuf, bias, residual, partial, actA, actB), name, meta)


# ... 448 lines not shown
```

### include/dpp_hip.h

```cpp
#ifndef DPP_HIP_H
#define DPP_HIP_H

#include <stddef.h>
#include <stdint.h>

#ifdef __cplusplus
extern "C" {
#endif

typedef void* dpp_stream_t;

#define DPP_OK 0
#define DPP_E_BADARG 10001
#define DPP_E_UNSUPPORTED 10002

#define DPP_ABI_VERSION 13
int dpp_abi_version(void);

#define DPP_ST_A 1
#define DPP_ST_B 2
#define DPP_ST_C 4
#define DPP_ST_BNX 8

typedef struct {
    int s, Wo, HoWo, Wi, HiWi;
} dpp_rowmap;

typedef struct {
    const float* mean;
    const float* scale;
    const float* beta;
    int mode;
    int cmod;
    const float* x2;
    const float* aux;
    float* out;
} dpp_act;

typedef struct {
    float* stats;
    const float* bn_x;
    const float* bn_mean;
    const float* bn_inv_std;
    const float* bn_scale;
    const float* bn_beta;
    int bn_relu;
    int pad_;
    float* bn_partial;
} dpp_epilogue;

typedef struct {
    const float* A; int lda; int a_kc; dpp_rowmap mapA; dpp_act actA;
    const float* B; int ldb; int b_kc; dpp_rowmap mapB; dpp_act actB;
    float* C; int ldc; dpp_rowmap mapC;
    const float* bias;
    const float* residual;
    int M, N, K;
    int splitk;
    float* partial;
    int bm, bn, wm;
    int variant;
    dpp_epilogue epi;
    int store;
    int precision;
} dpp_gemm_desc;
int dpp_gemm(const dpp_gemm_desc* d, dpp_stream_t stream);
int dpp_gemm_variant_rows(const dpp_gemm_desc* d);

int dpp_wgrad_stream_slices(int Co, int Ci, int M, int rows_per_wave);
int dpp_wgrad_stream(const float* dY, int Co, const float* X, int Ci, const dpp_rowmap* mapX, const dpp_act* actX, int M,
                     int rows_per_wave, float* partial, int store , dpp_stream_t stream);
int dpp_wgrad_stream_bf16_ok(int Co, int Ci);
int dpp_wgrad_stream_bf16(const float* dY, int Co, const float* X, int Ci, const dpp_rowmap* mapX, const dpp_act* actX, int M,
                     int rows_per_wave, float* partial, int store , dpp_stream_t stream);

int dpp_fc_wgrad_stream_ok(int Nb, int K, int N);
int dpp_fc_wgrad_stream(const float* X, const float* dY, float* dW, int Nb, int K, int N, const dpp_act* actX,
                        int store , dpp_stream_t stream);
int dpp_wgrad3_stream_slices(int Co, int Ci, int N, int H, int W, int rows_per_wave);
int dpp_wgrad3_stream(const float* dY, int Co, const float* X, int Ci, int N, int H, int W, const dpp_act* actX, int rows_per_wave,
                      float* partial, int store , dpp_stream_t stream);

int dpp_fc_gemm(const dpp_gemm_desc* d, int precision, int kchunk, dpp_stream_t stream);

int dpp_reduce_partials(const float* partial, int nz, int n, const float* bias, int nbias, float* out,
                        dpp_stream_t stream);


size_t dpp_reduce_job_bytes(void);
int dpp_reduce_multi_block_cols(void);
int dpp_reduce_multi(const void* jobs_dev, int njobs, int total_blocks, dpp_stream_t stream);

int dpp_conv3x3(const float* X, int N, int H, int W, int Ci, const dpp_act* act, const float* Wk, int Co,
                const float* bias, const float* residual, float* Y, int bm, const dpp_epilogue* epi,
                int store , dpp_stream_t stream);
int dpp_conv3x3_bf16(const float* X, int N, int H, int W, int Ci, const dpp_act* act, const float* Wk, int Co,
                     const float* bias, const float* residual, float* Y, int bm, const dpp_epilogue* epi, int store, dpp_stream_t stream);
int dpp_conv3x3_stream_rows(int N, int H, int W, int C);
int dpp_conv3x3_stream(const float* X, int N, int H, int W, int C, const dpp_act* act, const float* Wk, const float* bias, float* Y,
                       const dpp_epilogue* epi, dpp_stream_t stream);
int dpp_conv3x3_tiling(int N, int H, int W, int bm, int* th, int* tw, int* img);
int dpp_conv3x3_wtrans(const float* Wk, int Co, int Ci, float* Wd, dpp_stream_t stream);
size_t dpp_wtrans_job_bytes(void);
int dpp_conv3x3_wtrans_multi(const void* jobs_dev, int njobs, int total_blocks, dpp_stream_t stream);
int dpp_conv3x3_wgrad_blocks(int N, int H, int W, int Ci, int Co, int bm);
int dpp_conv3x3_wgrad(const float* X, int N, int H, int W, int Ci, const dpp_act* act, const float* dY, int Co,
                      float* partial, int bm, int store , dpp_stream_t stream);
int dpp_conv3x3_wgrad_bf16_ok(int N, int H, int W, int Ci, int Co);
int dpp_conv3x3_wgrad_bf16(const float* X, int N, int H, int W, int Ci, const dpp_act* act, const float* dY, int Co,
                           float* partial, int bm, int store , dpp_stream_t stream);

int dpp_stem_fwd(const float* X, int N, int H, int W, const float* Wk, const float* bias, int Co, float* Y, uint8_t* argmax,
                 float* stats, int store , dpp_stream_t stream);
int dpp_stem_wgrad_blocks(int N, int H, int W, int tiles_per_block);
int dpp_stem_wgrad(const float* X, int N, int H, int W, const float* dY, const uint8_t* argmax, int Co, float* partial,
                   int tiles_per_block, dpp_stream_t stream);

int dpp_convpool_fwd(const float* X, int N, int H, int W, int Ci, const dpp_act* act, const float* Wk, int kh, int kw, int pad,
                     int Co, int pool, const float* bias, float* Y, uint16_t* ties, dpp_stream_t stream);
int dpp_convpool_wgrad_blocks(int N, int Hp, int Wp);
// ... 154 lines not shown
```

Measured before the change: 37770 depth-crops/sec.

## Fold BN finalize into consuming conv's prologue, computing coefficients from partials

Instead of launching a separate batch-norm finalize kernel, the conv3x3 kernel (and the variant-4 1x1 GEMM path) can reduce the per-block BN partial sums itself. Each block recomputes mean and scale in its prologue, overlapped with the first halo load, and one writer block stores the coefficients and running stats. The engine defers the finalize when a BN output has a single conv consumer and the partials are small, and falls back to a flush otherwise. This removes a kernel launch and a dependency per BN layer. In exchange every block repeats the partial reduction, uses extra LDS and registers, and adds a __syncthreads in staging.

```diff
diff --git a/deep-prior-pp_amd/csrc/bn.hip b/deep-prior-pp_amd/csrc/bn.hip
--- a/deep-prior-pp_amd/csrc/bn.hip
+++ b/deep-prior-pp_amd/csrc/bn.hip
@@ -53,14 +53,9 @@
     }
 }
 
-__device__ __forceinline__ double wave_allsum(double v) {
-    for (int o = 1; o < DPP_WAVE; o <<= 1) v += __shfl_xor(v, o);
-    return v;
-}
-
 template <int WPC>
 __device__ __forceinline__ double group_allsum(double v, double* slot) {
-    v = wave_allsum(v);
+    v = dpp_wave_allsum(v);
     if (WPC == 1) return v;
     const int wave = threadIdx.x >> 6;
     if ((threadIdx.x & 63) == 0) slot[wave] = v;
@@ -88,41 +83,16 @@
     const bool one_sweep = nseg == 1 && nbs <= GT * U;
     float pm0[U], pq0[U];
     if (one_sweep) {
-        const float* pm_row = partial + dpp_partial_index(0, cc, 0, C, nbs);
-        const float* pq_row = partial + dpp_partial_index(1, cc, 0, C, nbs);
-        const float K = pm_row[0];
-#pragma unroll
-        for (int u = 0; u < U; ++u) {
-            const int b = lane + u * GT;
-            const int bb = b < nbs ? b : nbs - 1;
-            pm0[u] = pm_row[bb];
-            pq0[u] = pq_row[bb];
-        }
-        double s1 = 0.0, s2 = 0.0;
-#pragma unroll
-        for (int u = 0; u < U; ++u) {
-            const int b = lane + u * GT;
-            if (b < nbs) {
-                const double d = (double)pm0[u] - (double)K, nb_ = (double)rows_of(b);
-                s1 += nb_ * d;
-                s2 += (double)pq0[u] + nb_ * d * d;
-            }
-        }
+        float K;
+        dpp_bn_sweep_load<U, GT>(partial + dpp_partial_index(0, cc, 0, C, nbs), partial + dpp_partial_index(1, cc, 0, C, nbs), nbs, lane, K, pm0, pq0);
+        double s1, s2;
+        dpp_bn_sweep_sums<U, GT>(K, pm0, pq0, nbs, rpb, Mseg, lane, s1, s2);
         s1 = group_allsum<WPC>(s1, slot_a);
         s2 = group_allsum<WPC>(s2, slot_b);
         if (lane != 0 || c >= C) return;
-        const double mean1 = (double)K + s1 / (double)M;
-        const double var1 = (s2 - s1 * s1 / (double)M) / (double)M;
-        const float meanf = (float)mean1;
-        const float inv_std = (float)(1.0 / sqrt((var1 > 0.0 ? var1 : 0.0) + (double)eps));
-        mean_o[c] = meanf;
-        inv_std_o[c] = inv_std;
-        scale_o[c] = gam * inv_std;
-        if (upd) {
-            const float oma = 1.0f - alpha;
-            run_mean[c] = oma * rm_old + alpha * meanf;
-            run_inv_std[c] = oma * ri_old + alpha * inv_std;
-        }
+        float meanf, inv_std;
+        dpp_bn_sweep_finish(K, s1, s2, M, eps, meanf, inv_std);
+        dpp_bn_coef_store(c, meanf, inv_std, gam, mean_o, inv_std_o, scale_o, upd, alpha, rm_old, ri_old, run_mean, run_inv_std);
         return;
     }
     double snm = 0.0;
@@ -494,6 +464,11 @@
     return dpp_launch_status();
 }
 
+extern "C" int dpp_act_from_partials_ok(int consumer, int K, int nb) {
+    if (nb < 1 || nb > 4 * DPP_WAVE) return 0;
+    return consumer == 0 ? K == 64 : (consumer == 1 ? (K == 32 || K == 64) : 0);
+}
+
 extern "C" int dpp_bn_eval_coeffs(const float* gamma, const float* run_mean, const float* run_inv_std, int C, float* mean,
                                   float* inv_std, float* scale, dpp_stream_t stream) {
     if (!gamma || !run_mean || !run_inv_std || !mean || !inv_std || !scale || C < 1) return DPP_E_BADARG;
diff --git a/deep-prior-pp_amd/csrc/conv3x3.hip b/deep-prior-pp_amd/csrc/conv3x3.hip
--- a/deep-prior-pp_amd/csrc/conv3x3.hip
+++ b/deep-prior-pp_amd/csrc/conv3x3.hip
@@ -30,6 +30,7 @@
     C3Stage sg;
     unsigned long long* prof;
     int ntiles, woff;
+    int coff;
 };
 
 typedef __bf16 c3_bf16x8 __attribute__((ext_vector_type(8)));
@@ -56,9 +57,28 @@
     x0 = bx << a.ltw;
 }
 
-template <int UB, class E, class TX>
+struct c3_no_mid {
+    static constexpr bool from_partials = false;
+    __device__ __forceinline__ void operator()(int, float4&, float4&) const {}
+};
+template <int U>
+struct c3_inline_mid {
+    static constexpr bool from_partials = true;
+    dpp_bn_inline<16, U>& bi;
+    const dpp_act& act;
+    bool writer;
+    float* s_mean;
+    float* s_scale;
+    __device__ __forceinline__ void operator()(int c0, float4& mu, float4& sc) const {
+        bi.reduce(act, writer, s_mean, s_scale);
+        __syncthreads();
+        mu = *reinterpret_cast<const float4*>(&s_mean[c0]);
+        sc = *reinterpret_cast<const float4*>(&s_scale[c0]);
+    }
+};
+template <int UB, class E, class TX, class Mid = c3_no_mid>
 __device__ __forceinline__ void stage_halo(const TX* __restrict__ X, int N, int H, int W, int Ci, const dpp_act& act, int n0,
-                                           int y0, int x0, int TH, int TW, int IMG, E* Ah, int LDA, int KP, const C3Stage& sg) {
+                                           int y0, int x0, int TH, int TW, int IMG, E* Ah, int LDA, int KP, const C3Stage& sg, Mid mid = Mid()) {
     if (KP < Ci) KP = Ci;
     const int HW2 = (TH + 2) * (TW + 2), TW2 = TW + 2;
     const int HP = IMG * HW2;
@@ -68,10 +88,13 @@
     const bool cld = c0 < Ci;
     float4 mu = make_float4(0.f, 0.f, 0.f, 0.f), sc = mu, be = mu;
     if (cld && (act.mode & 2)) {
-        mu = *reinterpret_cast<const float4*>(act.mean + c0);
-        sc = *reinterpret_cast<const float4*>(act.scale + c0);
+        if (!Mid::from_partials) {
+            mu = *reinterpret_cast<const float4*>(act.mean + c0);
+            sc = *reinterpret_cast<const float4*>(act.scale + c0);
+        }
         be = *reinterpret_cast<const float4*>(act.beta + c0);
     }
+    bool first = true;
     for (int hb = (int)threadIdx.x >> sg.lqp; hb < HP; hb += UB * hstep) {
         float4 v[UB];
         bool in[UB];
@@ -85,6 +108,7 @@
             v[u] = make_float4(0.f, 0.f, 0.f, 0.f);
             if (in[u]) v[u] = dpp_ld4(X + (((size_t)n * H + y) * W + x) * Ci + c0);
         }
+        if (first) { mid(c0, mu, sc); first = false; }
 #pragma unroll
         for (int u = 0; u < UB; ++u) {
             const int hp = hb + u * hstep;
@@ -103,8 +127,9 @@
     }
 }
 
-template <int BM, int BN, int PREC = 0, class TX = float, bool EST = false>
+template <int BM, int BN, int PREC = 0, class TX = float, bool EST = false, int INL = 0>
 __global__ __launch_bounds__(DPP_THREADS) void conv3x3_kernel(Conv3Args a) {
+    static_assert(!INL || (PREC == 0 && !EST && std::is_same<TX, float>::value), "coefficients from partials: the float32 form");
     dpp_kernarg_warm<sizeof(Conv3Args)>();
     HIP_DYNAMIC_SHARED(float4, smem4)
     float* smem = reinterpret_cast<float*>(smem4);
@@ -125,6 +150,13 @@
     dpp_stamp(a.prof, 0);
     dpp_wide_coef wco;
     if (a.wide) wco.load<BN>(col0, a.Co, a.bias, a.epi, a.Y);
+    if constexpr (INL > 0) {
+        const bool writer = blockIdx.x == 0 && blockIdx.y == 0;
+        dpp_bn_inline<16, INL> bi;
+        bi.request(a.act, writer);
+        stage_halo<8>(reinterpret_cast<const TX*>(a.X), a.N, a.H, a.W, Ci, a.act, n0, y0, x0, TH, TW, a.img, Ah, LDA, KP, a.sg,
+                      c3_inline_mid<INL>{bi, a.act, writer, smem + a.coff, smem + a.coff + 64});
+    } else
     if (((HP + (DPP_THREADS >> a.sg.lqp) - 1) >> (8 - a.sg.lqp)) <= 4)
         stage_halo<4>(reinterpret_cast<const TX*>(a.X), a.N, a.H, a.W, Ci, a.act, n0, y0, x0, TH, TW, a.img, Ah, LDA, KP, a.sg);
     else
@@ -716,7 +748,14 @@
     a.X = X; a.N = N; a.H = H; a.W = W; a.Ci = Ci; a.Co = Co;
     a.prof = dpp_prof_buffer;
     if (act && (act->mode & 4)) return DPP_E_UNSUPPORTED;
+    const bool inl = act && (act->mode & DPP_ACT_FROM_PARTIALS) && act->partial;
+    if (inl) {
+        if (!(act->mode & 2) || precision || store || act->cmod != Ci || !dpp_act_from_partials_ok(0, Ci, act->nb)) return DPP_E_UNSUPPORTED;
+        if (!act->gamma || !act->mean || !act->inv_std || !act->scale || !act->beta || act->rpb < 1 || act->nb != dpp_cdiv(act->M, act->rpb))
+            return DPP_E_BADARG;
+    }
     if (act) a.act = *act; else { a.act.mode = 0; a.act.cmod = 1; a.act.mean = a.act.scale = a.act.beta = nullptr; }
+    if (!inl) a.act.mode &= ~DPP_ACT_FROM_PARTIALS;
     a.Wk = Wk; a.bias = bias; a.residual = residual; a.Y = Y;
     if (epi) a.epi = *epi; else a.epi = dpp_epilogue{};
     if (a.epi.bn_x && !(a.epi.bn_mean && a.epi.bn_inv_std && a.epi.bn_scale && a.epi.bn_beta && a.epi.bn_partial)) return DPP_E_BADARG;
@@ -744,6 +783,12 @@
     if ((store & (DPP_ST_C | DPP_ST_BNX)) && !a.wide) return DPP_E_UNSUPPORTED;
     size_t need = a.wide ? ((size_t)bm * (bn + 4) + 16 * bn) * sizeof(float) : (size_t)4 * bn * sizeof(float);
     if (lds < need) lds = need;
+    a.coff = 0;
+    if (inl) {
+        lds = (lds + 15) & ~(size_t)15;
+        a.coff = (int)(lds / sizeof(float));
+        lds += 2 * 64 * sizeof(float);
+    }
     if (lds > 160 * 1024) return DPP_E_UNSUPPORTED;
     dim3 grid(nblk, dpp_cdiv(Co, bn));
     hipStream_t st = static_cast<hipStream_t>(stream);
@@ -759,7 +804,7 @@
     const char* g1e = getenv("DPP_C3_P_64");
     const int geom1_on = g1e ? atoi(g1e) : 1;
     const bool geom1 = (geom1_on >= 2 || (geom1_on == 1 && precision)) && Ci == 64 && H == 8 && W == 8 && a.img == 2 && TH == 8 && TW == 8;
-    if (persist > 0 && a.wide && Ci == Co && bm == 128 && p_always && (geom0 || geom1) && (long)N * H * W * Ci < (1L << 31)) {
+    if (persist > 0 && !inl && a.wide && Ci == Co && bm == 128 && p_always && (geom0 || geom1) && (long)N * H * W * Ci < (1L << 31)) {
         const int pbn = geom1 ? 16 : (Ci == 64 ? bn64 : Co);
         const size_t pneed = ((size_t)bm * (pbn + 4) + 16 * pbn) * sizeof(float);
         const size_t region0 = (halo * rowb > pneed ? halo * rowb : pneed);
@@ -794,6 +839,14 @@
 #define DPP_C3(BM_, BN_) if (bm == BM_ && bn == BN_) { \
         if (precision) { if (store & DPP_ST_A) DPP_C3E(BM_, BN_, 1, dpp_bf16); else DPP_C3E(BM_, BN_, 1, float); } \
         if (store & DPP_ST_A) DPP_C3E(BM_, BN_, 0, dpp_bf16); else DPP_C3E(BM_, BN_, 0, float); }
+#define DPP_C3N(BM_, BN_) if (bm == BM_ && bn == BN_) { \
+        if (lds > 64 * 1024) { (void)hipFuncSetAttribute(reinterpret_cast<const void*>(&conv3x3_kernel<BM_, BN_, 0, float, false, 2>), hipFuncAttributeMaxDynamicSharedMemorySize, (int)lds); \
+                               (void)hipFuncSetAttribute(reinterpret_cast<const void*>(&conv3x3_kernel<BM_, BN_, 0, float, false, 4>), hipFuncAttributeMaxDynamicSharedMemorySize, (int)lds); } \
+        if (act->nb <= 2 * DPP_WAVE) DPP_LAUNCH((conv3x3_kernel<BM_, BN_, 0, float, false, 2>), grid, dim3(DPP_THREADS), lds, st, a); \
+        else DPP_LAUNCH((conv3x3_kernel<BM_, BN_, 0, float, false, 4>), grid, dim3(DPP_THREADS), lds, st, a); \
+        return dpp_launch_status(); }
+    if (inl) { DPP_C3N(128, 64) DPP_C3N(128, 32) DPP_C3N(128, 16) DPP_C3N(64, 64) DPP_C3N(64, 32) DPP_C3N(64, 16) return DPP_E_UNSUPPORTED; }
+#undef DPP_C3N
     DPP_C3(128, 64) DPP_C3(128, 32) DPP_C3(128, 16) DPP_C3(64, 64) DPP_C3(64, 32) DPP_C3(64, 16)
 #undef DPP_C3
 #undef DPP_C3E
@@ -869,7 +922,7 @@
     const int y16 = (store & DPP_ST_B) ? 1 : 0;
     Wgrad3Args a;
     a.X = X; a.N = N; a.H = H; a.W = W; a.Ci = Ci; a.Co = Co; a.dY = dY; a.partial = partial;
-    if (act && (act->mode & 4)) return DPP_E_UNSUPPORTED;
+    if (act && (act->mode & (4 | DPP_ACT_FROM_PARTIALS))) return DPP_E_UNSUPPORTED;
     if (act) a.act = *act; else { a.act.mode = 0; a.act.cmod = 1; a.act.mean = a.act.scale = a.act.beta = nullptr; }
     pick_tile(N, H, W, bm, a.lth, a.ltw, a.img);
     int TH = 1 << a.lth, TW = 1 << a.ltw;
diff --git a/deep-prior-pp_amd/csrc/conv3x3_wgrad_t.hip b/deep-prior-pp_amd/csrc/conv3x3_wgrad_t.hip
--- a/deep-prior-pp_amd/csrc/conv3x3_wgrad_t.hip
+++ b/deep-prior-pp_amd/csrc/conv3x3_wgrad_t.hip
@@ -328,7 +328,7 @@
     static const bool on = []() { const char* e = getenv("DPP_WGRAD3_T"); return !(e && e[0] == '0'); }();
     if (!on || Ci != Co || (Ci != 16 && Ci != 32 && Ci != 64) || W < 12 || H < 4) return false;
     if ((long)N * H * W * Ci >= (1L << 31)) return false;
-    if (act && ((act->mode & 4) || (act->mode && (act->cmod & 3)))) return false;
+    if (act && ((act->mode & (4 | DPP_ACT_FROM_PARTIALS)) || (act->mode && (act->cmod & 3)))) return false;
     return true;
 }
 
diff --git a/deep-prior-pp_amd/csrc/convpool.hip b/deep-prior-pp_amd/csrc/convpool.hip
--- a/deep-prior-pp_amd/csrc/convpool.hip
+++ b/deep-prior-pp_amd/csrc/convpool.hip
@@ -477,7 +477,7 @@
 
 extern "C" int dpp_convpool_fwd(const float* X, int N, int H, int W, int Ci, const dpp_act* act, const float* Wk, int kh, int kw, int pad,
                                 int Co, int pool, const float* bias, float* Y, uint16_t* ties, dpp_stream_t stream) {
-    if (act && (act->mode & 4)) return DPP_E_UNSUPPORTED;
+    if (act && (act->mode & (4 | DPP_ACT_FROM_PARTIALS))) return DPP_E_UNSUPPORTED;
     cp_geom g;
     if (!X || !Wk || !bias || !Y || !cp_make_geom(g, N, H, W, Ci, kh, kw, pad, Co, pool)) return DPP_E_BADARG;
     size_t lds = (size_t)g.sy * g.sx * Ci * sizeof(float);
@@ -510,7 +510,7 @@
 
 extern "C" int dpp_convpool_wgrad(const float* X, int N, int H, int W, int Ci, const dpp_act* act, const float* dY, const uint16_t* ties,
                                   int kh, int kw, int pad, int Co, int pool, float* partial, dpp_stream_t stream) {
-    if (act && (act->mode & 4)) return DPP_E_UNSUPPORTED;
+    if (act && (act->mode & (4 | DPP_ACT_FROM_PARTIALS))) return DPP_E_UNSUPPORTED;
     cp_geom g;
     if (!X || !dY || !partial || !cp_make_geom(g, N, H, W, Ci, kh, kw, pad, Co, pool) || (pool > 1 && !ties)) return DPP_E_BADARG;
     size_t lds = ((size_t)g.sy * g.sx * Ci + 2 * 64 * Co) * sizeof(float);
diff --git a/deep-prior-pp_amd/csrc/dpp_common.h b/deep-prior-pp_amd/csrc/dpp_common.h
--- a/deep-prior-pp_amd/csrc/dpp_common.h
+++ b/deep-prior-pp_amd/csrc/dpp_common.h
@@ -195,6 +195,124 @@
 }
 
 __device__ __forceinline__ size_t dpp_partial_index(int s, int c, int b, int C, int NB) { return ((size_t)s * C + c) * NB + b; }
+
+__device__ __forceinline__ double dpp_wave_allsum(double v) {
+    for (int o = 1; o < DPP_WAVE; o <<= 1) v += __shfl_xor(v, o);
+    return v;
+}
+
+template <int U, int GT>
+__device__ __forceinline__ void dpp_bn_sweep_load(const float* __restrict__ pm_row, const float* __restrict__ pq_row, int nbs, int lane,
+                                                  float& K, float (&pm)[U], float (&pq)[U]) {
+    K = pm_row[0];
+#pragma unroll
+    for (int u = 0; u < U; ++u) {
+        const int b = lane + u * GT;
+        const int bb = b < nbs ? b : nbs - 1;
+        pm[u] = pm_row[bb];
+        pq[u] = pq_row[bb];
+    }
+}
+
+__device__ __forceinline__ int dpp_bn_block_rows(int bi, int rpb, int M) { return (bi * rpb + rpb <= M) ? rpb : (M - bi * rpb); }
+
+template <int U, int GT>
+__device__ __forceinline__ void dpp_bn_sweep_sums(float K, const float (&pm)[U], const float (&pq)[U], int nbs, int rpb, int M, int lane,
+                                                  double& s1, double& s2) {
+    s1 = 0.0; s2 = 0.0;
+#pragma unroll
+    for (int u = 0; u < U; ++u) {
+        const int b = lane + u * GT;
+        if (b < nbs) {
+#pragma clang fp contract(off)
+            const double d = (double)pm[u] - (double)K, nb_ = (double)dpp_bn_block_rows(b, rpb, M);
+            const double t = nb_ * d;
+            s1 = __builtin_fma(nb_, d, s1);
+            s2 = s2 + __builtin_fma(t, d, (double)pq[u]);
+        }
+    }
+}
+
+__device__ __forceinline__ void dpp_bn_sweep_finish(float K, double s1, double s2, int M, float eps, float& meanf, float& inv_std) {
+#pragma clang fp contract(off)
+    const double mean1 = (double)K + s1 / (double)M;
+    const double var1 = (s2 - s1 * s1 / (double)M) / (double)M;
+    meanf = (float)mean1;
+    inv_std = (float)(1.0 / sqrt((var1 > 0.0 ? var1 : 0.0) + (double)eps));
+}
+
+__device__ __forceinline__ void dpp_bn_coef_store(int c, float meanf, float inv_std, float gam, float* __restrict__ mean_o,
+                                                  float* __restrict__ inv_std_o, float* __restrict__ scale_o, bool upd, float alpha,
+                                                  float rm_old, float ri_old, float* __restrict__ run_mean, float* __restrict__ run_inv_std) {
+#pragma clang fp contract(off)
+    mean_o[c] = meanf;
+    inv_std_o[c] = inv_std;
+    scale_o[c] = gam * inv_std;
+    if (upd) {
+        const float oma = 1.0f - alpha;
+        run_mean[c] = oma * rm_old + alpha * meanf;
+        run_inv_std[c] = oma * ri_old + alpha * inv_std;
+    }
+}
+
+template <int CPW, int U>
+struct dpp_bn_inline {
+    static_assert(CPW == 8 || CPW == 16, "32 or 64 input channels");
+    float K[CPW], pm[CPW][U], pq[CPW][U];
+    float Kown, gam, rm_old, ri_old;
+    int cown;
+    static constexpr int LOG = CPW == 16 ? 4 : 3;
+
+    __device__ __forceinline__ void request(const dpp_act& a, bool writer) {
+        const int lane = threadIdx.x & 63, wave = threadIdx.x >> 6, C = 4 * CPW;
+        int rev = 0;
+#pragma unroll
+        for (int lv = 0; lv < LOG; ++lv) rev |= (lane & (1 << lv)) ? (CPW >> (lv + 1)) : 0;
+        cown = wave * CPW + rev;
+#pragma unroll
+        for (int j = 0; j < CPW; ++j) {
+            const int c = wave * CPW + j;
+            dpp_bn_sweep_load<U, DPP_WAVE>(a.partial + dpp_partial_index(0, c, 0, C, a.nb), a.partial + dpp_partial_index(1, c, 0, C, a.nb),
+                                           a.nb, lane, K[j], pm[j], pq[j]);
+        }
+        Kown = a.partial[dpp_partial_index(0, cown, 0, C, a.nb)];
+        gam = a.gamma[cown];
+        const bool upd = writer && a.alpha > 0.0f && a.run_mean != nullptr;
+        rm_old = (upd ? a.run_mean : a.gamma)[cown];
+        ri_old = (upd ? a.run_inv_std : a.gamma)[cown];
+    }
+
+    __device__ __forceinline__ void reduce(const dpp_act& a, bool writer, float* s_mean, float* s_scale) {
+        const int lane = threadIdx.x & 63;
+        double s1[CPW], s2[CPW];
+#pragma unroll
+        for (int j = 0; j < CPW; ++j) dpp_bn_sweep_sums<U, DPP_WAVE>(K[j], pm[j], pq[j], a.nb, a.rpb, a.M, lane, s1[j], s2[j]);
+#pragma unroll
+        for (int lv = 0; lv < LOG; ++lv) {
+            const int m = 1 << lv, n = CPW >> lv;
+            const bool up = (lane & m) != 0;
+#pragma unroll
+            for (int i = 0; i < n / 2; ++i) {
+                const double k1 = up ? s1[i + n / 2] : s1[i], g1 = up ? s1[i] : s1[i + n / 2];
+                const double k2 = up ? s2[i + n / 2] : s2[i], g2 = up ? s2[i] : s2[i + n / 2];
+                s1[i] = k1 + __shfl_xor(g1, m);
+                s2[i] = k2 + __shfl_xor(g2, m);
+            }
+        }
+        double t1 = s1[0], t2 = s2[0];
+#pragma unroll
+        for (int lv = LOG; lv < 6; ++lv) { t1 += __shfl_xor(t1, 1 << lv); t2 += __shfl_xor(t2, 1 << lv); }
+        float meanf, inv_std;
+        dpp_bn_sweep_finish(Kown, t1, t2, a.M, a.eps, meanf, inv_std);
+        if (lane < CPW) {
+            s_mean[cown] = meanf;
+            s_scale[cown] = gam * inv_std;
+            if (writer)
+                dpp_bn_coef_store(cown, meanf, inv_std, gam, const_cast<float*>(a.mean), a.inv_std, const_cast<float*>(a.scale),
+                                  a.alpha > 0.0f && a.run_mean != nullptr, a.alpha, rm_old, ri_old, a.run_mean, a.run_inv_std);
+        }
+    }
+};
 
 
 template <int CN, int WM, int WN, int BN>
diff --git a/deep-prior-pp_amd/csrc/gemm.hip b/deep-prior-pp_amd/csrc/gemm.hip
--- a/deep-prior-pp_amd/csrc/gemm.hip
+++ b/deep-prior-pp_amd/csrc/gemm.hip
@@ -115,10 +115,13 @@
     if (d.splitk > 1 && (d.epi.stats || d.epi.bn_x)) return DPP_E_BADARG;
     if (d.epi.bn_x && !(d.epi.bn_mean && d.epi.bn_inv_std && d.epi.bn_scale && d.epi.bn_beta && d.epi.bn_partial)) return DPP_E_BADARG;
     if (d.splitk == 1 && !d.C) return DPP_E_BADARG;
+    if ((d.actA.mode & DPP_ACT_FROM_PARTIALS) && !d.actA.partial) d.actA.mode &= ~DPP_ACT_FROM_PARTIALS;
+    if ((d.actB.mode & DPP_ACT_FROM_PARTIALS) && !d.actB.partial) d.actB.mode &= ~DPP_ACT_FROM_PARTIALS;
     if (d.actA.mode && d.actA.cmod <= 0) return DPP_E_BADARG;
     if (d.actB.mode && d.actB.cmod <= 0) return DPP_E_BADARG;
     ga.vecA = aligned16(d.A) && (d.lda % 4 == 0);
     if (d.actB.mode & 4) return DPP_E_UNSUPPORTED;
+    if ((d.actB.mode & DPP_ACT_FROM_PARTIALS) || ((d.actA.mode & DPP_ACT_FROM_PARTIALS) && d.variant != 4)) return DPP_E_UNSUPPORTED;
     if (d.actA.mode & 4) {
         if (d.actA.mode != 4 || d.variant == 1 || !d.actA.x2 || !d.actA.aux || !d.actA.mean || !d.actA.scale || !d.actA.beta) return DPP_E_BADARG;
         ga.vecA = ga.vecA && aligned16(d.actA.x2) && aligned16(d.actA.out);
diff --git a/deep-prior-pp_amd/csrc/gemm_expand.hip b/deep-prior-pp_amd/csrc/gemm_expand.hip
--- a/deep-prior-pp_amd/csrc/gemm_expand.hip
+++ b/deep-prior-pp_amd/csrc/gemm_expand.hip
@@ -2,9 +2,10 @@
 
 namespace {
 
-template <int KT, bool BKC, bool IT2, bool ACT, bool RES, bool BNB, bool LZ = false, bool PB = false, bool ST = false>
+template <int KT, bool BKC, bool IT2, bool ACT, bool RES, bool BNB, bool LZ = false, bool PB = false, bool ST = false, int INL = 0>
 __global__ __launch_bounds__(DPP_THREADS) DPP_WAVES_PER_EU(1, 2) void gemm_expand_kernel(GemmArgs ga, int rpw) {
     static_assert(!PB || ((KT % 32 == 0 || KT == 16) && !LZ), "bf16 MFMA operands: whole 32-deep steps, or K = 16 with a zero upper half");
+    static_assert(!INL || (BKC && ACT && !LZ && !PB && !ST && KT >= 32), "coefficients from partials: the float32 forward form");
     dpp_kernarg_warm<sizeof(GemmArgs)>();
     const dpp_gemm_desc& d = ga.d;
     constexpr int KL = KT / 4, KV = KL / 4;
@@ -12,7 +13,7 @@
     const int lane = threadIdx.x & 63, l15 = lane & 15, kq = lane >> 4;
     const int NG = d.N >> 6, nblk = d.M / rpw;
     const int gw = blockIdx.x * 4 + (threadIdx.x >> 6);
-    if (gw >= NG * nblk) return;
+    if (!INL && gw >= NG * nblk) return;
     const int cg = gw % NG, rblk = gw / NG;
     const int n0 = cg * 64 + 4 * l15;
     const int wrow0 = rblk * rpw, iters = rpw / RI;
@@ -77,15 +78,30 @@
     Regs g0, g1;
     fetch(g0, 0);
     float4 mu[KV], sc[KV], be[KV], ax[LZ ? KV : 1];
-#pragma unroll
-    for (int j = 0; j < KV; ++j) {
-        mu[j] = sc[j] = be[j] = make_float4(0.f, 0.f, 0.f, 0.f);
-        if (LZ || (modeA & 2)) {
-            mu[j] = *reinterpret_cast<const float4*>(d.actA.mean + kq * KL + 4 * j);
-            sc[j] = *reinterpret_cast<const float4*>(d.actA.scale + kq * KL + 4 * j);
-            be[j] = *reinterpret_cast<const float4*>(d.actA.beta + kq * KL + 4 * j);
-        }
-        if (LZ) ax[j] = *reinterpret_cast<const float4*>(d.actA.aux + kq * KL + 4 * j);
+    if constexpr (INL) {
+        __shared__ float s_mean[KT], s_scale[KT];
+        dpp_bn_inline<KT / 4, INL> bi;
+        bi.request(d.actA, blockIdx.x == 0);
+#pragma unroll
+        for (int j = 0; j < KV; ++j) be[j] = *reinterpret_cast<const float4*>(d.actA.beta + kq * KL + 4 * j);
+        bi.reduce(d.actA, blockIdx.x == 0, s_mean, s_scale);
+        __syncthreads();
+#pragma unroll
+        for (int j = 0; j < KV; ++j) {
+            mu[j] = *reinterpret_cast<const float4*>(&s_mean[kq * KL + 4 * j]);
+            sc[j] = *reinterpret_cast<const float4*>(&s_scale[kq * KL + 4 * j]);
+        }
+    } else {
+#pragma unroll
+        for (int j = 0; j < KV; ++j) {
+            mu[j] = sc[j] = be[j] = make_float4(0.f, 0.f, 0.f, 0.f);
+            if (LZ || (modeA & 2)) {
+                mu[j] = *reinterpret_cast<const float4*>(d.actA.mean + kq * KL + 4 * j);
+                sc[j] = *reinterpret_cast<const float4*>(d.actA.scale + kq * KL + 4 * j);
+                be[j] = *reinterpret_cast<const float4*>(d.actA.beta + kq * KL + 4 * j);
+            }
+            if (LZ) ax[j] = *reinterpret_cast<const float4*>(d.actA.aux + kq * KL + 4 * j);
+        }
     }
     const bool lz_store = LZ && d.actA.out != nullptr && cg == 0;
     float4 cbias = make_float4(0.f, 0.f, 0.f, 0.f), cmean = cbias, cscale = cbias, cbeta = cbias, cistd = cbias;
@@ -271,6 +287,11 @@
     if (d.N % 64 || d.M % 32) return 0;
     if (d.mapA.s != 1 || d.mapB.s != 1 || d.mapC.s != 1 || d.actB.mode != 0) return 0;
     if (d.actA.mode != 0 && d.actA.cmod < d.K) return 0;
+    if (d.actA.mode & DPP_ACT_FROM_PARTIALS) {
+        const dpp_act& a = d.actA;
+        if (!d.b_kc || !(a.mode & 2) || (a.mode & 4) || d.store || d.precision || a.cmod != d.K || !dpp_act_from_partials_ok(1, d.K, a.nb)) return 0;
+        if (!a.gamma || !a.mean || !a.inv_std || !a.scale || !a.beta || a.rpb < 1 || a.nb != dpp_cdiv(a.M, a.rpb)) return 0;
+    }
     if (d.epi.stats && d.epi.bn_x) return 0;
     if (d.b_kc ? (d.epi.bn_x != nullptr || (d.actA.mode & 4)) : (d.actA.mode != 0 && d.actA.mode != 4)) return 0;
     if (d.actA.mode == 4 && d.actA.out && d.lda != d.K) return 0;
@@ -278,6 +299,7 @@
     int rpw = d.bm;
     if (rpw <= 0) rpw = d.M >= 65536 ? 128 : (d.M >= 16384 ? 64 : 32);
     if (rpw % 32 || d.M % rpw) return 0;
+    if ((d.actA.mode & DPP_ACT_FROM_PARTIALS) && ((d.M / rpw) * (d.N / 64)) % 4) return 0;
     return rpw;
 }
 
@@ -291,6 +313,17 @@
     const bool it2 = rpw > 32, act = d.actA.mode != 0, res = d.residual != nullptr, bnb = d.epi.bn_x != nullptr, lz = d.actA.mode == 4;
     const bool pb = d.precision == 1;
     const bool stg = d.store != 0;
+    if constexpr (KT >= 32) {
+        if (d.actA.mode & DPP_ACT_FROM_PARTIALS) {
+#define DPP_EXN(I_, R_, U_) DPP_LAUNCH((gemm_expand_kernel<KT, true, I_, true, R_, false, false, false, false, U_>), grid, dim3(DPP_THREADS), 0, st, ga, rpw)
+#define DPP_EXN_U(I_, R_) do { if (d.actA.nb <= 2 * DPP_WAVE) DPP_EXN(I_, R_, 2); else DPP_EXN(I_, R_, 4); } while (0)
+            if (it2) { if (res) DPP_EXN_U(true, true); else DPP_EXN_U(true, false); }
+            else { if (res) DPP_EXN_U(false, true); else DPP_EXN_U(false, false); }
+#undef DPP_EXN_U
+#undef DPP_EXN
+            return dpp_launch_status();
+        }
+    }
 #define DPP_EXS(K_, I_, A_, R_, B_, L_, P_, S_) DPP_LAUNCH((gemm_expand_kernel<KT, K_, I_, A_, R_, B_, L_, P_, S_>), grid, dim3(DPP_THREADS), 0, st, ga, rpw)
 #define DPP_EX(K_, I_, A_, R_, B_, L_, P_) do { if (!(L_) && stg) DPP_EXS(K_, I_, A_, R_, B_, L_, P_, !(L_)); else DPP_EXS(K_, I_, A_, R_, B_, L_, P_, false); } while (0)
 #define DPP_EX_P(K_, I_, A_, R_, B_) do { if (pb) { DPP_EX(K_, I_, A_, R_, B_, false, true); break; } \
diff --git a/deep-prior-pp_amd/hipdp/engine.py b/deep-prior-pp_amd/hipdp/engine.py
--- a/deep-prior-pp_amd/hipdp/engine.py
+++ b/deep-prior-pp_amd/hipdp/engine.py
@@ -334,11 +334,42 @@
                 return True
         return False
 
+    def _sole_conv_consumer(self, var):
+        while True:
+            cons = self.consumers.get(id(var), [])
+            if len(cons) != 1:
+                return None
+            c = cons[0]
+            if c.kind == 'relu' or (c.kind == 'layer' and _layer_kind(c.layer) == 'NonlinearityLayer'):
+                var = c
+            elif c.kind == 'layer' and _layer_kind(c.layer) == 'ConvLayer':
+                return c
+            else:
+                return None
+
+    def _flush_bn(self, view):
+        b = getattr(view, 'bn', None)
+        if b is not None and getattr(b, 'pending_finalize', None) is not None:
+            self.fwd.add(b.pending_finalize[0])
+            b.pending_finalize = None
+
+    def _bn_inline_act(self, view, consumer, K):
+        b = view.bn
+        if b is None or getattr(b, 'pending_finalize', None) is None or self.store16 or self.prec or view.chan != K:
+            return None
+        geo = b.pending_finalize[1]
+        if not self.rt.lib.dpp_act_from_partials_ok(consumer, K, geo['nb']):
+            return None
+        mode = Act.BN | (Act.RELU if view.relu else 0)
+        return ops.act_from_partials(mode, b, geo['partial'], geo['nb'], geo['rpb'], geo['M'], geo['eps'], geo['alpha'], K)
+
     def _emit_layer(self, var, residual, out_var=None):
         layer = var.layer
         kind = _layer_kind(layer)
         rt, st = self.rt, self.store
         src = self._emit(var.inputs[0])
+        if kind not in ('ConvLayer', 'NonlinearityLayer'):
+            self._flush_bn(src)
         if kind == 'BatchNormLayer':
             if not src.plain:
                 raise NotImplementedError("BatchNorm on a non-materialised input")
@@ -353,8 +384,13 @@
             fused = getattr(src.base, 'stats', None) if self.train else None
             if fused is not None:
                 part, nblk, rows = fused
-                self.fwd.add(ops.bn_finalize(rt, part, nblk, M, rows, C, b.gamma_buf, layer.cfgParams.epsilon, b.mean, b.inv_std,
-                                             b.scale, b.run_mean, b.run_inv_std, layer.cfgParams.alpha))
+                fin = ops.bn_finalize(rt, part, nblk, M, rows, C, b.gamma_buf, layer.cfgParams.epsilon, b.mean, b.inv_std,
+                                      b.scale, b.run_mean, b.run_inv_std, layer.cfgParams.alpha)
+                if 0 < 8 * nblk * C <= hz.BN_INLINE_MAX_BYTES and self._sole_conv_consumer(var) is not None:
+                    b.pending_finalize = (fin, dict(partial=part, nb=nblk, rpb=rows, M=M, eps=layer.cfgParams.epsilon,
+                                                    alpha=layer.cfgParams.alpha))
+                else:
+                    self.fwd.add(fin)
             elif self.train:
                 W = b.world
                 part = self.scratch(b.nb * 2 * C * (W + 1)).view(0, (b.nb * 2 * C,))
@@ -473,12 +509,21 @@
                                 name='conv1x1_%d' % layer.layerNum, precision=self._gemm_prec(variant, Ci))
             if variant in (2, 3, 4) and ops.gemm_variant_rows(rt, build(tile, variant, None)) != tile[0]:
                 variant, (tile, _) = 0, hz.gemm_plan(M, Co, Ci, allow_split=False)
+            inl = self._bn_inline_act(src, 1, Ci) if variant == 4 else None
+            if inl is not None:
+                plain, act = act, inl
+                if ops.gemm_variant_rows(rt, build(tile, variant, None)) == tile[0]:
+                    src.bn.pending_finalize = None
+                else:
+                    act = plain
+            self._flush_bn(src)
             if want_stats:
                 nblk = -(-M // tile[0])
                 out.stats = (rt.alloc((nblk, 2, Co), zero=False), nblk, tile[0])
                 epi = ops.epilogue(stats=out.stats[0])
             self.fwd.add(build(tile, variant, epi))
         elif self._conv3_stream(N, Hi, Wi, Ci, Co, src.base.buf, out.buf) and residual is None:
+            self._flush_bn(src)
             rows = rt.lib.dpp_conv3x3_stream_rows(N, Hi, Wi, Ci)
             if want_stats:
                 out.stats = (rt.alloc((M // rows, 2, Co), zero=False), M // rows, rows)
@@ -487,6 +532,10 @@
                                             name='conv3x3_%d' % layer.layerNum))
         else:
             bm = hz.conv3x3_bm(M, Co, hw=(Hi, Wi), prec=self.prec)
+            inl = self._bn_inline_act(src, 0, Ci)
+            if inl is not None:
+                act, src.bn.pending_finalize = inl, None
+            self._flush_bn(src)
             if want_stats:
                 th, tw, img = (C_int() for _ in range(3))
                 nblk = rt.lib.dpp_conv3x3_tiling(N, Hi, Wi, bm, th, tw, img)
diff --git a/deep-prior-pp_amd/hipdp/heuristics.py b/deep-prior-pp_amd/hipdp/heuristics.py
--- a/deep-prior-pp_amd/hipdp/heuristics.py
+++ b/deep-prior-pp_amd/hipdp/heuristics.py
@@ -9,6 +9,7 @@
 BN_RPB_TARGET_BLOCKS = int(knob('DPP_BN_BLOCKS', '1024'))
 BN_BWD_FUSE_MAX_BLOCKS = int(knob('DPP_BN_BWD_FUSE_NB', '0'))
 BN_BWD_FUSE_TARGET_WGS = int(knob('DPP_BN_BWD_FUSE_WGS', '512'))
+BN_INLINE_MAX_BYTES = int(knob('DPP_BN_INLINE_BYTES', str(128 * 1024)))
 
 
 
diff --git a/deep-prior-pp_amd/hipdp/lib.py b/deep-prior-pp_amd/hipdp/lib.py
--- a/deep-prior-pp_amd/hipdp/lib.py
+++ b/deep-prior-pp_amd/hipdp/lib.py
@@ -4,7 +4,7 @@
 _HERE = os.path.dirname(os.path.abspath(__file__))
 DEFAULT_LIB = os.path.join(os.path.dirname(_HERE), 'lib', 'libdpp_hip.so')
 
-ABI_VERSION = 13
+ABI_VERSION = 14
 ST_A, ST_B, ST_C, ST_BNX = 1, 2, 4, 8
 c_float_p = C.c_void_p
 stream_t = C.c_void_p
@@ -24,9 +24,12 @@
 
 class Act(C.Structure):
     _fields_ = [('mean', C.c_void_p), ('scale', C.c_void_p), ('beta', C.c_void_p), ('mode', C.c_int), ('cmod', C.c_int),
-                ('x2', C.c_void_p), ('aux', C.c_void_p), ('out', C.c_void_p)]
-
-    NONE, RELU, BN, BN_RELU, BN_BWD = 0, 1, 2, 3, 4
+                ('x2', C.c_void_p), ('aux', C.c_void_p), ('out', C.c_void_p),
+                ('partial', C.c_void_p), ('gamma', C.c_void_p), ('inv_std', C.c_void_p), ('run_mean', C.c_void_p),
+                ('run_inv_std', C.c_void_p), ('nb', C.c_int), ('rpb', C.c_int), ('M', C.c_int), ('eps', C.c_float),
+                ('alpha', C.c_float), ('pad_', C.c_int)]
+
+    NONE, RELU, BN, BN_RELU, BN_BWD, FROM_PARTIALS = 0, 1, 2, 3, 4, 8
 
     @staticmethod
     def none():
@@ -97,6 +100,7 @@
     'dpp_bn_stats_partial': (C.c_int, [C.c_void_p, C.c_int, C.c_int, C.c_int, C.c_void_p, C.c_int, stream_t]),
     'dpp_bn_finalize': (C.c_int, [C.c_void_p, C.c_int, C.c_int, C.c_int, C.c_int, C.c_int, C.c_void_p, C.c_float, C.c_void_p,
                                   C.c_void_p, C.c_void_p, C.c_void_p, C.c_void_p, C.c_float, stream_t]),
+    'dpp_act_from_partials_ok': (C.c_int, [C.c_int, C.c_int, C.c_int]),
     'dpp_bn_eval_coeffs': (C.c_int, [C.c_void_p, C.c_void_p, C.c_void_p, C.c_int, C.c_void_p, C.c_void_p, C.c_void_p,
                                      stream_t]),
     'dpp_bn_eval_job_bytes': (C.c_size_t, []),
diff --git a/deep-prior-pp_amd/hipdp/ops.py b/deep-prior-pp_amd/hipdp/ops.py
--- a/deep-prior-pp_amd/hipdp/ops.py
+++ b/deep-prior-pp_amd/hipdp/ops.py
@@ -225,6 +225,15 @@
     return a
 
 
+def act_from_partials(mode, bn, partial, nb, rpb, M, eps, alpha, C):
+    a = act(mode | Act.FROM_PARTIALS, bn.mean, bn.scale, bn.beta_buf, C)
+    a.partial, a.gamma, a.inv_std = partial.ptr, bn.gamma_buf.ptr, bn.inv_std.ptr
+    a.run_mean, a.run_inv_std = _p(bn.run_mean), _p(bn.run_inv_std)
+    a.nb, a.rpb, a.M, a.eps, a.alpha = int(nb), int(rpb), int(M), float(eps), float(alpha)
+    a._keep = a._keep + (partial, bn)
+    return a
+
+
 def act_bn_bwd(bn, q, p, x, C, out=None):
     return act(Act.BN_BWD, mean=bn.mean, scale=bn.scale, beta=q, cmod=C, x2=x, aux=p, out=out)
 
diff --git a/include/dpp_hip.h b/include/dpp_hip.h
--- a/include/dpp_hip.h
+++ b/include/dpp_hip.h
@@ -14,7 +14,7 @@
 #define DPP_E_BADARG 10001
 #define DPP_E_UNSUPPORTED 10002
 
-#define DPP_ABI_VERSION 13
+#define DPP_ABI_VERSION 14
 int dpp_abi_version(void);
 
 #define DPP_ST_A 1
@@ -35,7 +35,17 @@
     const float* x2;
     const float* aux;
     float* out;
+    const float* partial;
+    const float* gamma;
+    float* inv_std;
+    float* run_mean;
+    float* run_inv_std;
+    int nb, rpb, M;
+    float eps, alpha;
+    int pad_;
 } dpp_act;
+#define DPP_ACT_FROM_PARTIALS 8
+int dpp_act_from_partials_ok(int consumer, int K, int nb);
 
 typedef struct {
     float* stats;
```

After: 36700 depth-crops/sec. 2.8% lower.
